# sovrasov/3d-object-detection.pytorch

Hardware: AMD Instinct MI355X
Metric: regression train crops/sec @224^2 bs256 MobileNetV2 (higher is better)
Workload: dtype bf16; 1 GPU; mobilenetv2 9-class Objectron keypoint regression, train step (fwd + l1/add/CE losses + bwd + AdamW), 224x224 crops, per-GPU batch 256; global_batch=256, parallelism=dp1, roofline_sampled_steps=0, rccl_ranks=0

## Files before the change

### 3d-object-detection.pytorch_amd/csrc/abi.hip

```cpp
#include <cstddef>
#include <initializer_list>
#include <type_traits>

#include "../../include/t3d.h"
#include "abi_entries.h"

namespace {

template <class T>
struct Unknown : std::false_type {};

template <class T>
constexpr char type_code() {
  using U = std::remove_cv_t<std::remove_pointer_t<T>>;
  if constexpr (std::is_pointer<T>::value) {
    if constexpr (std::is_same<U, t3d_prologue>::value) return 'P';
    else if constexpr (std::is_same<U, t3d_bnbwd>::value) return 'B';
    else if constexpr (std::is_same<U, t3d_loss_cfg>::value) return 'L';
    else if constexpr (std::is_same<U, t3d_draw_style>::value) return 'S';
    else if constexpr (std::is_same<U, t3d_bn_fold>::value) return 'F';
    else {
      static_assert(!std::is_function<U>::value, "t3d.h: a function pointer is not a data pointer");
      return 'p';
    }
  } else if constexpr (std::is_same<T, int>::value) return 'i';
  else if constexpr (std::is_same<T, long long>::value) return 'l';
  else if constexpr (std::is_same<T, unsigned long long>::value) return 'u';
  else if constexpr (std::is_same<T, float>::value) return 'f';
  else if constexpr (std::is_same<T, double>::value) return 'd';
  else {
    static_assert(Unknown<T>::value, "t3d.h: an argument type the ABI table has no code for (see t3d_abi_entry)");
    return '?';
  }
}

template <class... A>
struct Types {
  static constexpr char str[sizeof...(A) + 1] = {type_code<A>()..., '\0'};
};
template <class... A>
constexpr const char* types_of(int (*)(A...)) { return Types<A...>::str; }

struct Entry { const char* name; const char* types; int in_step; };
#define T3D_S(fn) {#fn, types_of(&fn), 1},
#define T3D_Q(fn) {#fn, types_of(&fn), 0},
constexpr Entry kEntries[] = {T3D_ABI_ENTRIES(T3D_S, T3D_Q)};
#undef T3D_S
#undef T3D_Q
constexpr int kNumEntries = (int)(sizeof(kEntries) / sizeof(kEntries[0]));

struct Field { const char* name; size_t offset, bytes; };
struct Text { char s[640]; };

template <size_t N>
constexpr Text describe(const Field (&f)[N]) {
  Text t{};
  size_t n = 0;
  for (size_t i = 0; i < N; ++i) {
    if (i) t.s[n++] = ',';
    for (const char* c = f[i].name; *c; ++c) t.s[n++] = *c;
    for (size_t v : {f[i].offset, f[i].bytes}) {
      t.s[n++] = ':';
      size_t div = 1;
      while (v / div >= 10) div *= 10;
      for (; div; div /= 10) t.s[n++] = (char)('0' + v / div % 10);
    }
  }
  t.s[n] = '\0';
  return t;
}

#define F(m) {#m, offsetof(T3D_THIS, m), sizeof(T3D_THIS::m)},
#define T3D_STRUCT(type, members)                        \
  namespace layout_##type {                              \
  using T3D_THIS = type;                                 \
  constexpr Field fields[] = {members};                  \
  constexpr Text text = describe(fields);                \
  }
T3D_STRUCT(t3d_prologue, F(scale) F(shift) F(se) F(act) F(se_after_act))
T3D_STRUCT(t3d_bnbwd, F(alpha) F(beta) F(gamma) F(per_sample))
T3D_STRUCT(t3d_aug_sample, F(offset) F(h) F(w) F(flags) F(alpha) F(beta255) F(reserved) F(m))
T3D_STRUCT(t3d_aug_chain, F(n_ops) F(flags) F(kind) F(p) F(m2))
T3D_STRUCT(t3d_det_sample, F(offset) F(h) F(w) F(turns) F(left) F(top) F(cx0) F(cy0) F(cx1) F(cy1) F(flags) F(delta) F(alpha)
           F(sat) F(hue) F(perm) F(reserved))
T3D_STRUCT(t3d_jpeg_info, F(h) F(w) F(ncomp) F(sampling) F(mcus_x) F(mcus_y) F(seg_mcus) F(nseg) F(scan_offset) F(scan_bytes)
           F(reason) F(reserved) F(comp_dc) F(comp_ac) F(quant) F(dc_bits) F(dc_vals) F(ac_bits) F(ac_vals))
T3D_STRUCT(t3d_jpeg_seg, F(byte) F(pred) F(bit) F(reserved) F(mcu))
T3D_STRUCT(t3d_jpeg_item, F(file_offset) F(file_bytes) F(out_offset) F(block_offset) F(seg_offset) F(reserved))
T3D_STRUCT(t3d_loss_cfg, F(c_l1) F(c_mse) F(c_smoothl1) F(smoothl1_beta) F(c_add) F(c_diag) F(c_wing) F(wing_w) F(wing_eps)
           F(c_ce) F(lam_reg) F(lam_cls))
T3D_STRUCT(t3d_draw_style, F(rect_th) F(edge_th) F(kp_radius) F(font_scale) F(flags) F(colors))
T3D_STRUCT(t3d_bn_fold, F(kind) F(C) F(nrep) F(rstride) F(stats) F(count) F(gamma) F(beta) F(rm) F(rv) F(nbt) F(momentum)
           F(eps) F(o0) F(o1) F(o2) F(o3) F(o4) F(mean) F(invstd))
#undef T3D_STRUCT
#undef F

struct Struct { const char* name; int size; const char* fields; };
#define T3D_ROW(type) {#type, (int)sizeof(type), layout_##type::text.s},
constexpr Struct kStructs[] = {
    T3D_ROW(t3d_prologue) T3D_ROW(t3d_bnbwd) T3D_ROW(t3d_aug_sample) T3D_ROW(t3d_aug_chain) T3D_ROW(t3d_det_sample)
    T3D_ROW(t3d_jpeg_info) T3D_ROW(t3d_jpeg_seg) T3D_ROW(t3d_jpeg_item) T3D_ROW(t3d_loss_cfg) T3D_ROW(t3d_draw_style)
    T3D_ROW(t3d_bn_fold)};
#undef T3D_ROW
constexpr int kNumStructs = (int)(sizeof(kStructs) / sizeof(kStructs[0]));

}

extern "C" int t3d_abi_entry(int index, const char** name, const char** types, int* in_step) {
  if (index < 0 || index >= kNumEntries) return T3D_ERR_ARG;
  if (name) *name = kEntries[index].name;
  if (types) *types = kEntries[index].types;
  if (in_step) *in_step = kEntries[index].in_step;
  return T3D_OK;
}

extern "C" int t3d_abi_struct(int index, const char** name, int* size, const char** fields) {
  if (index < 0 || index >= kNumStructs) return T3D_ERR_ARG;
  if (name) *name = kStructs[index].name;
  if (size) *size = kStructs[index].size;
  if (fields) *fields = kStructs[index].fields;
  return T3D_OK;
}
```

### 3d-object-detection.pytorch_amd/csrc/elementwise.hip

```cpp
#include "common.h"

namespace {

template <typename T, bool U8>
__global__ __launch_bounds__(256) void im2col_kernel(const void* __restrict__ xin, const float* __restrict__ mean,
                                                     const float* __restrict__ istd, T* __restrict__ col, int B,
                                                     int H, int W, int Ho, int Wo) {
  extern __shared__ float tile[];
  const int WP = W + 2;
  const int hp = (Ho + 1) / 2;
  const int b = blockIdx.x / hp, oy0 = (blockIdx.x % hp) * 2;
  const int iy0 = oy0 * 2 - 1;
  const int tid = threadIdx.x;
  for (int i = tid; i < 15 * 2; i += 256) {
    const int rr = i >> 1;
    tile[rr * WP + ((i & 1) ? W + 1 : 0)] = 0.f;
  }
  if constexpr (U8) {
    const unsigned char* xu = reinterpret_cast<const unsigned char*>(xin);
    const float mu[3] = {mean[0], mean[1], mean[2]}, is[3] = {istd[0], istd[1], istd[2]};
    const int RB = W * 3;
    if ((RB & 3) == 0) {
      const int R4 = RB >> 2;
      for (int i = tid; i < 5 * R4; i += 256) {
// ... 177 lines not shown
  load_affine(a, c0, sc, sh);
#pragma unroll
  for (int j = 0; j < 8; ++j) s1[j] = s2[j] = 0.f;
  if (on) {
    for (size_t i = g; i < nvec; i += nthr) {
      float d[8], yv[8];
      Vec8<T>::load(dv + i * 8, d);
      Vec8<T>::load(y + i * 8, yv);
      const size_t bo = (i / CG / a.HW) * a.C + c0;
#pragma unroll
      for (int j = 0; j < 8; ++j) {
        const float da = fmaf(a.vec[bo + j], d[j], a.vec2[bo + j]);
        const float v = Vec8<T>::round(da * act_grad(yv[j] * sc[j] + sh[j], a.act));
        d[j] = v;
        s1[j] += v;
        s2[j] = fmaf(v, yv[j], s2[j]);
      }
      Vec8<T>::store(o + i * 8, d);
    }
  }
  if (a.stats) flush_stats(lstat, a.C, c0, on, s1, s2, a.stats);
}

__device__ __forceinline__ int pool_cgs(int CG) {
  int c = 1;
  while (c < CG && c < 32) c <<= 1;
  return c;
}

template <typename T>
__global__ __launch_bounds__(256) void se_after_sums_kernel(const EwArgs a) {
  __shared__ float red[8 * 32 * 8];
  const int CG = a.C / 8, b = blockIdx.x;
  const int cgs = pool_cgs(CG), nslots = 256 / cgs, rowl = cgs * 8;
  const int cgl = threadIdx.x & (cgs - 1), slot = threadIdx.x / cgs;
  const int cg = blockIdx.y * cgs + cgl;
  const bool on = cg < CG;
  const int c0 = on ? cg * 8 : 0;
  const T* __restrict__ dv = reinterpret_cast<const T*>(a.a);
  const T* __restrict__ y = reinterpret_cast<const T*>(a.b);
  float sc[8], sh[8], acc[8];
  load_affine(a, c0, sc, sh);
#pragma unroll
  for (int j = 0; j < 8; ++j) acc[j] = 0.f;
  if (on) {
    for (int hw = slot; hw < a.HW; hw += nslots) {
      float v[8], d[8];
      const size_t off = ((size_t)b * a.HW + hw) * a.C + c0;
      Vec8<T>::load(y + off, v);
      Vec8<T>::load(dv + off, d);
      act_affine_vec<8>(v, sc, sh, a.act);
#pragma unroll
      for (int j = 0; j < 8; ++j) acc[j] = fmaf(d[j], v[j], acc[j]);
    }
  }
#pragma unroll
  for (int j = 0; j < 8; ++j) red[slot * rowl + cgl * 8 + j] = acc[j];
  __syncthreads();
  const int t = threadIdx.x;
  const int c = blockIdx.y * rowl + t;
  if (t < rowl && c < a.C) {
    float s = 0.f;
    for (int q = 0; q < nslots; ++q) s += red[q * rowl + t];
    a.pooled[((size_t)b * a.C + c) * 2] = s;
    a.pooled[((size_t)b * a.C + c) * 2 + 1] = 0.f;
  }
}

template <typename T>
__global__ __launch_bounds__(256) void gap_fwd_kernel(const EwArgs a) {
  __shared__ float red[8 * 32 * 8];
  __shared__ float redm[8 * 32 * 8];
  __shared__ int redi[8 * 32 * 8];
  const int CG = a.C / 8, b = blockIdx.x;
  const int cgs = pool_cgs(CG), nslots = 256 / cgs, rowl = cgs * 8;
  const int cgl = threadIdx.x & (cgs - 1), slot = threadIdx.x / cgs;
  const int cg = blockIdx.y * cgs + cgl;
  const bool on = cg < CG;
  const int c0 = on ? cg * 8 : 0;
  const bool want_max = a.mode != T3D_POOL_AVG;
  const T* __restrict__ y = reinterpret_cast<const T*>(a.a);
  float sc[8], sh[8], acc[8], mx[8];
  int mi[8];
  load_affine(a, c0, sc, sh);
#pragma unroll
  for (int j = 0; j < 8; ++j) { acc[j] = 0.f; mx[j] = -INFINITY; mi[j] = 0; }
  if (on) {
    for (int hw = slot; hw < a.HW; hw += nslots) {
      float v[8];
      Vec8<T>::load(y + ((size_t)b * a.HW + hw) * a.C + c0, v);
      act_affine_vec<8>(v, sc, sh, a.act);
#pragma unroll
      for (int j = 0; j < 8; ++j) {
        acc[j] += v[j];
        if (v[j] > mx[j]) { mx[j] = v[j]; mi[j] = hw; }
      }
    }
  }
#pragma unroll
  for (int j = 0; j < 8; ++j) {
    red[slot * rowl + cgl * 8 + j] = acc[j];
    if (want_max) { redm[slot * rowl + cgl * 8 + j] = mx[j]; redi[slot * rowl + cgl * 8 + j] = mi[j]; }
  }
  __syncthreads();
  const int t = threadIdx.x;
  const int c = blockIdx.y * rowl + t;
  if (t < rowl && c < a.C) {
    float s = 0.f;
    for (int q = 0; q < nslots; ++q) s += red[q * rowl + t];
    float out = s * a.inv_hw;
    if (want_max) {
      float m = redm[t];
      int im = redi[t];
      for (int q = 1; q < nslots; ++q) {
        const float mq = redm[q * rowl + t];
        const int iq = redi[q * rowl + t];
        if (mq > m || (mq == m && iq < im)) { m = mq; im = iq; }
      }
      if (a.argmax) a.argmax[(size_t)b * a.C + c] = im;
      out = (a.mode == T3D_POOL_MAX) ? m : out + m;
    }
    a.pooled[(size_t)b * a.C + c] = out;
  }
}

template <typename T>
__global__ __launch_bounds__(256) void gap_bwd_kernel(const EwArgs a, int B, const int g_nrep, const long long g_rstride) {
  __shared__ float red[2][8 * 32 * 8];
  const int CG = a.C / 8;
  const int cgs = pool_cgs(CG), nslots = 256 / cgs, rowl = cgs * 8;
  const int cgl = threadIdx.x & (cgs - 1), slot = threadIdx.x / cgs;
  const int cg = blockIdx.y * cgs + cgl;
  const bool on = cg < CG;
  const int c0 = on ? cg * 8 : 0;
  const T* __restrict__ y = reinterpret_cast<const T*>(a.a);
  T* __restrict__ dz = reinterpret_cast<T*>(a.out);
  float sc[8], sh[8], s1[8], s2[8];
  load_affine(a, c0, sc, sh);
#pragma unroll
  for (int j = 0; j < 8; ++j) s1[j] = s2[j] = 0.f;
  if (on) {
    for (int b = blockIdx.x; b < B; b += gridDim.x) {
      float dp[8], dm[8];
      int am[8];
#pragma unroll
      for (int j = 0; j < 8; ++j) {
        const float g = a.vec[(size_t)b * a.C + c0 + j];
        dp[j] = (a.mode == T3D_POOL_MAX) ? 0.f : g * a.inv_hw;
        dm[j] = (a.mode == T3D_POOL_AVG) ? 0.f : g;
        am[j] = (a.mode == T3D_POOL_AVG) ? -1 : a.argmax[(size_t)b * a.C + c0 + j];
      }
      for (int hw = slot; hw < a.HW; hw += nslots) {
        const size_t off = ((size_t)b * a.HW + hw) * a.C + c0;
        float v[8], d[8];
        Vec8<T>::load(y + off, v);
#pragma unroll
        for (int j = 0; j < 8; ++j) d[j] = dp[j] + (hw == am[j] ? dm[j] : 0.f);
        act_grad_affine_vec<8>(d, v, sc, sh, a.act);
#pragma unroll
        for (int j = 0; j < 8; ++j) {
          d[j] = Vec8<T>::round(d[j]);
          s1[j] += d[j];
          s2[j] = fmaf(d[j], v[j], s2[j]);
        }
        Vec8<T>::store(dz + off, d);
      }
    }
  }
  if (a.stats) {
#pragma unroll
    for (int j = 0; j < 8; ++j) {
      red[0][slot * rowl + cgl * 8 + j] = s1[j];
      red[1][slot * rowl + cgl * 8 + j] = s2[j];
    }
    __syncthreads();
    const int t = threadIdx.x, c = blockIdx.y * rowl + t;
    if (t < rowl && c < a.C) {
      double u1 = 0.0, u2 = 0.0;
      for (int q = 0; q < nslots; ++q) {
        u1 += (double)red[0][q * rowl + t];
        u2 += (double)red[1][q * rowl + t];
      }
      double* st = a.stats + (size_t)(blockIdx.x % g_nrep) * g_rstride;
      atomicAdd(st + c, u1);
      atomicAdd(st + a.C + c, u2);
    }
  }
}

inline void fill_pro(EwArgs& a, const t3d_prologue* pro) {
  if (pro) { a.scale = pro->scale; a.shift = pro->shift; a.act = pro->act; }
}
inline int ew_grid(size_t nvec) {
  size_t g = (nvec + 255) / 256;
  return (int)(g < 1 ? 1 : (g > 2048 ? 2048 : g));
}

}

static int im2col_launch(int dtype, const void* x, bool u8, const float* mean, const float* istd, void* col, int B,
                         int H, int W, void* stream) {
  if (!x || !col || B <= 0 || H <= 0 || W <= 0 || (u8 && (!mean || !istd))) return T3D_ERR_ARG;
  const int Ho = (H + 2 - 3) / 2 + 1, Wo = (W + 2 - 3) / 2 + 1;
  const int grid = B * ((Ho + 1) / 2);
  const size_t lds = (size_t)15 * (W + 2) * sizeof(float);
  if (lds > 64 * 1024) return T3D_ERR_UNSUPPORTED;
  hipStream_t st = reinterpret_cast<hipStream_t>(stream);
#define T3D_IM2COL(T, U) \
  T3D_LAUNCH((im2col_kernel<T, U>), dim3(grid), dim3(256), lds, st, x, mean, istd, (T*)col, B, H, W, Ho, Wo)
  if (dtype == T3D_F32) {
    if (u8) T3D_IM2COL(float, true); else T3D_IM2COL(float, false);
  } else if (dtype == T3D_BF16) {
    if (u8) T3D_IM2COL(bf16_t, true); else T3D_IM2COL(bf16_t, false);
  } else if (dtype == T3D_F16) {
    if (u8) T3D_IM2COL(f16_t, true); else T3D_IM2COL(f16_t, false);
  } else {
    return T3D_ERR_ARG;
  }
#undef T3D_IM2COL
  T3D_CHECK_LAUNCH();
  return T3D_OK;
}

extern "C" int t3d_stem_im2col(int dtype, const float* x, void* col, int B, int H, int W, void* stream) {
  return im2col_launch(dtype, x, false, nullptr, nullptr, col, B, H, W, stream);
}

extern "C" int t3d_stem_im2col_u8(int dtype, const unsigned char* x, const float* mean, const float* inv_std, void* col,
                                  int B, int H, int W, void* stream) {
  return im2col_launch(dtype, x, true, mean, inv_std, col, B, H, W, stream);
}

extern "C" int t3d_bn_apply(int dtype, const void* y, const t3d_prologue* pro, const void* residual, void* z,
                            int M, int C, void* stream) {
  if (!y || !z || M <= 0 || C <= 0 || (C % 8)) return T3D_ERR_ARG;
  if (pro && pro->se) return T3D_ERR_UNSUPPORTED;
  EwArgs a{};
  a.a = y; a.res = residual; a.out = z; a.M = M; a.C = C;
  fill_pro(a, pro);
  const int grid = ew_grid((size_t)M * (C / 8));
  if ((size_t)grid * 256 < (size_t)(C / 8)) return T3D_ERR_UNSUPPORTED;
  hipStream_t st = reinterpret_cast<hipStream_t>(stream);
  a.fold = t3d_take_fold(a.scale);
  const size_t lds = a.fold ? (size_t)2 * C * sizeof(float) : 0;
  if (dtype == T3D_F32) T3D_LAUNCH(bn_apply_kernel<float>, dim3(grid), dim3(256), lds, st, a);
  else if (dtype == T3D_BF16) T3D_LAUNCH(bn_apply_kernel<bf16_t>, dim3(grid), dim3(256), lds, st, a);
  else if (dtype == T3D_F16) T3D_LAUNCH(bn_apply_kernel<f16_t>, dim3(grid), dim3(256), lds, st, a);
  else return T3D_ERR_ARG;
  T3D_CHECK_LAUNCH();
  return T3D_OK;
}

extern "C" int t3d_bn_act_bwd(int dtype, const void* dz, const void* y, const t3d_prologue* pro, void* dzp,
                              double* stats, int M, int C, void* stream) {
  if (!dz || !y || !dzp || M <= 0 || C <= 0 || (C % 8)) return T3D_ERR_ARG;
  if (pro && pro->se) return T3D_ERR_UNSUPPORTED;
  EwArgs a{};
  a.a = dz; a.b = y; a.out = dzp; a.stats = stats; a.M = M; a.C = C;
  fill_pro(a, pro);
  int grid = ew_grid((size_t)M * (C / 8));
  if (grid > 1024) grid = 1024;
  if ((size_t)grid * 256 < (size_t)(C / 8)) return T3D_ERR_UNSUPPORTED;
  const size_t lds = (size_t)2 * C * sizeof(double);
  hipStream_t st = reinterpret_cast<hipStream_t>(stream);
  if (dtype == T3D_F32) T3D_LAUNCH(bn_act_bwd_kernel<float>, dim3(grid), dim3(256), lds, st, a);
  else if (dtype == T3D_BF16) T3D_LAUNCH(bn_act_bwd_kernel<bf16_t>, dim3(grid), dim3(256), lds, st, a);
  else return T3D_ERR_ARG;
  T3D_CHECK_LAUNCH();
  return T3D_OK;
}

extern "C" int t3d_se_after_sums(int dtype, const void* dv, const void* y, const t3d_prologue* pro, float* ps, int B, int HW,
                                 int C, void* stream) {
  if (!dv || !y || !ps || B <= 0 || HW <= 0 || C <= 0 || (C % 8)) return T3D_ERR_ARG;
  if (pro && pro->se) return T3D_ERR_UNSUPPORTED;
  EwArgs a{};
  a.a = dv; a.b = y; a.pooled = ps; a.C = C; a.HW = HW;
  fill_pro(a, pro);
  dim3 grid(B, cdiv(C / 8, 32));
  hipStream_t st = reinterpret_cast<hipStream_t>(stream);
  if (const int rc = t3d_fold_fallback(a.scale, st)) return rc;
  if (dtype == T3D_F32) T3D_LAUNCH(se_after_sums_kernel<float>, grid, dim3(256), 0, st, a);
  else if (dtype == T3D_BF16) T3D_LAUNCH(se_after_sums_kernel<bf16_t>, grid, dim3(256), 0, st, a);
  else return T3D_ERR_ARG;
  T3D_CHECK_LAUNCH();
  return T3D_OK;
}

extern "C" int t3d_se_after_apply(int dtype, const void* dv, const void* y, const t3d_prologue* pro, const float* s,
                                  const float* g, void* du, double* stats, int B, int HW, int C, void* stream) {
  if (!dv || !y || !s || !g || !du || B <= 0 || HW <= 0 || C <= 0 || (C % 8)) return T3D_ERR_ARG;
  if (pro && pro->se) return T3D_ERR_UNSUPPORTED;
  EwArgs a{};
  a.a = dv; a.b = y; a.out = du; a.stats = stats; a.vec = s; a.vec2 = g; a.M = B * HW; a.C = C; a.HW = HW;
  fill_pro(a, pro);
  int grid = ew_grid((size_t)a.M * (C / 8));
  if (grid > 1024) grid = 1024;
  if ((size_t)grid * 256 < (size_t)(C / 8)) return T3D_ERR_UNSUPPORTED;
  const size_t lds = (size_t)2 * C * sizeof(double);
  hipStream_t st = reinterpret_cast<hipStream_t>(stream);
  if (dtype == T3D_F32) T3D_LAUNCH(se_after_apply_kernel<float>, dim3(grid), dim3(256), lds, st, a);
  else if (dtype == T3D_BF16) T3D_LAUNCH(se_after_apply_kernel<bf16_t>, dim3(grid), dim3(256), lds, st, a);
  else return T3D_ERR_ARG;
  T3D_CHECK_LAUNCH();
  return T3D_OK;
}

extern "C" int t3d_pool_fwd(int dtype, const void* y, const t3d_prologue* pro, int mode, float* pooled, int* argmax,
                            int B, int HW, int C, void* stream) {
  if (!y || !pooled || B <= 0 || HW <= 0 || C <= 0 || (C % 8)) return T3D_ERR_ARG;
  if (mode != T3D_POOL_AVG && mode != T3D_POOL_MAX && mode != T3D_POOL_AVGMAX) return T3D_ERR_ARG;
  if (pro && pro->se) return T3D_ERR_UNSUPPORTED;
  EwArgs a{};
  a.a = y; a.pooled = pooled; a.C = C; a.HW = HW; a.inv_hw = 1.f / (float)HW; a.mode = mode; a.argmax = argmax;
  fill_pro(a, pro);
  dim3 grid(B, cdiv(C / 8, 32));
  hipStream_t st = reinterpret_cast<hipStream_t>(stream);
  if (const int rc = t3d_fold_fallback(a.scale, st)) return rc;
  if (dtype == T3D_F32) T3D_LAUNCH(gap_fwd_kernel<float>, grid, dim3(256), 0, st, a);
  else if (dtype == T3D_BF16) T3D_LAUNCH(gap_fwd_kernel<bf16_t>, grid, dim3(256), 0, st, a);
  else if (dtype == T3D_F16) T3D_LAUNCH(gap_fwd_kernel<f16_t>, grid, dim3(256), 0, st, a);
  else return T3D_ERR_ARG;
  T3D_CHECK_LAUNCH();
  return T3D_OK;
}

extern "C" int t3d_gap_fwd(int dtype, const void* y, const t3d_prologue* pro, float* pooled, int B, int HW, int C,
                           void* stream) {
  return t3d_pool_fwd(dtype, y, pro, T3D_POOL_AVG, pooled, nullptr, B, HW, C, stream);
}

extern "C" int t3d_pool_bwd(int dtype, const float* dpooled, const void* y, const t3d_prologue* pro, int mode,
                            const int* argmax, void* dz, double* stats, int B, int HW, int C, void* stream) {
  if (!dpooled || !y || !dz || B <= 0 || HW <= 0 || C <= 0 || (C % 8)) return T3D_ERR_ARG;
  if (mode != T3D_POOL_AVG && mode != T3D_POOL_MAX && mode != T3D_POOL_AVGMAX) return T3D_ERR_ARG;
  if (mode != T3D_POOL_AVG && !argmax) return T3D_ERR_ARG;
  if (pro && pro->se) return T3D_ERR_UNSUPPORTED;
  EwArgs a{};
  a.a = y; a.vec = dpooled; a.out = dz; a.stats = stats; a.C = C; a.HW = HW; a.inv_hw = 1.f / (float)HW;
  a.mode = mode; a.argmax = const_cast<int*>(argmax);
  fill_pro(a, pro);
  dim3 grid(B < 256 ? B : 256, cdiv(C / 8, 32));
  hipStream_t st = reinterpret_cast<hipStream_t>(stream);
  if (dtype == T3D_F32) T3D_LAUNCH(gap_bwd_kernel<float>, grid, dim3(256), 0, st, a, B, g_t3d_reduce.nrep, g_t3d_reduce.stats_stride);
  else if (dtype == T3D_BF16) T3D_LAUNCH(gap_bwd_kernel<bf16_t>, grid, dim3(256), 0, st, a, B, g_t3d_reduce.nrep, g_t3d_reduce.stats_stride);
  else return T3D_ERR_ARG;
  T3D_CHECK_LAUNCH();
  return T3D_OK;
}
```

### 3d-object-detection.pytorch_amd/csrc/pwconv_common.h

```cpp
#pragma once
#include "common.h"

namespace t3d_pw {

struct GemmArgs {
  const void* a0;
  const void* a1;
  const float *p0, *p1, *p2;
  int act, se_after, per_sample, dgrad;
  const void* w;
  const float* bias;
  const void* e_y;
  const float *e_scale, *e_shift, *e_se;
  int e_act, e_se_after;
  const void* e_res;
  void* out;
  double* stats;
  float* ps_stats;
  int ps_wave;
  int M, HW, Kin, Nout, mtiles;
  int kz;
  float* part;
  const void* a2;
  int Kin2, ks1;
  int row0;
  const T3dFold* fold;
  const void* z_res;
  void* z_out;
  int unused_[8];
  int wfrag;
  T3dQuant quant;
};

template <typename T> __device__ __forceinline__ void ldvec(const T* p, float* v);
template <> __device__ __forceinline__ void ldvec<float>(const float* p, float* v) {
  const float4 a = *reinterpret_cast<const float4*>(p);
  v[0] = a.x; v[1] = a.y; v[2] = a.z; v[3] = a.w;
}
template <> __device__ __forceinline__ void ldvec<bf16_t>(const bf16_t* p, float* v) { Vec8<bf16_t>::load(p, v); }
template <typename T> __device__ __forceinline__ void stvec(T* p, const float* v);
template <> __device__ __forceinline__ void stvec<float>(float* p, const float* v) {
  *reinterpret_cast<float4*>(p) = make_float4(v[0], v[1], v[2], v[3]);
}
template <> __device__ __forceinline__ void stvec<bf16_t>(bf16_t* p, const float* v) { Vec8<bf16_t>::store(p, v); }


}
```

### 3d-object-detection.pytorch_amd/csrc/pwconv_deep.hip

```cpp
#include <cstdlib>
#include <type_traits>
#include "pwconv_route.h"

namespace t3d_pw {
namespace {

__device__ __forceinline__ f32x2 deep_fma_clamp01(f32x2 a, f32x2 b, f32x2 c) {
  f32x2 d;
  asm("v_pk_fma_f32 %0, %1, %2, %3 clamp" : "=v"(d) : "v"(a), "v"(b), "v"(c));
  return d;
}

#ifdef T3D_PW_TRACE
__device__ unsigned long long g_deep_trace[16];
#define DEEP_STAMP(i)                                                                                     \
  do {                                                                                                    \
    if (threadIdx.x == 0 && blockIdx.y == 0 && (blockIdx.x == 0 || blockIdx.x == gridDim.x - 1))         \
      g_deep_trace[(blockIdx.x == 0 ? 0 : 8) + (i)] = wall_clock64();                                     \
  } while (0)
#else
#define DEEP_STAMP(i)
#endif

constexpr int RT = 4;
constexpr int NW = 8;

template <bool DG, int NTW, int KSP>
__global__ __launch_bounds__(64 * NW) void pw_deep_kernel(const GemmArgs a, const int KS, const int ntiles, const int nrep,
                                                             const long long rstride) {
  constexpr int IT = RT * KSP / NW;
  static_assert(IT >= 1 && IT * NW == RT * KSP, "staging items must divide over the waves");
  extern __shared__ __attribute__((aligned(16))) unsigned char smem[];
  bf16x8* Af = reinterpret_cast<bf16x8*>(smem);
  const int kpad = KS * 32;
  float* coef = reinterpret_cast<float*>(smem + (size_t)2 * RT * KSP * 1024);
  const int BN = ntiles * 16;
  float* ecoef = coef + 3 * kpad;
  double* dstat = reinterpret_cast<double*>(ecoef + 2 * BN);

  const int tid = threadIdx.x, lane = tid & 63, wave = tid >> 6;
  const int lg = lane >> 4, lc = lane & 15;
  const int m0 = blockIdx.x * (16 * RT), n0 = blockIdx.y * BN;
  const bf16_t* __restrict__ A0 = reinterpret_cast<const bf16_t*>(a.a0);
  const bf16_t* __restrict__ A1 = reinterpret_cast<const bf16_t*>(a.a1);
  bf16_t* __restrict__ out = reinterpret_cast<bf16_t*>(a.out);
  const int nph = (KS + KSP - 1) / KSP;
  DEEP_STAMP(0);

  int tix[NTW];
  bool tok[NTW];
  const int tlast = min(ntiles, (a.Nout - n0 + 31) / 32 * 2) - 1;
  const bf16x8* wt_[NTW];
#pragma unroll
  for (int i = 0; i < NTW; ++i) {
    const int t = wave + NW * i;
    tok[i] = t <= tlast;
    tix[i] = min(t, tlast);
    wt_[i] = reinterpret_cast<const bf16x8*>(a.w) + ((size_t)(n0 / 16 + tix[i]) * KS) * 64 + lane;
  }
  bf16x8 wf[2][KSP][NTW];
  auto w_issue = [&](auto slot_tag, const int ph) {
    constexpr int SL = decltype(slot_tag)::value;
#pragma unroll
    for (int u = 0; u < KSP; ++u) {
      const int ks = min(ph * KSP + u, KS - 1);
#pragma unroll
      for (int t = 0; t < NTW; ++t) wf[SL][u][t] = wt_[t][(size_t)ks * 64];
    }
  };
  const int srt = wave % RT, sks = (wave / RT) * IT;
  const int mrow = min(m0 + srt * 16 + lc, a.M - 1);
  const size_t arow = (size_t)mrow * a.Kin + lg * 8;
  const bool rok = m0 + srt * 16 + lc < a.M;
  bf16x8 pa[2][IT], pb[DG ? 2 : 1][DG ? IT : 1];
  auto a_issue = [&](auto slot_tag, const int ph) {
    constexpr int SL = decltype(slot_tag)::value;
#pragma unroll
    for (int j = 0; j < IT; ++j) {
      const size_t o = arow + min((ph * KSP + sks + j) * 32, a.Kin - 8 - lg * 8);
      pa[SL][j] = *reinterpret_cast<const bf16x8*>(A0 + o);
      if (DG) pb[DG ? SL : 0][DG ? j : 0] = *reinterpret_cast<const bf16x8*>(A1 + o);
    }
  };
  w_issue(std::integral_constant<int, 0>{}, 0);
  a_issue(std::integral_constant<int, 0>{}, 0);
  a_issue(std::integral_constant<int, 1>{}, 1);

  for (int i = tid; i < BN * 2; i += 64 * NW) dstat[i] = 0.0;
  for (int i = tid; i < BN; i += 64 * NW) {
    const int n = n0 + i;
    const bool v = DG && a.e_scale && n < a.Nout;
    ecoef[i] = v ? a.e_scale[n] : 1.f;
    ecoef[BN + i] = v ? a.e_shift[n] : 0.f;
  }
  if (a.fold) {
    for (int i = a.Kin + tid; i < kpad; i += 64 * NW) {
      coef[i] = DG ? 0.f : 1.f; coef[kpad + i] = 0.f; coef[2 * kpad + i] = 0.f;
    }
    t3d_fold_block<DG ? 2 : 1>(a.fold, 0, a.Kin, coef, kpad, blockIdx.x == 0 && blockIdx.y == 0);
  } else {
    for (int i = tid; i < kpad; i += 64 * NW) {
      const bool v = i < a.Kin;
      if (!DG) {
        coef[i] = (v && a.p0) ? a.p0[i] : 1.f;
        coef[kpad + i] = (v && a.p0) ? a.p1[i] : 0.f;
      } else {
        coef[i] = v ? a.p0[i] : 0.f;
        coef[kpad + i] = v ? a.p1[i] : 0.f;
        coef[2 * kpad + i] = v ? a.p2[i] : 0.f;
      }
    }
    __syncthreads();
  }
  const bool c6f = !DG && a.p0 && a.act == T3D_ACT_RELU6;
  if (c6f) {
    for (int i = tid; i < 2 * kpad; i += 64 * NW) coef[i] *= T3D_SIXTH;
    __syncthreads();
  }
  const int fact = c6f ? -1 : a.act;
  DEEP_STAMP(1);

  f32x4 acc[RT][NTW];
#pragma unroll
  for (int r = 0; r < RT; ++r)
#pragma unroll
    for (int t = 0; t < NTW; ++t) acc[r][t] = f32x4{0.f, 0.f, 0.f, 0.f};

  auto phase = [&](auto slot_tag, const int ph) {
    constexpr int SL = decltype(slot_tag)::value;
    bf16x8* Ab = Af + (size_t)SL * RT * KSP * 64;
#pragma unroll
    for (int j = 0; j < IT; ++j) {
      const int k = (ph * KSP + sks + j) * 32 + lg * 8;
      const bool ok = rok && (k < a.Kin);
      const int kc = min(k, kpad - 8);
      const float4 c0a = *reinterpret_cast<const float4*>(coef + kc), c0b = *reinterpret_cast<const float4*>(coef + kc + 4);
      const float4 c1a = *reinterpret_cast<const float4*>(coef + kpad + kc),
                   c1b = *reinterpret_cast<const float4*>(coef + kpad + kc + 4);
      const float c0[8] = {c0a.x, c0a.y, c0a.z, c0a.w, c0b.x, c0b.y, c0b.z, c0b.w};
      const float c1[8] = {c1a.x, c1a.y, c1a.z, c1a.w, c1b.x, c1b.y, c1b.z, c1b.w};
      float x[8];
#pragma unroll
      for (int e = 0; e < 8; ++e) x[e] = (float)pa[SL][j][e];
      if (!DG) {
        if (fact == -1) {
#pragma unroll
          for (int e = 0; e < 8; e += 2) {
            const f32x2 t = deep_fma_clamp01(f32x2{x[e], x[e + 1]}, f32x2{c0[e], c0[e + 1]}, f32x2{c1[e], c1[e + 1]});
            x[e] = t[0];
            x[e + 1] = t[1];
          }
        } else {
          act_affine_vec<8>(x, c0, c1, fact);
        }
      } else {
        const float4 c2a = *reinterpret_cast<const float4*>(coef + 2 * kpad + kc),
                     c2b = *reinterpret_cast<const float4*>(coef + 2 * kpad + kc + 4);
        const float c2[8] = {c2a.x, c2a.y, c2a.z, c2a.w, c2b.x, c2b.y, c2b.z, c2b.w};
#pragma unroll
        for (int e = 0; e < 8; ++e) x[e] = c0[e] * x[e] + c1[e] * (float)pb[DG ? SL : 0][DG ? j : 0][e] + c2[e];
      }
      bf16x8 b;
#pragma unroll
      for (int e = 0; e < 8; ++e) b[e] = ok ? (bf16_t)x[e] : (bf16_t)0.f;
      Ab[(srt * KSP + sks + j) * 64 + lane] = b;
    }
    __syncthreads();
    if (ph == 0) DEEP_STAMP(2);
    __builtin_amdgcn_sched_barrier(0);
    w_issue(std::integral_constant<int, 1 - SL>{}, ph + 1);
    a_issue(std::integral_constant<int, SL>{}, ph + 2);
    __builtin_amdgcn_sched_barrier(0);
#pragma unroll
    for (int u = 0; u < KSP; ++u) {
      bf16x8 b[RT];
#pragma unroll
      for (int r = 0; r < RT; ++r) b[r] = Ab[(r * KSP + u) * 64 + lane];
#pragma unroll
      for (int t = 0; t < NTW; ++t)
#pragma unroll
        for (int r = 0; r < RT; ++r) acc[r][t] = __builtin_amdgcn_mfma_f32_16x16x32_bf16(wf[SL][u][t], b[r], acc[r][t], 0, 0, 0);
    }
    __builtin_amdgcn_sched_barrier(0);
  };
  for (int ph = 0; ph < nph; ph += 2) {
    phase(std::integral_constant<int, 0>{}, ph);
    if (ph + 1 < nph) phase(std::integral_constant<int, 1>{}, ph + 1);
  }

  DEEP_STAMP(3);
  const bool keep_stats = a.stats != nullptr;
  float st1[NTW][4], st2[NTW][4];
#pragma unroll
  for (int i = 0; i < NTW; ++i)
#pragma unroll
    for (int j = 0; j < 4; ++j) st1[i][j] = st2[i][j] = 0.f;
  bf16x4 eyr[DG ? RT : 1][NTW], err[DG ? RT : 1][NTW];
  if (DG) {
#pragma unroll
    for (int r = 0; r < RT; ++r) {
      const size_t mo = (size_t)min(m0 + r * 16 + lc, a.M - 1) * a.Nout;
#pragma unroll
      for (int i = 0; i < NTW; ++i) {
        const int n = min(n0 + (tix[i] >> 1) * 32 + lg * 8 + (tix[i] & 1) * 4, a.Nout - 4);
        if (a.e_y) eyr[DG ? r : 0][i] = *reinterpret_cast<const bf16x4*>(reinterpret_cast<const bf16_t*>(a.e_y) + mo + n);
        if (a.e_res) err[DG ? r : 0][i] = *reinterpret_cast<const bf16x4*>(reinterpret_cast<const bf16_t*>(a.e_res) + mo + n);
      }
    }
  }
#pragma unroll
  for (int r = 0; r < RT; ++r) {
    const int m = m0 + r * 16 + lc;
    const bool ok = m < a.M;
#pragma unroll
    for (int i = 0; i < NTW; ++i) {
      const int nl = (tix[i] >> 1) * 32 + lg * 8 + (tix[i] & 1) * 4, n = n0 + nl;
      if (!tok[i] || n >= a.Nout) continue;
      float v[4], yv[4];
#pragma unroll
      for (int j = 0; j < 4; ++j) v[j] = acc[r][i][j];
      if (c6f) {
#pragma unroll
        for (int j = 0; j < 4; ++j) v[j] *= 6.f;
      }
      if (DG && a.e_y) {
#pragma unroll
        for (int j = 0; j < 4; ++j) yv[j] = (float)eyr[DG ? r : 0][i][j];
        if (a.e_act != T3D_ACT_NONE) {
          const float4 s0 = *reinterpret_cast<const float4*>(ecoef + nl), h0 = *reinterpret_cast<const float4*>(ecoef + BN + nl);
          const float es[4] = {s0.x, s0.y, s0.z, s0.w}, eh[4] = {h0.x, h0.y, h0.z, h0.w};
          act_grad_affine_vec<4>(v, yv, es, eh, a.e_act);
        }
      }
      if (DG && a.e_res) {
#pragma unroll
        for (int j = 0; j < 4; ++j) v[j] += (float)err[DG ? r : 0][i][j];
      }
      bf16x4 o;
#pragma unroll
      for (int j = 0; j < 4; ++j) {
        o[j] = (bf16_t)v[j];
        v[j] = ok ? (float)o[j] : 0.f;
      }
      if (ok) *reinterpret_cast<bf16x4*>(out + (size_t)m * a.Nout + n) = o;
      if (keep_stats) {
#pragma unroll
        for (int j = 0; j < 4; ++j) {
          st1[i][j] += v[j];
          st2[i][j] = fmaf(v[j], (DG && a.e_y) ? yv[j] : v[j], st2[i][j]);
        }
      }
    }
  }
  DEEP_STAMP(4);
  if (keep_stats) {
#pragma unroll
    for (int i = 0; i < NTW; ++i) {
      const int nl = (tix[i] >> 1) * 32 + lg * 8 + (tix[i] & 1) * 4;
#pragma unroll
      for (int j = 0; j < 4; ++j) {
        const float s1 = row16_sum(st1[i][j]), s2 = row16_sum(st2[i][j]);
        if (lc == 0 && tok[i] && n0 + nl < a.Nout) {
          dstat[(nl + j) * 2] = t3d_snap(s1, a.quant, false);
          dstat[(nl + j) * 2 + 1] = t3d_snap(s2, a.quant, !DG);
        }
      }
    }
    __syncthreads();
    for (int i = tid; i < BN * 2; i += 64 * NW) {
      const int n = n0 + (i >> 1);
      if (n < a.Nout) atomicAdd(a.stats + (size_t)(blockIdx.x % nrep) * rstride + (size_t)(i & 1) * a.Nout + n, dstat[i]);
    }
  }
  DEEP_STAMP(5);
}

size_t deep_lds(int KS, int ntiles, int KSP = 4) { return (size_t)2 * RT * KSP * 1024 + (size_t)3 * KS * 32 * 4 + (size_t)ntiles * 16 * (2 * 4 + 2 * 8); }

template <bool DG, int NTW, int KSP>
int launch_deep(GemmArgs& a, int KS, int ntiles, int nchunks, hipStream_t st) {
  const size_t lds = deep_lds(KS, ntiles, KSP);
  const void* fn = (const void*)pw_deep_kernel<DG, NTW, KSP>;
  if (lds > 64 * 1024) (void)t3d_max_lds(fn, (int)lds);
  a.quant = (!DG && a.stats && !T3D_ENV_SET("T3D_NO_SNAP")) ? t3d_quant_for(a.M) : T3dQuant{0.0, 0.0};
  a.fold = t3d_take_fold(a.p0);
  T3D_LAUNCH_TIMED((pw_deep_kernel<DG, NTW, KSP>), dim3(cdiv(a.M, 16 * RT), nchunks), dim3(64 * NW), lds, st, a, KS, ntiles,
                     g_t3d_reduce.nrep, g_t3d_reduce.stats_stride);
  T3D_CHECK_LAUNCH();
  return T3D_OK;
}

__global__ void pack_frag_kernel(const unsigned short* __restrict__ w, unsigned short* __restrict__ out, int rows, int cols, int KS,
                                 size_t total) {
  for (size_t i = blockIdx.x * (size_t)blockDim.x + threadIdx.x; i < total; i += (size_t)gridDim.x * blockDim.x) {
    const int j = i & 7, lc = (i >> 3) & 15, lg = (i >> 7) & 3;
    const size_t tk = i >> 9;
    const int ks = (int)(tk % KS), T = (int)(tk / KS);
    const int n = (T >> 1) * 32 + (lc >> 2) * 8 + (T & 1) * 4 + (lc & 3), k = ks * 32 + lg * 8 + j;
    out[i] = (n < rows && k < cols) ? w[(size_t)n * cols + k] : (unsigned short)0;
  }
}

}

#ifdef T3D_PW_TRACE
extern "C" int t3d_debug_deep_trace(unsigned long long* out) {
  return hipMemcpyFromSymbol(out, HIP_SYMBOL(g_deep_trace), sizeof(unsigned long long) * 16) == hipSuccess ? 0 : -1;
}
#endif

bool deep_shape(int Kin, int Nout) {
  if (Kin < 512 || (Kin % 8) || (Nout % 8)) return false;
  const int KS = cdiv(Kin, 32);
  int nt_cap = 120 / KS;
  if (nt_cap > 10) nt_cap = 10;
  nt_cap &= ~1;
  return !(nt_cap >= 2 && Nout <= nt_cap * 16);
}

struct DeepChunks {
  int nchunks, ntiles;
  explicit DeepChunks(int Nout) {
    const int pairs = cdiv(Nout, 32);
    nchunks = cdiv(pairs, 8);
    ntiles = 2 * cdiv(pairs, nchunks);
  }
};

bool deep_can(const PwCall& c) {
  if (c.dtype != T3D_BF16 || !c.wfrag || (c.op != PW_FWD && c.op != PW_DGRAD) || c.gen() || c.bias) return false;
  if (c.op == PW_DGRAD && !c.alpha_gamma) return false;
  return deep_shape(c.Kin, c.Nout) && deep_lds(cdiv(c.Kin, 32), DeepChunks(c.Nout).ntiles) <= 150 * 1024;
}

int deep_launch(const PwCall& c, GemmArgs& a, hipStream_t st) {
  if (!deep_can(c)) return T3D_ERR_ARG;
  const DeepChunks ch(a.Nout);
  return a.dgrad ? launch_deep<true, 2, 4>(a, cdiv(a.Kin, 32), ch.ntiles, ch.nchunks, st)
                 : launch_deep<false, 2, 4>(a, cdiv(a.Kin, 32), ch.ntiles, ch.nchunks, st);
}

}

extern "C" int t3d_pwconv_frag_bytes(int rows, int cols) {
  if (rows <= 0 || cols <= 0) return 0;
  return 2 * cdiv(rows, 32) * cdiv(cols, 32) * 1024;
}

extern "C" int t3d_pwconv_wants_frag(int K, int N) { return t3d_pw::deep_shape(K, N) ? 1 : 0; }

extern "C" int t3d_pwconv_pack_frag(const void* w, void* out, int rows, int cols, void* stream) {
  if (!w || !out || rows <= 0 || cols <= 0) return T3D_ERR_ARG;
  const size_t total = (size_t)t3d_pwconv_frag_bytes(rows, cols) / 2;
  T3D_LAUNCH(t3d_pw::pack_frag_kernel, dim3((unsigned)((total + 255) / 256 < 2048 ? (total + 255) / 256 : 2048)), dim3(256), 0,
                     reinterpret_cast<hipStream_t>(stream), reinterpret_cast<const unsigned short*>(w), reinterpret_cast<unsigned short*>(out), rows,
                     cols, cdiv(cols, 32), total);
  T3D_CHECK_LAUNCH();
  return T3D_OK;
}
```

### 3d-object-detection.pytorch_amd/csrc/pwconv_route.h

```cpp
#pragma once
#include "pwconv_common.h"

namespace t3d_pw {

enum { PW_FWD = T3D_PW_OP_FWD, PW_FWD_STATS = T3D_PW_OP_FWD_STATS, PW_MAT = T3D_PW_OP_MAT, PW_DGRAD = T3D_PW_OP_DGRAD, PW_WGRAD = T3D_PW_OP_WGRAD };

struct PwCall {
  int op, dtype, wfrag;
  int gated;
  int per_sample;
  int ps_stats;
  int e_se;
  int bias, stats;
  int alpha_gamma;
  int act;
  int residual;
  int M, HW, Kin, Nout;
  bool gen() const { return per_sample || ps_stats || e_se || (op != PW_DGRAD && gated); }
};

int t3d_pw_route(const PwCall& c);

bool deep_can(const PwCall& c);
int deep_launch(const PwCall& c, GemmArgs& a, hipStream_t st);
bool deep_shape(int Kin, int Nout);
bool stream_can(const PwCall& c);
int stream_launch(const PwCall& c, GemmArgs& a, hipStream_t st);
bool stream_f16_can(const PwCall& c);
int stream_launch_f16(const PwCall& c, GemmArgs& a, hipStream_t st);
bool reg32_can(const PwCall& c);
int reg32_launch(const PwCall& c, GemmArgs& a, hipStream_t st);
bool reg32_wgrad_can(const PwCall& c);
int reg32_wgrad_launch(const PwCall& c, const float* dz, const float* y, const t3d_bnbwd* bb, const float* x, const t3d_prologue* pro,
                       float* dw, hipStream_t st);
bool lds_can(const PwCall& c);
int lds_launch(const PwCall& c, GemmArgs& a, hipStream_t st);
bool lds_wgrad_can(const PwCall& c);
int lds_wgrad_launch(const PwCall& c, const void* dz, const void* y, const t3d_bnbwd* bb, const void* x, const t3d_prologue* pro, float* dw,
                     hipStream_t st);
bool tr_can(const PwCall& c);
int tr_launch(const PwCall& c, const void* dz, const void* y, const t3d_bnbwd* bb, const void* x, const t3d_prologue* pro, float* dw,
              hipStream_t st);

}
```

### 3d-object-detection.pytorch_amd/csrc/pwconv_route.hip

```cpp
#include "pwconv_route.h"

using namespace t3d_pw;

extern "C" int t3d_bn_apply(int dtype, const void* y, const t3d_prologue* pro, const void* residual, void* z, int M, int C,
                            void* stream);

namespace {

int g_forced = T3D_PW_AUTO;

bool family_can(int route, const PwCall& c) {
  const bool wg = c.op == PW_WGRAD;
  switch (route) {
    case T3D_PW_DEEP: return deep_can(c);
    case T3D_PW_STREAM: return stream_can(c) || stream_f16_can(c);
    case T3D_PW_REG32: return wg ? reg32_wgrad_can(c) : reg32_can(c);
    case T3D_PW_LDS: return wg ? lds_wgrad_can(c) : lds_can(c);
    case T3D_PW_TR: return tr_can(c);
    default: return false;
  }
}
const int kOrder[] = {T3D_PW_DEEP, T3D_PW_STREAM, T3D_PW_REG32, T3D_PW_TR, T3D_PW_LDS};

int settle(int route, const PwCall& c, const float* key, hipStream_t st) {
// ... 17 lines not shown
  PwCall c{};
  c.op = op; c.dtype = dtype & ~T3D_W_FRAG; c.wfrag = (dtype & T3D_W_FRAG) != 0;
  c.M = M; c.HW = HW; c.Kin = Kin; c.Nout = Nout;
  return c;
}

}

int t3d_pw::t3d_pw_route(const PwCall& c) {
  const bool sizes = c.M > 0 && c.HW > 0 && c.Kin > 0 && c.Nout > 0 && !(c.Kin % 8) && !(c.Nout % 8);
  if (c.op == PW_FWD_STATS) {
    const bool stream = g_forced == T3D_PW_AUTO || g_forced == T3D_PW_STREAM;
    return sizes && stream && stream_can(c) ? T3D_PW_STREAM : T3D_ERR_UNSUPPORTED;
  }
  if (!sizes || c.dtype < T3D_F32 || c.dtype > T3D_F16) return T3D_ERR_ARG;
  if (c.wfrag && c.dtype == T3D_F32) return T3D_ERR_ARG;
  if (c.op == PW_MAT && c.gated) return T3D_ERR_ARG;
  if (c.op == PW_WGRAD && (c.wfrag || c.dtype == T3D_F16)) return T3D_ERR_ARG;
  const int none = c.op != PW_MAT ? T3D_ERR_UNSUPPORTED : !c.wfrag ? T3D_PW_PAIR : c.dtype == T3D_BF16 ? T3D_ERR_UNSUPPORTED : T3D_ERR_ARG;
  if (g_forced != T3D_PW_AUTO) return family_can(g_forced, c) ? g_forced : (none == T3D_PW_PAIR ? none : T3D_ERR_UNSUPPORTED);
  for (const int r : kOrder)
    if (family_can(r, c)) return r;
  return none;
}

extern "C" int t3d_pwconv_route(int op, int dtype, int gated, int per_sample, int ps_stats, int e_se, int bias, int stats,
                                int alpha_gamma, int act, int residual, int M, int HW, int K, int N) {
  if (op < PW_FWD || op > PW_WGRAD) return T3D_ERR_ARG;
  const bool bwd = op == PW_DGRAD || op == PW_WGRAD;
  PwCall c = call(op, dtype, M, HW, bwd ? N : K, bwd ? K : N);
  const bool fwd = !bwd, dg = op == PW_DGRAD;
  c.gated = gated && !dg; c.per_sample = per_sample && bwd; c.ps_stats = ps_stats && dg; c.e_se = e_se && dg;
  c.bias = bias && (op == PW_FWD || op == PW_FWD_STATS); c.stats = stats && op != PW_WGRAD; c.alpha_gamma = alpha_gamma && bwd;
  c.act = fwd ? act : T3D_ACT_NONE; c.residual = residual && op == PW_MAT;
  return t3d_pw_route(c);
}

extern "C" int t3d_pwconv_force_route(int route) {
  if (route != T3D_PW_AUTO && (route < 0 || route > T3D_PW_TR)) return T3D_ERR_ARG;
  g_forced = route;
  return T3D_OK;
}

extern "C" int t3d_pwconv_fwd(int dtype, const void* x, const t3d_prologue* pro, const void* w, const float* bias,
                              void* y, double* stats, int M, int HW, int K, int N, void* stream) {
  if (!x || !w || (!y && !stats)) return T3D_ERR_ARG;
  PwCall c = call(y ? PW_FWD : PW_FWD_STATS, dtype, M, HW, K, N);
  c.gated = pro && pro->se; c.act = pro ? pro->act : T3D_ACT_NONE; c.bias = bias != nullptr; c.stats = stats != nullptr;
  const int route = t3d_pw_route(c);
  if (route < 0) return route;
  GemmArgs a{};
  a.a0 = x;
  if (pro) { a.p0 = pro->scale; a.p1 = pro->shift; a.p2 = pro->se; a.act = pro->act; a.se_after = pro->se_after_act; }
  a.w = w; a.bias = bias; a.out = y; a.stats = stats;
  a.M = M; a.HW = HW; a.Kin = K; a.Nout = N;
  return run(route, c, a, stream);
}

extern "C" int t3d_pwconv_fwd_mat(int dtype, const void* y_in, const t3d_prologue* pro_in, const void* residual, void* z_out,
                                  const void* w, void* y, double* stats, int M, int HW, int K, int N, void* stream) {
  if (!y_in || !pro_in || !z_out || !w || !y) return T3D_ERR_ARG;
  PwCall c = call(PW_MAT, dtype, M, HW, K, N);
  c.gated = pro_in->se != nullptr; c.act = pro_in->act; c.residual = residual != nullptr; c.stats = stats != nullptr;
  const int route = t3d_pw_route(c);
  if (route < 0) return route;
  if (route == T3D_PW_PAIR) {
    if (c.dtype == T3D_F32 && g_forced == T3D_PW_AUTO)
      if (const int rc = t3d_fold_fallback(pro_in->scale, reinterpret_cast<hipStream_t>(stream))) return rc;
    if (const int rc = t3d_bn_apply(c.dtype, y_in, pro_in, residual, z_out, M, K, stream)) return rc;
    return t3d_pwconv_fwd(c.dtype, z_out, nullptr, w, nullptr, y, stats, M, HW, K, N, stream);
  }
  GemmArgs a{};
  a.a0 = y_in;
  a.p0 = pro_in->scale; a.p1 = pro_in->shift; a.act = pro_in->act;
  a.z_res = residual; a.z_out = z_out;
  a.w = w; a.out = y; a.stats = stats;
  a.M = M; a.HW = HW; a.Kin = K; a.Nout = N;
  return run(route, c, a, stream);
}

extern "C" int t3d_pwconv_dgrad(int dtype, const void* dz, const void* y, const t3d_bnbwd* bb, const void* wt,
                                const void* x_raw, const t3d_prologue* pro_in, const void* residual, void* dx,
                                double* stats, float* ps_stats, int M, int HW, int K, int N, void* stream) {
  if (!dz || !y || !bb || !wt || !dx || !bb->beta) return T3D_ERR_ARG;
  PwCall c = call(PW_DGRAD, dtype, M, HW, N, K);
  c.per_sample = bb->per_sample != 0; c.alpha_gamma = bb->alpha && bb->gamma; c.e_se = x_raw && pro_in && pro_in->se;
  c.stats = stats != nullptr; c.ps_stats = ps_stats != nullptr;
  const int route = t3d_pw_route(c);
  if (route < 0) return route;
  GemmArgs a{};
  a.dgrad = 1;
  a.a0 = dz; a.a1 = y;
  a.p0 = bb->alpha; a.p1 = bb->beta; a.p2 = bb->gamma; a.per_sample = bb->per_sample;
  a.w = wt;
  if (x_raw) {
    a.e_y = x_raw;
    if (pro_in) {
      a.e_scale = pro_in->scale; a.e_shift = pro_in->shift; a.e_se = pro_in->se;
      a.e_act = pro_in->act; a.e_se_after = pro_in->se_after_act;
    }
  }
  a.e_res = residual; a.out = dx; a.stats = stats; a.ps_stats = ps_stats;
  a.M = M; a.HW = HW; a.Kin = N; a.Nout = K;
  return run(route, c, a, stream);
}

extern "C" int t3d_pwconv_wgrad(int dtype, const void* dz, const void* y, const t3d_bnbwd* bb, const void* x,
                                const t3d_prologue* pro, float* dw, int M, int HW, int K, int N, void* stream) {
  if (!dz || !y || !bb || !x || !dw) return T3D_ERR_ARG;
  PwCall c = call(PW_WGRAD, dtype, M, HW, N, K);
  c.gated = pro && pro->se; c.per_sample = bb->per_sample != 0; c.alpha_gamma = bb->alpha && bb->gamma;
  const int route = t3d_pw_route(c);
  if (route < 0) return route;
  hipStream_t st = reinterpret_cast<hipStream_t>(stream);
  if (const int rc = settle(route, c, bb->alpha, st)) return rc;
  switch (route) {
    case T3D_PW_TR: return tr_launch(c, dz, y, bb, x, pro, dw, st);
    case T3D_PW_REG32:
      return reg32_wgrad_launch(c, reinterpret_cast<const float*>(dz), reinterpret_cast<const float*>(y), bb,
                                reinterpret_cast<const float*>(x), pro, dw, st);
    default: return lds_wgrad_launch(c, dz, y, bb, x, pro, dw, st);
  }
}
```

### 3d-object-detection.pytorch_amd/csrc/pwconv_stream.hip

```cpp
#include <cstdlib>
#include <type_traits>
#ifdef T3D_PW_TRACE
#include <hip/hip_runtime.h>
static __device__ unsigned long long g_pw_trace[16];
#define T3D_FOLD_STAMP(i)                                                                                 \
  do {                                                                                                    \
    asm volatile("s_waitcnt vmcnt(0) lgkmcnt(0)" ::: "memory");                                           \
    if (threadIdx.x == 0 && (blockIdx.x == 0 || blockIdx.x == gridDim.x - 1))                            \
      g_pw_trace[(blockIdx.x == 0 ? 0 : 8) + 5 + (i)] = wall_clock64();                                   \
  } while (0)
#endif
#include "pwconv_route.h"

#ifndef T3D_PW_F16
typedef bf16_t ST;
typedef bf16x8 ST8;
#define T3D_PW_MFMA __builtin_amdgcn_mfma_f32_16x16x32_bf16
#define T3D_PW_LAUNCH stream_launch
#define T3D_PW_CAN stream_can
#else
typedef f16_t ST;
typedef f16x8 ST8;
#define T3D_PW_MFMA __builtin_amdgcn_mfma_f32_16x16x32_f16
#define T3D_PW_LAUNCH stream_launch_f16
#define T3D_PW_CAN stream_f16_can
#endif

namespace t3d_pw {
__device__ __forceinline__ f32x2 pk_fma_clamp01(f32x2 a, f32x2 b, f32x2 c) {
  f32x2 d;
  asm("v_pk_fma_f32 %0, %1, %2, %3 clamp" : "=v"(d) : "v"(a), "v"(b), "v"(c));
  return d;
}

namespace {


#ifdef T3D_PW_TRACE
#define PW_STAMP(i)                                                                                     \
  do {                                                                                                    \
    if (threadIdx.x == 0 && (blockIdx.x == 0 || blockIdx.x == gridDim.x - 1))                            \
      g_pw_trace[(blockIdx.x == 0 ? 0 : 8) + (i)] = wall_clock64();                                       \
  } while (0)
#else
#define PW_STAMP(i)
#endif

template <int NT, int R, bool DG, bool GEN, bool YF = false, int KU = 2, bool ZM = false>
__global__ __launch_bounds__(512, KU > 2 ? 1 : 2) void pw_stream_kernel(const GemmArgs a, const int nchunks, const int KS, const int nrep, const long long rstride) {
  constexpr int BN = NT * 16;
  extern __shared__ __attribute__((aligned(16))) unsigned char smem[];
  ST8* Wf = reinterpret_cast<ST8*>(smem);
  const int kpad = KS * 32;
  float* coef = reinterpret_cast<float*>(smem + (size_t)NT * KS * 1024);
  float* lstat = coef + 3 * kpad;
  float* ecoef = lstat + BN * 2;
  double* dstat = reinterpret_cast<double*>(ecoef + 2 * BN);

  const int tid = threadIdx.x, lane = tid & 63, wave = tid >> 6;
  const int lg = lane >> 4, lc = lane & 15;
  const int nxb = gridDim.x / nchunks;
  int chunk, xb;
  if (nchunks > 1 && (nxb & 7) == 0) {
    const int xcd = blockIdx.x & 7, j = blockIdx.x >> 3;
    chunk = j % nchunks;
    xb = (j / nchunks) * 8 + xcd;
  } else {
    chunk = blockIdx.x % nchunks;
    xb = blockIdx.x / nchunks;
  }
  const int n0 = chunk * BN;
  const ST* __restrict__ A0 = reinterpret_cast<const ST*>(a.a0);
  const ST* __restrict__ A1 = reinterpret_cast<const ST*>(a.a1);
  const ST* __restrict__ A2 = reinterpret_cast<const ST*>(a.a2);
  const int ks1 = A2 ? a.ks1 : (1 << 30);
  const ST* __restrict__ Wg = reinterpret_cast<const ST*>(a.w);
  ST* __restrict__ out = reinterpret_cast<ST*>(a.out);
  PW_STAMP(0);

  const int nthr = blockDim.x, WAVES = nthr >> 6;
  auto stage_weights = [&]() {
  if (a.wfrag) {
    constexpr int SU = 8;
    const int total = NT * KS * 64, tiles = (a.Nout + 31) / 32 * 2, t0 = n0 / 16;
    const ST8* __restrict__ P = reinterpret_cast<const ST8*>(a.w) + (size_t)t0 * KS * 64;
    const int valid = max(0, min(NT, tiles - t0)) * KS * 64;
    for (int i0 = tid; i0 < total; i0 += nthr * SU) {
      ST8 v[SU];
#pragma unroll
      for (int u = 0; u < SU; ++u) v[u] = P[min(i0 + u * nthr, valid - 1)];
#pragma unroll
      for (int u = 0; u < SU; ++u) {
        const int i = i0 + u * nthr;
        if (i >= valid) {
#pragma unroll
          for (int j = 0; j < 8; ++j) v[u][j] = (ST)0.f;
        }
        if (i < total) Wf[i] = v[u];
      }
    }
  } else {
    constexpr int SU = 8;
    const int total = NT * KS * 64;
    for (int i0 = tid; i0 < total; i0 += nthr * SU) {
      ST8 v[SU];
      bool ok[SU];
#pragma unroll
      for (int u = 0; u < SU; ++u) {
        const int i = min(i0 + u * nthr, total - 1);
        const int l = i & 63, ks = (i >> 6) % KS, t = (i >> 6) / KS;
        const int n = n0 + (t >> 1) * 32 + ((l & 15) >> 2) * 8 + (t & 1) * 4 + (l & 3), k = ks * 32 + (l >> 4) * 8;
        ok[u] = n < a.Nout && k < a.Kin;
        v[u] = *reinterpret_cast<const ST8*>(Wg + (size_t)min(n, a.Nout - 1) * a.Kin + min(k, a.Kin - 8));
      }
#pragma unroll
      for (int u = 0; u < SU; ++u) {
        if (!ok[u]) {
#pragma unroll
          for (int j = 0; j < 8; ++j) v[u][j] = (ST)0.f;
        }
        if (i0 + u * nthr < total) Wf[i0 + u * nthr] = v[u];
      }
    }
  }
  for (int i = tid; i < BN * 2; i += nthr) { lstat[i] = 0.f; dstat[i] = 0.0; }
  for (int i = tid; i < BN; i += nthr) {
    const int n = n0 + i;
    const bool v = DG && a.e_scale && n < a.Nout;
    ecoef[i] = v ? a.e_scale[n] : 1.f;
    ecoef[BN + i] = v ? a.e_shift[n] : 0.f;
  }
  };
  constexpr bool DGL = DG && !YF;
  if (!YF && a.fold) {
    for (int i = a.Kin + tid; i < kpad; i += nthr) {
      coef[i] = DG ? 0.f : 1.f; coef[kpad + i] = 0.f; coef[2 * kpad + i] = 0.f;
    }
    t3d_fold_block<DG ? 2 : 1>(a.fold, 0, a.Kin, coef, kpad, blockIdx.x == 0, stage_weights);
  } else {
  stage_weights();
  for (int i = tid; i < kpad; i += nthr) {
    const bool v = i < a.Kin;
    if (YF) {
      coef[i] = 1.f; coef[kpad + i] = 0.f; coef[2 * kpad + i] = 0.f;
    } else if (!DG) {
      coef[i] = (v && a.p0) ? a.p0[i] : 1.f;
      coef[kpad + i] = (v && a.p0) ? a.p1[i] : 0.f;
    } else {
      coef[i] = (v && !a.per_sample) ? a.p0[i] : 0.f;
      coef[kpad + i] = v ? a.p1[i] : 0.f;
      coef[2 * kpad + i] = (v && !a.per_sample) ? a.p2[i] : 0.f;
    }
  }
  }
  __syncthreads();
  const bool c6f = !DG && !ZM && !YF && a.act == T3D_ACT_RELU6 && !(GEN && a.p2);
  if (c6f) {
    for (int i = tid; i < 2 * kpad; i += nthr) coef[i] *= T3D_SIXTH;
    __syncthreads();
  }
  PW_STAMP(1);

  const bool plainA = !ZM && (YF || (!DG && !a.p0 && !a.p2 && a.act == T3D_ACT_NONE));
  const bool keep_stats = a.stats != nullptr;
  float st1[NT / 2][8], st2[NT / 2][8];
#pragma unroll
  for (int q = 0; q < NT / 2; ++q)
#pragma unroll
    for (int j = 0; j < 8; ++j) st1[q][j] = st2[q][j] = 0.f;

  const int ngroups = (a.M + 16 * R - 1) / (16 * R);
  const int nb = n0 + lg * 8;

  const bool ps_mode = GEN && a.ps_stats != nullptr;
  const int wv = xb * WAVES + wave, nwv = nxb * WAVES;
  const int gps = (a.HW + 16 * R - 1) / (16 * R);
  const bool wos = ps_mode && a.ps_wave;
  const int s_end = ps_mode ? a.M / a.HW : 1, s_step = wos ? nwv : (ps_mode ? nxb : 1);
  for (int sb = wos ? wv : (ps_mode ? xb : 0); sb < s_end; sb += s_step) {
  const int g_begin = wos ? 0 : (ps_mode ? wave : wv), g_end = ps_mode ? gps : ngroups, g_step = wos ? 1 : (ps_mode ? WAVES : nwv);
  const int mbase = ps_mode ? sb * a.HW : 0, mlim = ps_mode ? min(a.M, (sb + 1) * a.HW) : a.M;
  for (int g = g_begin; g < g_end; g += g_step) {
    const int m0 = mbase + g * 16 * R;
    f32x4 acc[R][NT];
#pragma unroll
    for (int r = 0; r < R; ++r)
#pragma unroll
      for (int t = 0; t < NT; ++t) acc[r][t] = f32x4{0.f, 0.f, 0.f, 0.f};
    int mrow[R], mld[R];
    bool mok[R];
#pragma unroll
    for (int r = 0; r < R; ++r) {
      mrow[r] = m0 + r * 16 + lc;
      mok[r] = mrow[r] < mlim;
      mld[r] = min(mrow[r], a.M - 1);
    }

    constexpr bool HOIST = DG && !YF && !GEN && KU > 2;
    ST8 eyh[R][NT / 2];
    if constexpr (HOIST) {
#pragma unroll
      for (int r = 0; r < R; ++r)
#pragma unroll
        for (int q = 0; q < NT / 2; ++q)
          eyh[r][q] = *reinterpret_cast<const ST8*>(reinterpret_cast<const ST*>(a.e_y) + (size_t)mld[r] * a.Nout +
                                                       min(nb + 32 * q, a.Nout - 8));
    }
    auto k_round = [&](auto ku_tag, auto guard_tag, const int ks0) {
      constexpr int KUr = decltype(ku_tag)::value;
      constexpr bool GUARD = decltype(guard_tag)::value;
      ST8 fa[KUr][R], fb[KUr][R];
      ST8 fz[ZM ? KUr : 1][R];
      float4 gs[GEN && !DGL ? KUr : 1][R][2];
      const bool gated = GEN && !DGL && a.p2 != nullptr;
#pragma unroll
      for (int u = 0; u < KUr; ++u) {
        const int ks = ks0 + u;
        if (GUARD && ks >= KS) continue;
        if (YF && ks >= ks1) {
          const int k = min((ks - ks1) * 32 + lg * 8, a.Kin2 - 8);
#pragma unroll
          for (int r = 0; r < R; ++r) fa[u][r] = *reinterpret_cast<const ST8*>(A2 + (size_t)mld[r] * a.Kin2 + k);
        } else {
          const int k = min(ks * 32 + lg * 8, a.row0 - 8);
#pragma unroll
          for (int r = 0; r < R; ++r) {
            {
              fa[u][r] = *reinterpret_cast<const ST8*>(A0 + (size_t)mld[r] * a.row0 + k);
              if (DGL) fb[u][r] = *reinterpret_cast<const ST8*>(A1 + (size_t)mld[r] * a.row0 + k);
              if constexpr (ZM) {
                if (a.z_res)
                  fz[u][r] = *reinterpret_cast<const ST8*>(reinterpret_cast<const ST*>(a.z_res) + (size_t)mld[r] * a.row0 + k);
              }
              if constexpr (GEN && !DGL) {
                if (gated) {
                  const float* gp = a.p2 + (size_t)(mld[r] / a.HW) * a.Kin + min(ks * 32 + lg * 8, a.Kin - 8);
                  gs[u][r][0] = *reinterpret_cast<const float4*>(gp);
                  gs[u][r][1] = *reinterpret_cast<const float4*>(gp + 4);
                }
              }
            }
          }
        }
      }
#pragma unroll
      for (int u = 0; u < KUr; ++u) {
        const int ks = ks0 + u;
        if (!GUARD || ks < KS) {
          const int k = ks * 32 + lg * 8;
          ST8 b[R];
          if (plainA) {
#pragma unroll
            for (int r = 0; r < R; ++r) b[r] = fa[u][r];
          } else {
            const float4 c0a = *reinterpret_cast<const float4*>(coef + k), c0b = *reinterpret_cast<const float4*>(coef + k + 4);
            const float4 c1a = *reinterpret_cast<const float4*>(coef + kpad + k),
                         c1b = *reinterpret_cast<const float4*>(coef + kpad + k + 4);
            const float c0[8] = {c0a.x, c0a.y, c0a.z, c0a.w, c0b.x, c0b.y, c0b.z, c0b.w};
            const float c1[8] = {c1a.x, c1a.y, c1a.z, c1a.w, c1b.x, c1b.y, c1b.z, c1b.w};
            if (!DGL) {
#pragma unroll
              for (int r = 0; r < R; ++r) {
                const bool ok = mok[r] && (k < a.Kin);
                float x[8];
#pragma unroll
                for (int j = 0; j < 8; ++j) x[j] = (float)fa[u][r][j];
                if (GEN && a.p2) {
                  const float4 g0 = gs[GEN && !DGL ? u : 0][r][0], g1 = gs[GEN && !DGL ? u : 0][r][1];
                  const float sg[8] = {g0.x, g0.y, g0.z, g0.w, g1.x, g1.y, g1.z, g1.w};
                  float sv[8];
#pragma unroll
                  for (int j = 0; j < 8; ++j) sv[j] = ok ? sg[j] : 1.f;
                  if (!a.se_after) {
                    float c0s[8], c1s[8];
#pragma unroll
                    for (int j = 0; j < 8; ++j) { c0s[j] = c0[j] * sv[j]; c1s[j] = c1[j] * sv[j]; }
                    act_affine_vec<8>(x, c0s, c1s, a.act);
                  } else {
                    act_affine_vec<8>(x, c0, c1, a.act);
#pragma unroll
                    for (int j = 0; j < 8; ++j) x[j] *= sv[j];
                  }
                } else if (c6f) {
#pragma unroll
                  for (int j = 0; j < 8; j += 2) {
                    const f32x2 t = pk_fma_clamp01(f32x2{x[j], x[j + 1]}, f32x2{c0[j], c0[j + 1]}, f32x2{c1[j], c1[j + 1]});
                    x[j] = t[0];
                    x[j + 1] = t[1];
                  }
                } else {
                  act_affine_vec<8>(x, c0, c1, a.act);
                }
                if constexpr (ZM) {
                  if (a.z_res) {
#pragma unroll
                    for (int j = 0; j < 8; ++j) x[j] += (float)fz[u][r][j];
                  }
                }
#pragma unroll
                for (int j = 0; j < 8; ++j) b[r][j] = (ST)x[j];
                if constexpr (ZM) {
                  if (chunk == 0 && ok)
                    *reinterpret_cast<ST8*>(reinterpret_cast<ST*>(a.z_out) + (size_t)mrow[r] * a.row0 + k) = b[r];
                }
              }
            } else {
              const float4 c2a = *reinterpret_cast<const float4*>(coef + 2 * kpad + k),
                           c2b = *reinterpret_cast<const float4*>(coef + 2 * kpad + k + 4);
              const float c2[8] = {c2a.x, c2a.y, c2a.z, c2a.w, c2b.x, c2b.y, c2b.z, c2b.w};
#pragma unroll
              for (int r = 0; r < R; ++r) {
                const bool ok = mok[r] && (k < a.Kin);
                const size_t pb = (GEN && a.per_sample && ok) ? (size_t)(mrow[r] / a.HW) * a.Kin + k : 0;
#pragma unroll
                for (int j = 0; j < 8; ++j) {
                  const float al = (GEN && a.per_sample) ? (ok ? a.p0[pb + j] : 0.f) : c0[j];
                  const float ga = (GEN && a.per_sample) ? (ok ? a.p2[pb + j] : 0.f) : c2[j];
                  b[r][j] = (ST)(al * (float)fa[u][r][j] + c1[j] * (float)fb[u][r][j] + ga);
                }
              }
            }
          }
#pragma unroll
          for (int t = 0; t < NT; ++t) {
            const ST8 wf = Wf[(t * KS + ks) * 64 + lane];
#pragma unroll
            for (int r = 0; r < R; ++r) acc[r][t] = T3D_PW_MFMA(wf, b[r], acc[r][t], 0, 0, 0);
          }
        }
      }
    };
    int ks0 = 0;
    if constexpr (KU > 2)
      for (; ks0 + KU <= KS; ks0 += KU) k_round(std::integral_constant<int, KU>{}, std::false_type{}, ks0);
    for (; ks0 < KS; ks0 += 2) k_round(std::integral_constant<int, 2>{}, std::true_type{}, ks0);


    if (g == g_begin) PW_STAMP(2);
#pragma unroll
    for (int r = 0; r < R; ++r) {
      const int m = mrow[r];
      const bool ok = mok[r];
      const int mrow0 = m0 + r * 16, mlast = mrow0 + 15;
      const int bidx = ok ? m / a.HW : 0;
      ST8 eyr[NT / 2], err[NT / 2];
      float4 esg[GEN ? NT / 2 : 1][2];
      if constexpr (GEN && DG) {
        if (a.e_se) {
#pragma unroll
          for (int q = 0; q < NT / 2; ++q) {
            const float* gp = a.e_se + (size_t)(mld[r] / a.HW) * a.Nout + min(nb + 32 * q, a.Nout - 8);
            esg[q][0] = *reinterpret_cast<const float4*>(gp);
            esg[q][1] = *reinterpret_cast<const float4*>(gp + 4);
          }
        }
      }
      if constexpr (HOIST) {
#pragma unroll
        for (int q = 0; q < NT / 2; ++q) eyr[q] = eyh[r][q];
      } else if (DG) {
        if (a.e_y) {
#pragma unroll
          for (int q = 0; q < NT / 2; ++q)
            eyr[q] = *reinterpret_cast<const ST8*>(reinterpret_cast<const ST*>(a.e_y) + (size_t)mld[r] * a.Nout +
                                                      min(nb + 32 * q, a.Nout - 8));
        }
        if (a.e_res) {
#pragma unroll
          for (int q = 0; q < NT / 2; ++q)
            err[q] = *reinterpret_cast<const ST8*>(reinterpret_cast<const ST*>(a.e_res) + (size_t)mld[r] * a.Nout +
                                                      min(nb + 32 * q, a.Nout - 8));
        }
      }
#pragma unroll
      for (int q = 0; q < NT / 2; ++q) {
        const int n = nb + 32 * q;
        if (n >= a.Nout) continue;
        float v[8], yv[8];
#pragma unroll
        for (int j = 0; j < 8; ++j) v[j] = acc[r][2 * q + (j >> 2)][j & 3];
        if (c6f) {
#pragma unroll
          for (int j = 0; j < 8; ++j) v[j] *= 6.f;
        }
        if ((!DG || YF) && a.bias) {
#pragma unroll
          for (int j = 0; j < 8; ++j) v[j] += a.bias[n + j];
        }
        if (DG && a.e_y) {
#pragma unroll
          for (int j = 0; j < 8; ++j) yv[j] = (float)eyr[q][j];
          if (GEN && a.e_se) {
            const float4 s0 = *reinterpret_cast<const float4*>(ecoef + (n - n0)), s1 = *reinterpret_cast<const float4*>(ecoef + (n - n0) + 4);
            const float4 h0 = *reinterpret_cast<const float4*>(ecoef + BN + (n - n0)),
                         h1 = *reinterpret_cast<const float4*>(ecoef + BN + (n - n0) + 4);
            float es[8] = {s0.x, s0.y, s0.z, s0.w, s1.x, s1.y, s1.z, s1.w};
// ... 32 lines not shown
#pragma unroll
        for (int j = 0; j < 8; ++j) v[j] = ok ? Vec8<ST>::round(v[j]) : 0.f;
        if (ok && out) Vec8<ST>::store(out + (size_t)m * a.Nout + n, v);
        if (keep_stats) {
#pragma unroll
          for (int j = 0; j < 8; ++j) {
            st1[q][j] += v[j];
            st2[q][j] = fmaf(v[j], (DG && a.e_y) ? yv[j] : v[j], st2[q][j]);
          }
        } else if (GEN && a.ps_stats) {
#pragma unroll
          for (int j = 0; j < 8; ++j) {
            st1[q][j] += v[j];
            st2[q][j] = fmaf(v[j], yv[j], st2[q][j]);
          }
        }
      }
    }
  }
  if (wos) {
#pragma unroll
    for (int q = 0; q < NT / 2; ++q) {
      const int n = nb + 32 * q;
#pragma unroll
      for (int j = 0; j < 8; ++j) {
        const float s1 = row16_sum(st1[q][j]), s2 = row16_sum(st2[q][j]);
        st1[q][j] = st2[q][j] = 0.f;
        if (lc == 0 && n < a.Nout) {
          a.ps_stats[((size_t)sb * a.Nout + n + j) * 2] = s1;
          a.ps_stats[((size_t)sb * a.Nout + n + j) * 2 + 1] = s2;
        }
      }
    }
  } else if (ps_mode) {
#pragma unroll
    for (int q = 0; q < NT / 2; ++q) {
      const int n = nb + 32 * q;
#pragma unroll
      for (int j = 0; j < 8; ++j) {
        const float s1 = row16_sum(st1[q][j]), s2 = row16_sum(st2[q][j]);
        st1[q][j] = st2[q][j] = 0.f;
        if (lc == 0 && n < a.Nout && g_begin < g_end) {
          atomicAdd(dstat + (n - n0 + j) * 2, (double)s1);
          atomicAdd(dstat + (n - n0 + j) * 2 + 1, (double)s2);
        }
      }
    }
    __syncthreads();
    for (int i = tid; i < BN * 2; i += nthr) {
      const int n = n0 + (i >> 1);
      if (n < a.Nout) a.ps_stats[((size_t)sb * a.Nout + n) * 2 + (i & 1)] = (float)dstat[i];
      dstat[i] = 0.0;
    }
    __syncthreads();
  }
  }
  PW_STAMP(3);

  if (keep_stats) {
#pragma unroll
    for (int q = 0; q < NT / 2; ++q) {
      const int n = nb + 32 * q;
      float mine = 0.f;
#pragma unroll
      for (int j = 0; j < 8; ++j) {
        const float s1 = row16_sum(st1[q][j]), s2 = row16_sum(st2[q][j]);
        mine = lc == j ? s1 : (lc == j + 8 ? s2 : mine);
      }
      if (n < a.Nout) {
        const double d = lc < 8 ? t3d_snap(mine, a.quant, false) : t3d_snap(mine, a.quant, !DG);
        atomicAdd(dstat + (n - n0 + (lc & 7)) * 2 + (lc >> 3), d);
      }
    }
    __syncthreads();
    for (int i = tid; i < BN * 2; i += nthr) {
      const int n = n0 + (i >> 1);
      if (n < a.Nout) atomicAdd(a.stats + (size_t)(xb % nrep) * rstride + (size_t)(i & 1) * a.Nout + n, dstat[i]);
    }
  }
  PW_STAMP(4);
}

template <int NT, int R, bool DG, bool GEN, bool YF = false, int KU = 2, bool ZM = false>
int launch_v(GemmArgs& a, int KS, hipStream_t st) {
  constexpr int BN = NT * 16;
  const int kpad = KS * 32;
  const size_t lds = (size_t)NT * KS * 1024 + (size_t)3 * kpad * 4 + BN * 4 * 4 + BN * 2 * 8;
  const int nchunks = cdiv(a.Nout, BN);
  const int ngroups = cdiv(a.M, 16 * R);
  const bool ps = GEN && a.ps_stats != nullptr;
  const int gps = cdiv(a.HW, 16 * R);
  const int threads = (lds <= 48 * 1024 || (ps && gps <= 4)) ? 256 : 512;
  const void* fn = (const void*)pw_stream_kernel<NT, R, DG, GEN, YF, KU, ZM>;
  if (lds > 64 * 1024) (void)t3d_max_lds(fn, (int)lds);
  static int occ_cache[2] = {0, 0};
  int& occ = occ_cache[threads == 512];
  if (occ == 0) {
    int n = 0;
    if (hipOccupancyMaxActiveBlocksPerMultiprocessor(&n, fn, threads, 0) != hipSuccess || n < 1) n = 1;
    occ = n;
  }
  int per_cu = occ;
  const int by_lds = (int)(160 * 1024 / (lds + 512));
  if (per_cu > by_lds) per_cu = by_lds;
  if (per_cu < 1) per_cu = 1;
  int nxb = (256 * per_cu) / nchunks;
  a.ps_wave = (ps && gps <= 16) ? 1 : 0;
  const int need = ps ? (a.ps_wave ? cdiv(a.M / a.HW, threads / 64) : a.M / a.HW) : cdiv(ngroups, threads / 64);
  if (nxb > need) nxb = need;
  if (nxb < 1) nxb = 1;
  if (nchunks > 1 && nxb >= 8) {
    const int up = (nxb + 7) & ~7;
    nxb = (up * nchunks <= 256 * per_cu) ? up : (nxb & ~7);
  }
  a.quant = (!DG && a.stats && !T3D_ENV_SET("T3D_NO_SNAP")) ? t3d_quant_for(a.M) : T3dQuant{0.0, 0.0};
  a.fold = (YF || a.per_sample) ? nullptr : t3d_take_fold(a.p0);
  T3D_LAUNCH_TIMED((pw_stream_kernel<NT, R, DG, GEN, YF, KU, ZM>), dim3(nxb * nchunks), dim3(threads), lds, st, a, nchunks, KS,
                     g_t3d_reduce.nrep, g_t3d_reduce.stats_stride);
  T3D_CHECK_LAUNCH();
  return T3D_OK;
}

template <int NT, int R>
int launch_nt(GemmArgs& a, int KS, hipStream_t st) {
#ifdef T3D_PW_F16
  if (a.p2) return launch_v<NT, R, false, true>(a, KS, st);
  return launch_v<NT, R, false, false>(a, KS, st);
#else
  if (a.a2) return launch_v<NT, R, true, false, true>(a, KS, st);
  const bool gen = a.per_sample || a.ps_stats || a.e_se || (!a.dgrad && a.p2);
  if (a.dgrad) return gen ? launch_v<NT, R, true, true>(a, KS, st) : launch_v<NT, R, true, false>(a, KS, st);
  if (a.z_out) return launch_v<NT, R, false, false, false, 2, true>(a, KS, st);
  return gen ? launch_v<NT, R, false, true>(a, KS, st) : launch_v<NT, R, false, false>(a, KS, st);
#endif
}

}

#if defined(T3D_PW_TRACE) && !defined(T3D_PW_F16)
extern "C" int t3d_debug_pw_trace(unsigned long long* out) {
  return hipMemcpyFromSymbol(out, HIP_SYMBOL(g_pw_trace), sizeof(unsigned long long) * 16) == hipSuccess ? 0 : -1;
}
#endif

#ifdef T3D_PW_F16
bool T3D_PW_CAN(const PwCall& c) { return c.dtype == T3D_F16 && c.op == PW_FWD && !c.stats && c.Kin <= 1920; }
#else
bool T3D_PW_CAN(const PwCall& c) {
  if (c.dtype != T3D_BF16 || c.op == PW_WGRAD || c.Kin > 1920) return false;
  if (c.ps_stats && (c.stats || c.M % c.HW)) return false;
  return !(c.op == PW_MAT && c.gated);
}
#endif

int T3D_PW_LAUNCH(const PwCall& c, GemmArgs& a, hipStream_t st) {
  if (!T3D_PW_CAN(c)) return T3D_ERR_ARG;
  if (!a.row0) a.row0 = a.Kin;
  const int KS = cdiv(a.Kin, 32);
  int nt_cap = (120 * 1024 / 1024) / KS;
  if (nt_cap > 10) nt_cap = 10;
  const int gen_cap = 6;
  if (a.dgrad && (a.per_sample || a.ps_stats || a.e_se) && nt_cap > gen_cap) nt_cap = gen_cap;
  nt_cap &= ~1;
  int NT = 2;
  {
    int best_chunks = 1 << 30, best_pad = 1 << 30;
    for (int nt = 2; nt <= nt_cap; nt += 2) {
      const int ch = cdiv(a.Nout, nt * 16), pad = ch * nt * 16 - a.Nout;
      if (ch < best_chunks || (ch == best_chunks && pad < best_pad)) { best_chunks = ch; best_pad = pad; NT = nt; }
    }
  }
  if (NT > 6 && nt_cap >= 6 && cdiv(a.Nout, NT * 16) > 1 && a.Nout % 96 == 0 &&
      !(a.per_sample || a.ps_stats || a.e_se || (!a.dgrad && a.p2)))
    NT = 6;
  switch (NT) {
    case 2: return launch_nt<2, 2>(a, KS, st);
    case 4: return launch_nt<4, 2>(a, KS, st);
    case 6:
      if (a.per_sample || a.ps_stats || a.e_se || (!a.dgrad && a.p2)) return launch_nt<6, 1>(a, KS, st);
      return launch_nt<6, 2>(a, KS, st);
    case 8: return launch_nt<8, 1>(a, KS, st);
    default: return launch_nt<10, 1>(a, KS, st);
  }
}

}
```

### 3d-object-detection.pytorch_amd/csrc/pwconv_wgrad_tr.hip

```cpp
#include <cstdlib>
#include "pwconv_route.h"

namespace {

__device__ __forceinline__ f32x2 pk_fma_clamp01(f32x2 a, f32x2 b, f32x2 c) {
  f32x2 d;
  asm("v_pk_fma_f32 %0, %1, %2, %3 clamp" : "=v"(d) : "v"(a), "v"(b), "v"(c));
  return d;
}

typedef __attribute__((ext_vector_type(4))) short s16x4;

__device__ __forceinline__ void act_vec8(float* v, int act) {
  switch (act) {
    case T3D_ACT_RELU:
#pragma unroll
      for (int j = 0; j < 8; ++j) v[j] = fmaxf(v[j], 0.f);
      break;
    case T3D_ACT_RELU6:
#pragma unroll
      for (int j = 0; j < 8; ++j) v[j] = __builtin_amdgcn_fmed3f(v[j], 0.f, 6.f);
      break;
    case T3D_ACT_HSWISH:
#pragma unroll
      for (int j = 0; j < 8; ++j) v[j] = v[j] * (__builtin_amdgcn_fmed3f(v[j] + 3.f, 0.f, 6.f) * T3D_SIXTH);
      break;
    default: break;
  }
}

struct WgtArgs {
  const void *dz, *y, *x;
  const float *alpha, *beta, *gamma;
  int per_sample;
  const float *scale, *shift, *se;
  int act, se_after;
  float* dw;
  int M, HW, K, N;
  int yfree, Nz;
  int swap;
  int ptiles, qtiles, rows_per_split, nsplit;
  float* ws;
  const T3dFold* fold;
  const bf16_t* wd;
  const bf16_t* wtr;
  const void *e_res, *e_y;
  void* dx;
  double* stats;
  int nrep;
  long long rstride;
  int unused_[10];
  int assign;
  int gs_ns;
  unsigned mulHW;
};

__device__ __forceinline__ bf16x8 tr_frag(const bf16_t* tile, int rs, int ch0, int lane) {
  const int g = lane >> 4, q = (lane & 15) >> 2, p = lane & 3;
  const bf16_t* a0 = tile + (8 * g + q) * rs + ch0 + 4 * p;
  const s16x4 lo = __builtin_amdgcn_ds_read_tr16_b64_v4i16((s16x4 __attribute__((address_space(3)))*)(a0));
  const s16x4 hi = __builtin_amdgcn_ds_read_tr16_b64_v4i16((s16x4 __attribute__((address_space(3)))*)(a0 + 4 * rs));
  typedef __attribute__((ext_vector_type(8))) short s16x8;
  const s16x8 v = {lo[0], lo[1], lo[2], lo[3], hi[0], hi[1], hi[2], hi[3]};
  return __builtin_bit_cast(bf16x8, v);
}

template <int NTPW, int NTQ, bool SWAP, int G, int D, int GEN, bool YF, int SK = 1, bool DGF = false>
__global__ __launch_bounds__(256 * G) void pw_wgrad_tr_kernel(const WgtArgs a) {
  static_assert(!DGF || (YF && !SWAP), "the fused data gradient exists for the y-free layout only");
  constexpr int PB = 64 * NTPW, QB = 16 * NTQ;
  constexpr int RSP = PB + 8, RSQ = QB + 8;
  constexpr int STEP = 32 * SK;
  extern __shared__ __attribute__((aligned(16))) unsigned char smem[];
  constexpr int BUFE = STEP * (RSP + RSQ);
  const int grp = threadIdx.x >> 8;
  bf16_t* const tiles = reinterpret_cast<bf16_t*>(smem) + grp * 2 * BUFE;
  float* coef = reinterpret_cast<float*>(reinterpret_cast<bf16_t*>(smem) + G * 2 * BUFE);
  constexpr int RSW = PB + 8;
  constexpr int NCOEF = 3 * (SWAP ? QB : PB) + 2 * (SWAP ? PB : QB);
  bf16_t* const wdl = reinterpret_cast<bf16_t*>(coef + ((NCOEF + 3) & ~3));
  double* const dstat = reinterpret_cast<double*>(wdl + (DGF ? QB * RSW : 0));

  const int tid = threadIdx.x & 255, lane = tid & 63, wave = tid >> 6;
  const int P = SWAP ? a.K : a.N, Q = SWAP ? a.N : a.K;
  const int ntiles = a.ptiles * a.qtiles, s8 = a.nsplit & ~7;
  int tile, split;
  {
    const int L = blockIdx.x;
    if (ntiles > 1 && L < ntiles * s8) {
      const int j = L >> 3;
      tile = j % ntiles;
      split = (j / ntiles) * 8 + (L & 7);
    } else {
      const int Lr = ntiles > 1 ? L - ntiles * s8 : L;
      tile = Lr % ntiles;
      split = (ntiles > 1 ? s8 : 0) + Lr / ntiles;
    }
  }
  const int pt = tile / a.qtiles, qt = tile % a.qtiles;
  const int p0 = pt * PB, q0 = qt * QB;
  const int mbeg = split * a.rows_per_split, mend = min(a.M, mbeg + a.rows_per_split);
  constexpr int dyB = SWAP ? QB : PB, aB = SWAP ? PB : QB;
  const int dy0 = SWAP ? q0 : p0, a0c = SWAP ? p0 : q0;
  float* cdy = coef;
  float* ca = coef + 3 * dyB;
  if (!YF && a.fold) {
    const int nv = min(dyB, a.N - dy0);
    for (int i = nv + threadIdx.x; i < dyB; i += 256 * G) cdy[i] = cdy[dyB + i] = cdy[2 * dyB + i] = 0.f;
    t3d_fold_block<2>(a.fold, dy0, nv, cdy, dyB, false);
  } else {
  for (int i = threadIdx.x; i < dyB && !YF; i += 256 * G) {
    const int n = dy0 + i;
    const bool v = n < a.N;
    cdy[i] = (v && !a.per_sample) ? a.alpha[n] : 0.f;
    cdy[dyB + i] = v ? a.beta[n] : 0.f;
    cdy[2 * dyB + i] = (v && !a.per_sample) ? a.gamma[n] : 0.f;
  }
  }
  const bool c6 = !GEN && !YF && a.act == T3D_ACT_RELU6 && !a.se;
  for (int i = threadIdx.x; i < aB; i += 256 * G) {
    const int k = a0c + i;
    const bool v = k < a.K;
    ca[i] = ((v && a.scale) ? a.scale[k] : 1.f) * (c6 ? T3D_SIXTH : 1.f);
    ca[aB + i] = ((v && a.scale) ? a.shift[k] : 0.f) * (c6 ? T3D_SIXTH : 1.f);
  }
  float* const gsl = coef + ((NCOEF + 3) & ~3);
  const int gs_b0 = GEN ? mbeg / a.HW : 0;
  if constexpr (GEN == 2) {
    {
      const int nb = a.M / a.HW;
      for (int i = threadIdx.x; i < a.gs_ns * aB; i += 256 * G) {
        const int sb = i / aB, c = i % aB, b = min(gs_b0 + sb, nb - 1), k = a0c + c;
        gsl[i] = k < a.K ? a.se[(size_t)b * a.K + k] : 0.f;
      }
    }
  }
  if constexpr (DGF) {
    if (a.wd) {
      for (int i = threadIdx.x; i < QB * (PB / 8); i += 256 * G) {
        const int r = i / (PB / 8), c = (i % (PB / 8)) * 8;
        *reinterpret_cast<bf16x8*>(wdl + r * RSW + c) = *reinterpret_cast<const bf16x8*>(a.wd + (size_t)r * PB + c);
      }
    } else {
      const int Nz = a.Nz, K = a.K;
      float* fco = cdy;
      if (a.fold) {
        for (int i = Nz + threadIdx.x; i < dyB; i += 256 * G) fco[i] = fco[dyB + i] = fco[2 * dyB + i] = 0.f;
        t3d_fold_block<2>(a.fold, 0, Nz, fco, dyB, blockIdx.x == 0);
      } else {
        for (int i = threadIdx.x; i < dyB; i += 256 * G) {
          const bool v = i < Nz;
          fco[i] = v ? a.alpha[i] : 0.f; fco[dyB + i] = v ? a.beta[i] : 0.f; fco[2 * dyB + i] = v ? a.gamma[i] : 0.f;
        }
      }
      for (int i = threadIdx.x; i < QB * (RSW / 8); i += 256 * G) *reinterpret_cast<bf16x8*>(wdl + i * 8) = bf16x8{};
      __syncthreads();
      const float *alpha = fco, *beta = fco + dyB, *gamma = fco + 2 * dyB;
      const bf16_t* __restrict__ wtr = a.wtr;
      for (int i = threadIdx.x; i < QB * (Nz / 8); i += 256 * G) {
        const int k = i / (Nz / 8), n = (i % (Nz / 8)) * 8;
        if (k < K) {
          const bf16x8 v = *reinterpret_cast<const bf16x8*>(wtr + (size_t)k * Nz + n);
          bf16x8 o;
#pragma unroll
          for (int j = 0; j < 8; ++j) o[j] = (bf16_t)(alpha[n + j] * (float)v[j]);
          *reinterpret_cast<bf16x8*>(wdl + k * RSW + n) = o;
        }
      }
      f32x4* qred = reinterpret_cast<f32x4*>(tiles);
      const int lgq_ = lane >> 4, lcq_ = lane & 15;
      const int nst = (Nz + 31) / 32;
      for (int kt = 0; kt < QB / 16; ++kt)
        for (int qt2 = 0; qt2 < QB / 16; ++qt2) {
          f32x4 qa = {0.f, 0.f, 0.f, 0.f};
          if (grp == 0) {
            const int ka = min(kt * 16 + lcq_, K - 1), kb = min(qt2 * 16 + lcq_, K - 1);
            const bf16_t* ra = wtr + (size_t)ka * Nz;
            const bf16_t* rb = wtr + (size_t)kb * Nz;
            for (int st = wave; st < nst; st += 4) {
              const int n = st * 32 + 8 * lgq_;
              const bool live = n < Nz;
              const int nc = min(n, Nz - 8);
              const bf16x8 fa = *reinterpret_cast<const bf16x8*>(ra + nc);
              const bf16x8 fb = *reinterpret_cast<const bf16x8*>(rb + nc);
              bf16x8 b;
#pragma unroll
              for (int j = 0; j < 8; ++j) b[j] = (bf16_t)(live ? beta[nc + j] * (float)fb[j] : 0.f);
              qa = __builtin_amdgcn_mfma_f32_16x16x32_bf16(fa, b, qa, 0, 0, 0);
            }
            if (wave) qred[(wave - 1) * 64 + lane] = qa;
          }
          __syncthreads();
          if (grp == 0 && wave == 0) {
            qa += qred[lane];
            qa += qred[64 + lane];
            qa += qred[128 + lane];
#pragma unroll
            for (int r = 0; r < 4; ++r) {
              const int k = kt * 16 + 4 * lgq_ + r, k2 = qt2 * 16 + lcq_;
              if (k < K && k2 < K) wdl[k * RSW + Nz + k2] = (bf16_t)qa[r];
            }
          }
          __syncthreads();
        }
      if (grp == 0) {
        for (int kb = 0; kb < QB; kb += 16) {
          const int row = tid >> 4, sub = tid & 15, k = kb + row;
          float s2 = 0.f;
          if (k < K)
            for (int n = sub * 8; n < Nz; n += 128) {
              const bf16x8 v = *reinterpret_cast<const bf16x8*>(wtr + (size_t)k * Nz + n);
#pragma unroll
              for (int j = 0; j < 8; ++j) s2 = fmaf(gamma[n + j], (float)v[j], s2);
            }
          s2 = row16_sum(s2);
          if (sub == 0 && k < K) wdl[k * RSW + Nz + K] = (bf16_t)s2;
        }
      }
    }
    for (int i = threadIdx.x; i < 2 * QB; i += 256 * G) dstat[i] = 0.0;
  }
  const bf16_t* __restrict__ dz = reinterpret_cast<const bf16_t*>(a.dz);
  const bf16_t* __restrict__ yy = reinterpret_cast<const bf16_t*>(a.y);
  const bf16_t* __restrict__ xx = reinterpret_cast<const bf16_t*>(a.x);
  const bool plain_a = !a.scale && !a.se && a.act == T3D_ACT_NONE;

  constexpr int dyV = dyB / 8, aV = aB / 8;
  constexpr int ndv = STEP * dyV, nav = STEP * aV;
  constexpr int VDY = (ndv + 255) / 256, VA = (nav + 255) / 256;
  constexpr int NU = DGF ? (STEP / 16) * NTQ : 1, UPW = (NU + 3) / 4;
  struct Epi { bf16x4 res[UPW], xr[UPW]; };
  struct NoMask {};
  struct Regs { bf16x8 rz[VDY], ry[VDY], rx[VA]; Epi e; NoMask okm; };
  Regs rr[D];
  Epi ecur;
  const int lgq = lane >> 4, lcq = lane & 15;
  const bf16_t* __restrict__ eres = reinterpret_cast<const bf16_t*>(a.e_res);
  const bf16_t* __restrict__ eyr = reinterpret_cast<const bf16_t*>(a.e_y);

  auto gload = [&](Regs& R, int m0) {
#pragma unroll
    for (int i = 0; i < VDY; ++i) {
      const int v = min(tid + 256 * i, ndv - 1);
      const int row = v / dyV, m = min(m0 + row, a.M - 1);
      if constexpr (YF) {
        const int n = dy0 + (v % dyV) * 8;
        const bool fromz = n < a.Nz;
        const bf16_t* src = fromz ? dz + (size_t)m * a.Nz + n : xx + (size_t)m * a.K + min(max(n - a.Nz, 0), a.K - 8);
        R.rz[i] = *reinterpret_cast<const bf16x8*>(src);
      } else {
        const int n = min(dy0 + (v % dyV) * 8, a.N - 8);
        R.rz[i] = *reinterpret_cast<const bf16x8*>(dz + (size_t)m * a.N + n);
        R.ry[i] = *reinterpret_cast<const bf16x8*>(yy + (size_t)m * a.N + n);
      }
    }
#pragma unroll
    for (int i = 0; i < VA; ++i) {
      const int v = min(tid + 256 * i, nav - 1);
      const int row = v / aV, k = min(a0c + (v % aV) * 8, a.K - 8), m = min(m0 + row, a.M - 1);
      R.rx[i] = *reinterpret_cast<const bf16x8*>(xx + (size_t)m * a.K + k);
    }
    if constexpr (DGF) {
#pragma unroll
      for (int i = 0; i < UPW; ++i) {
        const int un = min(wave + 4 * i, NU - 1), pt = un / NTQ, kt = un % NTQ;
        const size_t o = (size_t)min(m0 + pt * 16 + lcq, a.M - 1) * a.K + min(kt * 16 + 4 * lgq, a.K - 4);
        if (eres) R.e.res[i] = *reinterpret_cast<const bf16x4*>(eres + o);
        if (eyr) R.e.xr[i] = *reinterpret_cast<const bf16x4*>(eyr + o);
      }
    }
  };
  auto ld8 = [](const float* p, float* o) {
    const float4 q0 = *reinterpret_cast<const float4*>(p), q1 = *reinterpret_cast<const float4*>(p + 4);
    o[0] = q0.x; o[1] = q0.y; o[2] = q0.z; o[3] = q0.w; o[4] = q1.x; o[5] = q1.y; o[6] = q1.z; o[7] = q1.w;
  };
  bf16x8 zero8;
#pragma unroll
  for (int j = 0; j < 8; ++j) zero8[j] = (bf16_t)0.f;
  auto lstore = [&](const Regs& R, int m0, int buf) {
    const auto& rz = R.rz; const auto& ry = R.ry; const auto& rx = R.rx;
    bf16_t* const pb_ = tiles + buf * BUFE;
    bf16_t* const qb_ = pb_ + STEP * RSP;
    bf16_t* dyt = SWAP ? qb_ : pb_;
    bf16_t* at = SWAP ? pb_ : qb_;
    constexpr int rsd = SWAP ? RSQ : RSP, rsa = SWAP ? RSP : RSQ;
#pragma unroll
    for (int i = 0; i < VDY; ++i) {
      const int v = tid + 256 * i;
      if (v < ndv) {
        const int row = v / dyV, cl = (v % dyV) * 8, m = m0 + row;
        const bool ok = m < mend && dy0 + cl < a.N;
        bf16x8 o;
        if constexpr (YF) {
          const int n = dy0 + cl;
          o = rz[i];
          if (n >= a.Nz + a.K) {
            o = zero8;
            if (n == a.Nz + a.K) o[0] = (bf16_t)1.f;
          }
          *reinterpret_cast<bf16x8*>(dyt + row * rsd + cl) = ok ? o : zero8;
          continue;
        }
        float al[8], be[8], ga[8];
        ld8(cdy + dyB + cl, be);
        if constexpr (GEN == 1) {
          if (a.per_sample) {
            const size_t pb = (size_t)(min(m, a.M - 1) / a.HW) * a.N + min(dy0 + cl, a.N - 8);
#pragma unroll
            for (int j = 0; j < 8; ++j) { al[j] = a.alpha[pb + j]; ga[j] = a.gamma[pb + j]; }
          } else {
            ld8(cdy + cl, al);
            ld8(cdy + 2 * dyB + cl, ga);
          }
        } else {
          ld8(cdy + cl, al);
          ld8(cdy + 2 * dyB + cl, ga);
        }
#pragma unroll
        for (int j = 0; j < 8; ++j) o[j] = (bf16_t)fmaf(al[j], (float)rz[i][j], fmaf(be[j], (float)ry[i][j], ga[j]));
        *reinterpret_cast<bf16x8*>(dyt + row * rsd + cl) = ok ? o : zero8;
      }
    }
#pragma unroll
    for (int i = 0; i < VA; ++i) {
      const int v = tid + 256 * i;
      if (v < nav) {
        const int row = v / aV, cl = (v % aV) * 8, m = m0 + row;
        const bool ok = m < mend && a0c + cl < a.K;
        bf16x8 o = rx[i];
        if (!plain_a) {
          float u[8], sc[8], sh[8];
          ld8(ca + cl, sc);
          ld8(ca + aB + cl, sh);
#pragma unroll
          for (int j = 0; j < 8; ++j) u[j] = (float)rx[i][j];
          bool done = false;
          if constexpr (GEN == 2) {
            float svv[8];
            const int rel = min(m, mend - 1) - gs_b0 * a.HW;
            ld8(gsl + (int)__umulhi((unsigned)rel, a.mulHW) * aB + cl, svv);
            if (a.se_after) {
              act_affine_vec<8>(u, sc, sh, a.act);
#pragma unroll
              for (int j = 0; j < 8; ++j) u[j] *= svv[j];
            } else {
#pragma unroll
              for (int j = 0; j < 8; ++j) u[j] = fmaf(u[j], sc[j], sh[j]) * svv[j];
              act_vec8(u, a.act);
            }
            done = true;
          }
          if constexpr (GEN == 1) {
            if (a.se) {
              float svv[8];
              {
                const float* se = a.se + (size_t)(min(m, a.M - 1) / a.HW) * a.K + min(a0c + cl, a.K - 8);
#pragma unroll
                for (int j = 0; j < 8; ++j) svv[j] = se[j];
              }
#pragma unroll
              for (int j = 0; j < 8; ++j) {
                float t = fmaf(u[j], sc[j], sh[j]);
                const float sv = svv[j];
                if (!a.se_after) t *= sv;
                t = act_apply(t, a.act);
                if (a.se_after) t *= sv;
                u[j] = t;
              }
              done = true;
            }
          }
          if (c6) {
#pragma unroll
            for (int j = 0; j < 8; j += 2) {
              const f32x2 t = pk_fma_clamp01(f32x2{u[j], u[j + 1]}, f32x2{sc[j], sc[j + 1]}, f32x2{sh[j], sh[j + 1]});
              u[j] = t[0];
              u[j + 1] = t[1];
            }
          } else if (!done) act_affine_vec<8>(u, sc, sh, a.act);
#pragma unroll
          for (int j = 0; j < 8; ++j) o[j] = (bf16_t)u[j];
        }
        *reinterpret_cast<bf16x8*>(at + row * rsa + cl) = ok ? o : zero8;
      }
    }
  };

  f32x4 acc[NTPW][NTQ];
#pragma unroll
  for (int i = 0; i < NTPW; ++i)
#pragma unroll
    for (int j = 0; j < NTQ; ++j) acc[i][j] = f32x4{0.f, 0.f, 0.f, 0.f};
  float st1[UPW][4], st2[UPW][4];
#pragma unroll
  for (int i = 0; i < UPW; ++i)
#pragma unroll
    for (int r = 0; r < 4; ++r) st1[i][r] = st2[i][r] = 0.f;
  auto dgrad_step = [&](const bf16_t* pcur, int m0) {
    bf16_t* __restrict__ dxo = reinterpret_cast<bf16_t*>(a.dx);
#pragma unroll
    for (int i = 0; i < UPW; ++i) {
      const int un = wave + 4 * i;
      if (un < NU) {
        const int pt = un / NTQ, kt = un % NTQ;
        f32x4 d = {0.f, 0.f, 0.f, 0.f};
#pragma unroll
        for (int js = 0; js < PB / 32; ++js) {
          const bf16x8 af = *reinterpret_cast<const bf16x8*>(wdl + (kt * 16 + lcq) * RSW + js * 32 + 8 * lgq);
          const bf16x8 bfr = *reinterpret_cast<const bf16x8*>(pcur + (pt * 16 + lcq) * RSP + js * 32 + 8 * lgq);
          d = __builtin_amdgcn_mfma_f32_16x16x32_bf16(af, bfr, d, 0, 0, 0);
        }
        const int m = m0 + pt * 16 + lcq, k = kt * 16 + 4 * lgq;
        const bool ok = m < mend && k < a.K;
        float v[4] = {d[0], d[1], d[2], d[3]}, yv[4] = {0.f, 0.f, 0.f, 0.f};
        if (eres) {
#pragma unroll
          for (int r = 0; r < 4; ++r) v[r] += (float)ecur.res[i][r];
        }
        bf16x4 o;
#pragma unroll
        for (int r = 0; r < 4; ++r) {
          o[r] = (bf16_t)v[r];
          v[r] = ok ? (float)o[r] : 0.f;
        }
        if (ok) *reinterpret_cast<bf16x4*>(dxo + (size_t)m * a.K + k) = o;
        if (a.stats) {
#pragma unroll
          for (int r = 0; r < 4; ++r) {
            if (eyr) yv[r] = (float)ecur.xr[i][r];
            st1[i][r] += v[r];
            st2[i][r] = fmaf(v[r], eyr ? yv[r] : v[r], st2[i][r]);
          }
        }
      }
    }
  };

  __syncthreads();
  const int nsteps = (mend - mbeg + STEP - 1) / STEP;
  const int niter = (nsteps + G - 1) / G;
  auto step_m = [&](int it) { return mbeg + (it * G + grp) * STEP; };
#pragma unroll
  for (int u = 0; u < D; ++u) gload(rr[u], step_m(u));
  lstore(rr[0], step_m(0), 0);
  if constexpr (DGF) ecur = rr[0].e;
  __syncthreads();
  int buf = 0;
  for (int it0 = 0; it0 < niter; it0 += D) {
#pragma unroll
    for (int u = 0; u < D; ++u) {
      const int it = it0 + u;
      if (it < niter) {
        gload(rr[u], step_m(it + D));
        const bf16_t* pcur = tiles + buf * BUFE;
        const bf16_t* qcur = pcur + STEP * RSP;
#pragma unroll
        for (int kk = 0; kk < SK; ++kk) {
          bf16x8 qf[NTQ];
#pragma unroll
          for (int j = 0; j < NTQ; ++j) qf[j] = tr_frag(qcur + kk * 32 * RSQ, RSQ, j * 16, lane);
#pragma unroll
          for (int i = 0; i < NTPW; ++i) {
            const bf16x8 pf = tr_frag(pcur + kk * 32 * RSP, RSP, (wave + 4 * i) * 16, lane);
#pragma unroll
            for (int j = 0; j < NTQ; ++j) acc[i][j] = __builtin_amdgcn_mfma_f32_16x16x32_bf16(pf, qf[j], acc[i][j], 0, 0, 0);
          }
        }
        if constexpr (DGF) {
          dgrad_step(pcur, step_m(it));
          ecur = rr[(u + 1) % D].e;
        }
        lstore(rr[(u + 1) % D], step_m(it + 1), buf ^ 1);
        __syncthreads();
        buf ^= 1;
      }
    }
  }

  if constexpr (DGF) {
    if (a.stats) {
#pragma unroll
      for (int i = 0; i < UPW; ++i) {
        const int un = wave + 4 * i;
#pragma unroll
        for (int r = 0; r < 4; ++r) {
          const float s1 = row16_sum(st1[i][r]), s2 = row16_sum(st2[i][r]);
          const int k = (un % NTQ) * 16 + 4 * lgq + r;
          if (un < NU && lcq == 0 && k < a.K) {
            atomicAdd(dstat + 2 * k, (double)s1);
            atomicAdd(dstat + 2 * k + 1, (double)s2);
          }
        }
      }
      __syncthreads();
      for (int i = threadIdx.x; i < 2 * a.K; i += 256 * G)
        atomicAdd(a.stats + (size_t)(blockIdx.x % a.nrep) * a.rstride + (size_t)(i & 1) * a.K + (i >> 1), dstat[i]);
      __syncthreads();
    }
  }
  if constexpr (G == 2) {
    f32x4* ex = reinterpret_cast<f32x4*>(smem);
#pragma unroll
    for (int i = 0; i < NTPW; ++i) {
      if (grp == 1) {
#pragma unroll
        for (int j = 0; j < NTQ; ++j) ex[(tid * NTQ) + j] = acc[i][j];
      }
      __syncthreads();
      if (grp == 0) {
#pragma unroll
        for (int j = 0; j < NTQ; ++j) acc[i][j] += ex[(tid * NTQ) + j];
      }
      __syncthreads();
    }
    if (grp == 1) return;
  }

  if (c6) {
#pragma unroll
    for (int i = 0; i < NTPW; ++i)
#pragma unroll
      for (int j = 0; j < NTQ; ++j) acc[i][j] = acc[i][j] * 6.f;
  }
  const int lg = lane >> 4, lc = lane & 15;
  if (a.ws) {
    float* wsb = a.ws + ((size_t)split * ntiles + tile) * (PB * QB);
#pragma unroll
    for (int i = 0; i < NTPW; ++i)
#pragma unroll
      for (int j = 0; j < NTQ; ++j)
#pragma unroll
        for (int r = 0; r < 4; ++r)
          wsb[((wave + 4 * i) * 16 + lg * 4 + r) * QB + j * 16 + lc] = acc[i][j][r];
    return;
  }
#pragma unroll
  for (int i = 0; i < NTPW; ++i)
#pragma unroll
    for (int j = 0; j < NTQ; ++j)
#pragma unroll
      for (int r = 0; r < 4; ++r) {
        const int p = p0 + (wave + 4 * i) * 16 + lg * 4 + r, q = q0 + j * 16 + lc;
        if (p < P && q < Q) {
          const int n = SWAP ? q : p, k = SWAP ? p : q;
          unsafeAtomicAdd(a.dw + (size_t)n * a.K + k, acc[i][j][r]);
        }
      }
}

template <int SP>
__global__ __launch_bounds__(256) void wgrad_reduce_kernel(const float* __restrict__ ws, float* __restrict__ dw, int N, int K,
                                                           int PB, int QB, int qtiles, int tiles, int S, int assign) {
  constexpr int EL = 256 / SP;
  __shared__ float red[SP][EL];
  const int Qpad = qtiles * QB;
  const int el = threadIdx.x % EL, sp = threadIdx.x / EL;
  const int e = blockIdx.x * EL + el;
  const int p = e / Qpad, q = e % Qpad;
  const bool live = p < N && q < K;
  float s = 0.f;
  if (live) {
    const float* src = ws + (size_t)((p / PB) * qtiles + q / QB) * (PB * QB) + (size_t)(p % PB) * QB + q % QB;
    const size_t stride = (size_t)tiles * PB * QB;
#pragma unroll 8
    for (int i = sp; i < S; i += SP) s += src[(size_t)i * stride];
  }
  if (SP > 1) {
    red[sp][el] = s;
    __syncthreads();
    if (sp == 0) {
#pragma unroll
      for (int j = 1; j < SP; ++j) s += red[j][el];
    }
  }
  if (sp == 0 && live) dw[(size_t)p * K + q] = assign ? s : dw[(size_t)p * K + q] + s;
}

template <int SG>
__global__ __launch_bounds__(256) void wgrad_reduce_tr_kernel(const float* __restrict__ ws, float* __restrict__ dw, int N, int K,
                                                               int PB, int QB, int qtiles, int tiles, int S, int assign) {
  constexpr int PT = 8 / SG;
  __shared__ float part[8][33];
  const int Qpad = qtiles * QB, nq = (Qpad + 31) / 32;
  const int p0 = (blockIdx.x / nq) * PT, q0 = (blockIdx.x % nq) * 32;
  const int tx = threadIdx.x & 31, rest = threadIdx.x >> 5, sg = rest / PT, pl = rest % PT;
  const size_t stride = (size_t)tiles * PB * QB;
  const int q = q0 + tx, p = p0 + pl;
  float s = 0.f;
  if (p < K && q < N) {
    const float* src = ws + (size_t)((p / PB) * qtiles + q / QB) * (PB * QB) + (size_t)(p % PB) * QB + q % QB;
#pragma unroll 8
    for (int i = sg; i < S; i += SG) s += src[(size_t)i * stride];
  }
  part[rest][tx] = s;
  __syncthreads();
  if (threadIdx.x < 32 * PT) {
    const int pl2 = threadIdx.x % PT, ql = threadIdx.x / PT;
    const int k = p0 + pl2, n = q0 + ql;
    if (k < K && n < N) {
      float t = part[pl2][ql];
#pragma unroll
      for (int g = 1; g < SG; ++g) t += part[g * PT + pl2][ql];
      dw[(size_t)n * K + k] = assign ? t : dw[(size_t)n * K + k] + t;
    }
  }
}

template <int NTPW, int NTQ, bool SWAP, int D, int GEN, bool YF = false, int SK = 1>
int launch_d(WgtArgs& a, hipStream_t st) {
  constexpr int G = 2;
  constexpr int STEP = 32 * SK;
  constexpr int PB = 64 * NTPW, QB = 16 * NTQ;
  const int P = a.swap ? a.K : a.N, Q = a.swap ? a.N : a.K;
  a.ptiles = cdiv(P, PB);
  a.qtiles = cdiv(Q, QB);
  const int tiles = a.ptiles * a.qtiles;
  const int dyB = a.swap ? QB : PB, aB = a.swap ? PB : QB;
  size_t lds = (size_t)G * 2 * STEP * ((PB + 8) + (QB + 8)) * 2 + (size_t)(3 * dyB + 2 * aB) * 4;
  const int tgt_blocks = 256;
  const long long cap_mb = 8;
  int S = (tgt_blocks + tiles - 1) / tiles;
  const long long tile_bytes = (long long)tiles * PB * QB * 4;
  const bool use_ws = g_t3d_ws.ptr && g_t3d_ws.bytes >= tile_bytes;
  if (use_ws) {
    const long long fit = g_t3d_ws.bytes / tile_bytes;
    if (S > fit) S = (int)fit;
  } else {
    const long long flush_cap = (cap_mb << 20) / ((long long)a.N * a.K * 4 + 1);
    if (S > flush_cap) S = (int)(flush_cap < 1 ? 1 : flush_cap);
  }
  const int maxs = cdiv(a.M, STEP * 4 * G);
  if (S > maxs) S = maxs;
  if (S < 1) S = 1;
  a.rows_per_split = cdiv(cdiv(a.M, S), STEP) * STEP;
  S = cdiv(a.M, a.rows_per_split);
  a.gs_ns = 0;
  if constexpr (GEN == 2) {
    const long long ns = a.rows_per_split / a.HW + 2, span = (long long)a.rows_per_split + a.HW;
    if (!a.se || a.per_sample || a.HW < 2 || ns * aB * 4 > 32 * 1024 || span * a.HW >= (1ll << 32)) return launch_d<NTPW, NTQ, SWAP, 1, 1>(a, st);
    a.gs_ns = (int)ns;
    a.mulHW = (unsigned)(((1ull << 32) + a.HW - 1) / a.HW);
    lds = ((lds + 15) & ~(size_t)15) + (size_t)ns * aB * 4;
  }
  a.ws = use_ws ? reinterpret_cast<float*>(g_t3d_ws.ptr) : nullptr;
  if (a.assign && !use_ws && hipMemsetAsync(a.dw, 0, (size_t)a.N * a.K * sizeof(float), st) != hipSuccess) return T3D_ERR_LAUNCH;
  if (lds > 64 * 1024)
    (void)t3d_max_lds((const void*)pw_wgrad_tr_kernel<NTPW, NTQ, SWAP, G, D, GEN, YF, SK, false>, (int)lds);
  a.nsplit = S;
  T3D_LAUNCH_TIMED((pw_wgrad_tr_kernel<NTPW, NTQ, SWAP, G, D, GEN, YF, SK, false>), dim3(tiles * S), dim3(256 * G), lds, st, a);
  if (use_ws) {
#define T3D_WGR(SPV)                                                                                                              \
  do {                                                                                                                            \
    if (SWAP)                                                                                                                     \
      T3D_LAUNCH(wgrad_reduce_tr_kernel<(SPV == 16 ? 8 : SPV)>, dim3(cdiv(a.K, 8 / (SPV == 16 ? 8 : SPV)) * cdiv(a.qtiles * QB, 32)), dim3(256), 0, st, \
                         a.ws, a.dw, a.N, a.K, PB, QB, a.qtiles, tiles, S, a.assign);                                             \
    else                                                                                                                          \
      T3D_LAUNCH(wgrad_reduce_kernel<SPV>, dim3(cdiv(a.N * a.qtiles * QB, 256 / SPV)), dim3(256), 0, st, a.ws, a.dw, a.N, \
                         a.K, PB, QB, a.qtiles, tiles, S, a.assign);                                                              \
  } while (0)
    if (S >= 64) T3D_WGR(16);
    else if (S >= 8) T3D_WGR(4);
    else T3D_WGR(1);
#undef T3D_WGR
  }
  T3D_CHECK_LAUNCH();
  return T3D_OK;
}

template <int NTPW, int NTQ, bool SWAP>
int launch_sw(WgtArgs& a, hipStream_t st) {
  constexpr bool narrow = 64 * NTPW + 16 * NTQ <= 288;
  const bool sk2 = narrow && a.M >= (1 << 20);
  if (a.yfree) {
    if constexpr (SWAP) return T3D_ERR_ARG;
    else {
      if constexpr (narrow)
        if (sk2) return launch_d<NTPW, NTQ, false, 2, false, true, 2>(a, st);
      return launch_d<NTPW, NTQ, false, 2, false, true>(a, st);
    }
  }
  if (a.per_sample) return launch_d<NTPW, NTQ, SWAP, 1, 1>(a, st);
  if (a.se) return launch_d<NTPW, NTQ, SWAP, 2, 2>(a, st);
  if constexpr (narrow)
    if (sk2) return launch_d<NTPW, NTQ, SWAP, 2, false, false, 2>(a, st);
  return launch_d<NTPW, NTQ, SWAP, 2, false>(a, st);
}

template <int NTPW, int NTQ>
int launch_cfg(WgtArgs& a, hipStream_t st) {
  return a.swap ? launch_sw<NTPW, NTQ, true>(a, st) : launch_sw<NTPW, NTQ, false>(a, st);
}

static int choose_and_launch(WgtArgs& a, hipStream_t st) {
  const int M = a.M, K = a.K, N = a.N;
  a.swap = K > N;
  const int P = a.swap ? K : N, Q = a.swap ? N : K;
  const int min_steps = 12;
  auto steps_with = [&](int ntpw, int qb) {
    const int tiles = cdiv(P, 64 * ntpw) * cdiv(Q, qb);
    int S = cdiv(256, tiles);
    if (S < 1) S = 1;
    return M / (S * 2 * 32);
  };
  if (Q <= 16) return (P <= 64 || steps_with(2, 16) < min_steps) ? launch_cfg<1, 1>(a, st) : launch_cfg<2, 1>(a, st);
  if (Q <= 32) {
    if (P <= 64 || steps_with(3, 32) < min_steps) return launch_cfg<1, 2>(a, st);
    return P <= 128 ? launch_cfg<2, 2>(a, st) : launch_cfg<3, 2>(a, st);
  }
  if (Q <= 64) {
    if (P > 192 && steps_with(6, 64) >= min_steps && a.yfree) return launch_cfg<6, 4>(a, st);
    if (P > 64 && steps_with(3, 64) >= min_steps) return launch_cfg<3, 4>(a, st);
    return launch_cfg<1, 4>(a, st);
  }
  if (Q <= 96) return (P > 64 && steps_with(3, 96) >= 5) ? launch_cfg<3, 6>(a, st) : launch_cfg<1, 6>(a, st);
  if (Q <= 112) return (P > 64 && steps_with(3, 112) >= 8) ? launch_cfg<3, 7>(a, st) : launch_cfg<1, 7>(a, st);
  if (Q % 128 == 0) return (P > 64 && steps_with(3, 128) >= min_steps) ? launch_cfg<3, 8>(a, st) : launch_cfg<1, 8>(a, st);
  return (P > 64 && steps_with(3, 160) >= min_steps) ? launch_cfg<3, 10>(a, st) : launch_cfg<1, 10>(a, st);
}

}

int t3d_pw_wgrad_reduce(const float* ws, float* dw, int N, int K, int PB, int QB, int qtiles, int tiles, int S, hipStream_t st) {
  const int blocks = [&](int sp) { return cdiv(N * qtiles * QB, 256 / sp); }(S >= 64 ? 16 : (S >= 8 ? 4 : 1));
  if (S >= 64) T3D_LAUNCH(wgrad_reduce_kernel<16>, dim3(blocks), dim3(256), 0, st, ws, dw, N, K, PB, QB, qtiles, tiles, S, 0);
  else if (S >= 8) T3D_LAUNCH(wgrad_reduce_kernel<4>, dim3(blocks), dim3(256), 0, st, ws, dw, N, K, PB, QB, qtiles, tiles, S, 0);
  else T3D_LAUNCH(wgrad_reduce_kernel<1>, dim3(blocks), dim3(256), 0, st, ws, dw, N, K, PB, QB, qtiles, tiles, S, 0);
  T3D_CHECK_LAUNCH();
  return T3D_OK;
}

bool t3d_pw::tr_can(const PwCall& c) { return c.dtype == T3D_BF16 && c.op == PW_WGRAD; }

int t3d_pw::tr_launch(const PwCall& c, const void* dz, const void* y, const t3d_bnbwd* bb, const void* x, const t3d_prologue* pro,
                      float* dw, hipStream_t st) {
  if (!tr_can(c)) return T3D_ERR_ARG;
  WgtArgs a{};
  a.dz = dz; a.y = y; a.x = x;
  a.alpha = bb->alpha; a.beta = bb->beta; a.gamma = bb->gamma; a.per_sample = bb->per_sample;
  if (pro) { a.scale = pro->scale; a.shift = pro->shift; a.se = pro->se; a.act = pro->act; a.se_after = pro->se_after_act; }
  a.dw = dw; a.M = c.M; a.HW = c.HW; a.K = c.Nout; a.N = c.Kin;
  a.fold = a.per_sample ? nullptr : t3d_take_fold(a.alpha);
  return choose_and_launch(a, st);
}

struct YfCfg { int ntpw, ntq, sk, S, rows_per_split, PB, QB; };
static bool yf_cfg(int M, int K, int N, YfCfg& c) {
  const int P = N + K + 8;
  if (K > 32 || P > 256 || P <= 64) return false;
  c.ntq = K <= 16 ? 1 : 2;
  c.ntpw = P <= 128 ? 2 : (P <= 192 ? 3 : 4);
  c.sk = M >= (1 << 20) ? 2 : 1;
  c.PB = 64 * c.ntpw; c.QB = 16 * c.ntq;
  const int step = 32 * c.sk;
  int S = 256;
  const int maxs = cdiv(M, step * 4 * 2);
  if (S > maxs) S = maxs;
  if (S < 1) S = 1;
  c.rows_per_split = cdiv(cdiv(M, S), step) * step;
  c.S = cdiv(M, c.rows_per_split);
  return true;
}

template <int NTPW, int NTQ, int SK>
static int launch_fused(WgtArgs& a, const YfCfg& c, hipStream_t st) {
  constexpr int G = 2, STEP = 32 * SK, PB = 64 * NTPW, QB = 16 * NTQ;
  a.ptiles = a.qtiles = 1;
  a.rows_per_split = c.rows_per_split;
  a.nsplit = c.S;
  const int ncoef = 3 * PB + 2 * QB;
  const size_t lds = (size_t)G * 2 * STEP * ((PB + 8) + (QB + 8)) * 2 + (size_t)((ncoef + 3) & ~3) * 4 + (size_t)QB * (PB + 8) * 2 +
                     (size_t)2 * QB * sizeof(double);
  const void* fn = (const void*)pw_wgrad_tr_kernel<NTPW, NTQ, false, G, 2, false, true, SK, true>;
  if (lds > 64 * 1024) (void)t3d_max_lds(fn, (int)lds);
  T3D_LAUNCH_TIMED((pw_wgrad_tr_kernel<NTPW, NTQ, false, G, 2, false, true, SK, true>), dim3(c.S), dim3(256 * G), lds, st, a);
  T3D_CHECK_LAUNCH();
  return T3D_OK;
}

size_t t3d_pw_bwd_yfree_scratch(int M, int K, int N) {
  YfCfg c;
  if (!yf_cfg(M, K, N, c)) return 0;
  return (size_t)c.S * c.PB * c.QB * 4 + (((size_t)(N + K + 8) * K * 4 + 255) & ~(size_t)255);
}

int t3d_pw_bwd_yfree_launch(const void* dz, const void* x, const void* wd, const void* wt, const t3d_bnbwd* bb, const void* x_raw,
                            const void* residual, void* dx, double* stats, void* scratch, int M, int HW, int K, int N, hipStream_t st) {
  YfCfg c;
  if (!yf_cfg(M, K, N, c)) return T3D_ERR_UNSUPPORTED;
  WgtArgs a{};
  a.dz = dz; a.x = x; a.y = dz;
  if (!wd) {
    a.wtr = reinterpret_cast<const bf16_t*>(wt);
    a.alpha = bb->alpha; a.beta = bb->beta; a.gamma = bb->gamma;
    a.fold = t3d_take_fold(bb->alpha);
  }
  a.M = M; a.HW = HW; a.K = K;
  a.yfree = 1; a.Nz = N; a.N = N + K + 8;
  a.ws = reinterpret_cast<float*>(scratch);
  a.wd = reinterpret_cast<const bf16_t*>(wd);
  a.e_res = residual; a.e_y = x_raw; a.dx = dx; a.stats = stats;
  a.nrep = g_t3d_reduce.nrep; a.rstride = g_t3d_reduce.stats_stride;
  if (a.stats && a.nrep < 1) { a.nrep = 1; a.rstride = 0; }
#define T3D_YFL(P_, Q_, S_) return launch_fused<P_, Q_, S_>(a, c, st)
  if (c.ntpw == 2 && c.ntq == 1) { if (c.sk == 2) T3D_YFL(2, 1, 2); else T3D_YFL(2, 1, 1); }
  if (c.ntpw == 2 && c.ntq == 2) { if (c.sk == 2) T3D_YFL(2, 2, 2); else T3D_YFL(2, 2, 1); }
  if (c.ntpw == 3 && c.ntq == 1) { if (c.sk == 2) T3D_YFL(3, 1, 2); else T3D_YFL(3, 1, 1); }
  if (c.ntpw == 3 && c.ntq == 2) { if (c.sk == 2) T3D_YFL(3, 2, 2); else T3D_YFL(3, 2, 1); }
  if (c.ntpw == 4 && c.ntq == 2) { if (c.sk == 2) T3D_YFL(4, 2, 2); else T3D_YFL(4, 2, 1); }
  if (c.ntpw == 4 && c.ntq == 1) { if (c.sk == 2) T3D_YFL(4, 1, 2); else T3D_YFL(4, 1, 1); }
#undef T3D_YFL
  return T3D_ERR_UNSUPPORTED;
}

int t3d_pw_bwd_yfree_reduce(void* scratch, float** tmp_out, int M, int K, int N, hipStream_t st) {
  YfCfg c;
  if (!yf_cfg(M, K, N, c)) return T3D_ERR_UNSUPPORTED;
  float* ws = reinterpret_cast<float*>(scratch);
  float* tmp = ws + (size_t)c.S * c.PB * c.QB;
  const int rows = N + K + 8;
#define T3D_YFR(SPV) T3D_LAUNCH(wgrad_reduce_kernel<SPV>, dim3(cdiv(rows * c.QB, 256 / SPV)), dim3(256), 0, st, ws, tmp, rows, K, c.PB, c.QB, 1, 1, c.S, 1)
  if (c.S >= 64) T3D_YFR(16);
  else if (c.S >= 8) T3D_YFR(4);
  else T3D_YFR(1);
// ... 15 lines not shown
```

### 3d-object-detection.pytorch_amd/torchdet3d/_native.py

```python
import ctypes
import os

import torch

_HERE = os.path.dirname(os.path.abspath(__file__))
LIB_PATH = os.environ.get('T3D_LIB') or os.path.join(os.path.dirname(_HERE), 'libt3d_hip.so')

W_FRAG = 0x100
F32, BF16, F16 = 0, 1, 2
ACT = {'none': 0, 'relu': 1, 'relu6': 2, 'hswish': 3}
DW_AUTO, DW_TILE, DW_ROW3, DW_PLANE7, DW_ROWK, DW_LDS = -1, 0, 1, 2, 3, 4
PW_AUTO, PW_DEEP, PW_STREAM, PW_REG32, PW_LDS, PW_TR, PW_PAIR = -1, 0, 1, 2, 3, 4, 5
PW_OP_FWD, PW_OP_FWD_STATS, PW_OP_MAT, PW_OP_DGRAD, PW_OP_WGRAD = 0, 1, 2, 3, 4
ERR_ARG, ERR_UNSUPPORTED = -1, -3
POOL = {'avg': 0, 'max': 1, 'avg+max': 2}
_P, _I, _F, _D, _L = ctypes.c_void_p, ctypes.c_int, ctypes.c_float, ctypes.c_double, ctypes.c_longlong


class BnBwd(ctypes.Structure):
    _fields_ = [('alpha', _P), ('beta', _P), ('gamma', _P), ('per_sample', _I)]


class Prologue(ctypes.Structure):
    _fields_ = [('scale', _P), ('shift', _P), ('se', _P), ('act', _I), ('se_after_act', _I)]


class LossCfg(ctypes.Structure):
    _fields_ = [(n, _F) for n in ('c_l1', 'c_mse', 'c_smoothl1', 'smoothl1_beta', 'c_add', 'c_diag', 'c_wing',
                                  'wing_w', 'wing_eps', 'c_ce', 'lam_reg', 'lam_cls')]


class BnFold(ctypes.Structure):
    _fields_ = [('kind', _I), ('C', _I), ('nrep', _I), ('rstride', _L), ('stats', _P), ('count', _D), ('gamma', _P), ('beta', _P),
                ('rm', _P), ('rv', _P), ('nbt', _P), ('momentum', _F), ('eps', _F), ('o0', _P), ('o1', _P), ('o2', _P),
                ('o3', _P), ('o4', _P), ('mean', _P), ('invstd', _P)]


class DrawStyleC(ctypes.Structure):
    _fields_ = [('rect_th', _I), ('edge_th', _I), ('kp_radius', _I), ('font_scale', _I), ('flags', _I),
                ('colors', ctypes.c_ubyte * 3 * 8)]


DRAW_IDS = 1
_PP = ctypes.POINTER(Prologue)
_BP = ctypes.POINTER(BnBwd)
_LP = ctypes.POINTER(LossCfg)

_ARGTYPE = {'i': _I, 'l': _L, 'u': ctypes.c_ulonglong, 'f': _F, 'd': _D, 'p': _P,
            'P': _PP, 'B': _BP, 'L': _LP, 'S': ctypes.POINTER(DrawStyleC),
            'F': _P}


def _rows(fn, *outs):
    if fn.argtypes is None:
        fn.argtypes, fn.restype = [_I] + [ctypes.POINTER(type(o)) for o in outs], _I
    i = 0
    while fn(i, *[ctypes.byref(o) for o in outs]) == 0:
        yield tuple(o.value.decode() if isinstance(o, ctypes.c_char_p) else o.value for o in outs)
        i += 1


def abi_structs():
    return {name: (size, [(f, int(o), int(b)) for f, o, b in (x.split(':') for x in fields.split(','))])
            for name, size, fields in _rows(lib().t3d_abi_struct, ctypes.c_char_p(), _I(), ctypes.c_char_p())}


_lib = None


def lib():
    global _lib, SIGNATURES, STEP_ENTRIES
    if _lib is None:
        if not os.path.exists(LIB_PATH):
            raise RuntimeError(f'{LIB_PATH} not found: build it with `python __graft_entry__.py` '
                               '(there is no CPU fallback for the HIP path)')
        loaded = ctypes.CDLL(LIB_PATH)
        rows = list(_rows(loaded.t3d_abi_entry, ctypes.c_char_p(), ctypes.c_char_p(), _I()))
        SIGNATURES = dict((name, [_ARGTYPE[c] for c in types]) for name, types, _ in rows)
        STEP_ENTRIES = frozenset(name for name, _, in_step in rows if in_step)
        for name, args in SIGNATURES.items():
            fn = getattr(loaded, name)
            fn.argtypes = args
            fn.restype = _I
        _lib = loaded
    return _lib


def __getattr__(name):
    if name in ('SIGNATURES', 'STEP_ENTRIES'):
        lib()
        return globals()[name]
    raise AttributeError(f'module {__name__!r} has no attribute {name!r}')


def ptr(t):
    if t is None:
        return None
    assert t.is_cuda and t.is_contiguous(), 'native ops need contiguous device tensors'
    return t.data_ptr()


def dtype_code(t):
    if t.dtype == torch.float32:
# ... 13 lines not shown
        return _raw_stream(torch.cuda.current_device())
    return torch.cuda.current_stream().cuda_stream


class KernelTimer:

    def __init__(self, only=None, prealloc=0, kernel_exact=False):
        self.only, self.rec, self.sig, self.kernel_exact = only, [], [], kernel_exact
        self.pool = [torch.cuda.Event(enable_timing=True) for _ in range(prealloc)]
        for e in self.pool:
            e.record()

    def event(self):
        return self.pool.pop() if self.pool else torch.cuda.Event(enable_timing=True)

    def per_launch(self):
        torch.cuda.synchronize()
        return [(n, sg, e0.elapsed_time(e1), nb) for (n, nb, e0, e1), sg in zip(self.rec, self.sig)]

    def summary(self):
        torch.cuda.synchronize()
        out = {}
        for name, nbytes, e0, e1 in self.rec:
            d = out.setdefault(name, dict(launches=0, ms=0.0, bytes=0))
            d['launches'] += 1
            d['ms'] += e0.elapsed_time(e1)
            d['bytes'] += nbytes or 0
        return out


timer = None
_KERNEL_TIMED = frozenset(('t3d_dwconv_fwd', 't3d_dwconv_bwd', 't3d_expdw_fwd', 't3d_pwconv_fwd', 't3d_pwconv_fwd_mat', 't3d_pwconv_dgrad',
                           't3d_pwconv_wgrad', 't3d_pwconv_dgrad_yfree', 't3d_pwconv_wgrad_yfree', 't3d_pwconv_bwd_yfree',
                           't3d_pwconv_bwd_yfree_w'))
_ABLATE = frozenset(x for x in os.environ.get('T3D_ABLATE', '').split(',') if x)


SLOT_IMGS, SLOT_GT, SLOT_CATS, SLOT_DROPOUT, SLOT_STEP, SLOT_LR, SLOT_RB_DST, SLOT_RB_EVENT, NSLOTS = range(9)
recorder = None


def call(name, *args, nbytes=None, slots=None):
    if _ABLATE and name in _ABLATE:
        return
    fn = getattr(lib(), name)
    if recorder is not None:
        recorder.add_call(name, args, nbytes, slots)
        rc = fn(*args)
        recorder.after_call()
        if rc != 0:
            raise RuntimeError(f'{name} failed with code {rc}')
        return
    t = timer
    if t is not None and (t.only is None or name in t.only):
        e0, e1 = t.event(), t.event()
        if name in _KERNEL_TIMED and t.kernel_exact:
            lib().t3d_set_launch_events(e0.cuda_event, e1.cuda_event)
            rc = fn(*args)
            lib().t3d_set_launch_events(None, None)
        else:
            e0.record()
            rc = fn(*args)
            e1.record()
        t.rec.append((name, nbytes, e0, e1))
        t.sig.append(tuple(a for a in args[:-1] if isinstance(a, int) and not isinstance(a, bool) and 0 <= a < (1 << 31)))
    else:
        rc = fn(*args)
    if rc != 0:
        raise RuntimeError(f'{name} failed with code {rc}')


def launch_count():
    n = ctypes.c_ulonglong(0)
    lib().t3d_launch_count(ctypes.byref(n), None)
    return n.value


def prologue(scale=None, shift=None, se=None, act='none', se_after_act=False):
    p = Prologue(ptr(scale), ptr(shift), ptr(se), ACT[act] if isinstance(act, str) else act, int(se_after_act))
    p._keep = (scale, shift, se)
    return p


def bnbwd(alpha, beta, gamma, per_sample=False):
    b = BnBwd(ptr(alpha), ptr(beta), ptr(gamma), int(per_sample))
    b._keep = (alpha, beta, gamma)
    return b


_U64 = (1 << 64) - 1


def _word(argtype, v):
    import struct
    if argtype is _F:
        return struct.unpack('<I', struct.pack('<f', float(v)))[0]
    if argtype is _D:
        return struct.unpack('<Q', struct.pack('<d', float(v)))[0]
    if v is None:
        return 0
    return int(v) & _U64


def double_bits(x):
    import struct
    return struct.unpack('<Q', struct.pack('<d', float(x)))[0]


HANDOFF = os.environ.get('T3D_PLAN_HANDOFF', '1') != '0'


class PlanRecorder:

    def __init__(self, ptr_slots=None):
        self.plan = _P()
        rc = lib().t3d_plan_create(ctypes.byref(self.plan))
        if rc != 0:
            raise RuntimeError(f't3d_plan_create failed with code {rc}')
        self.ptr_slots = dict(ptr_slots or {})
        self.calls = []
        self.keep = []
        self.breaks = []
        n = ctypes.c_ulonglong(0)
        lib().t3d_launch_count(ctypes.byref(n), None)
        self.launches, self.last_on = n.value, {}
        self.broken = None

    def add_call(self, name, args, nbytes, slots):
        types = SIGNATURES[name]
        n = len(types)
        if len(args) != n:
            raise RuntimeError(f'{name}: {len(args)} arguments for a {n}-argument entry point')
        kinds, words, sizes = (_I * n)(), (ctypes.c_ulonglong * n)(), (_I * n)()
        for i, (t, v) in enumerate(zip(types, args)):
            if slots and i in slots:
                kinds[i], words[i] = 2, slots[i]
            elif isinstance(v, ctypes.Structure):
                kinds[i], words[i], sizes[i] = 1, ctypes.addressof(v), ctypes.sizeof(v)
                self.keep.append(getattr(v, '_keep', None))
            elif t is _P and v is not None and int(v) in self.ptr_slots:
                kinds[i], words[i] = 2, self.ptr_slots[int(v)]
            elif t in (_PP, _BP, _LP):
                if v is not None:
                    raise RuntimeError(f'{name}: argument {i} is not a ctypes structure')
                kinds[i], words[i] = 0, 0
            else:
                kinds[i], words[i] = 0, _word(t, v)
        rc = lib().t3d_plan_add_call(self.plan, name.encode(), n, kinds, words, sizes)
        if rc != 0:
            raise RuntimeError(f't3d_plan_add_call({name}) failed with code {rc}')
        self.calls.append((name, tuple(a for a in args[:-1] if isinstance(a, int) and not isinstance(a, bool) and 0 <= a < (1 << 31)),
                           nbytes))

    def after_call(self):
        n, st = ctypes.c_ulonglong(0), _P()
        lib().t3d_launch_count(ctypes.byref(n), ctypes.byref(st))
        if n.value != self.launches:
            self.launches = n.value
            self.last_on[st.value or 0] = lib().t3d_plan_num_ops(self.plan, -1) - 1

    def add_fork(self, from_stream, to_stream):
        prod = self.last_on.get(from_stream or 0) if HANDOFF else None
        if prod is not None:
            rc = lib().t3d_plan_add_fork_after(self.plan, prod, from_stream, to_stream)
        else:
            rc = lib().t3d_plan_add_fork(self.plan, from_stream, to_stream)
        if rc != 0:
            raise RuntimeError(f't3d_plan_add_fork failed with code {rc}')

# ... 24 lines not shown
```

### 3d-object-detection.pytorch_amd/torchdet3d/models/engine.py

```python
import contextlib
import math
import os

import torch

from .. import _native as N
from .arch import Arch

BN_EPS, BN_MOM = 1e-5, 0.1
NREP = 16
FUSED_EVAL_MIN_B = int(os.environ.get('T3D_FUSED_EVAL_MIN_B', '96'))
DW_SLOTS = 512
WORKSPACE_BYTES = 64 << 20
MAIN_WORKSPACE_BYTES = 16 << 20
YFREE_MIN_ELEMS = int(os.environ.get('T3D_YFREE_MIN', 8 << 20))
YFREE_MAX_K = 112
HOOK_MIN = 1 << 20
SE_AFTER_FUSED = None


def _se_after_fused_by_shape(dt, B, HW, C, R):
    if B < 8:
        return False
    if C * R <= 4096:
        return True
    return B >= 16 and B * HW >= 1024


class _BN:
    __slots__ = ('name', 'C', 'gamma', 'beta', 'dgamma', 'dbeta', 'rm', 'rv', 'nbt', 'stats', 'bstats', 'scale',
                 'shift', 'mean', 'invstd', 'alpha', 'bbeta', 'gammac', 'count', 'pro_cache', 'pend', 'desc', 'nrep')


def _nrep_for(C):
    return 16 if C <= 160 else (8 if C <= 640 else 4)


def _concurrent_stream(device, tries=8):
    main = torch.cuda.current_stream(device)
    cands = []
    with torch.cuda.device(device):
        probe = torch.zeros(1, device=device)
        for _ in range(tries):
            st = torch.cuda.Stream(device=device, priority=0)
            cands.append(st)
            e0, e_side, e_main = (torch.cuda.Event(enable_timing=True) for _ in range(3))
            torch.cuda.synchronize(device)
            e0.record(main)
            torch.cuda._sleep(4_000_000)
            e_main.record(main)
            with torch.cuda.stream(st):
                probe.add_(1.0)
                e_side.record(st)
            torch.cuda.synchronize(device)
            ratio = e0.elapsed_time(e_side) / max(e0.elapsed_time(e_main), 1e-6)
            _concurrent_stream.log.append(round(ratio, 3))
            if ratio < 0.5:
                return st
    return cands[0]


_concurrent_stream.log = []


class _Src:
    __slots__ = ('t', 'pro', 'B', 'H', 'W', 'C', 'raw', 'bn', 'gpro', 'finished_act', 'dz', 'zres', 'zbuf')

    def __init__(self, t, pro, B, H, W, C, raw=None, bn=None, gpro=None, finished_act=False):
        self.t, self.pro, self.B, self.H, self.W, self.C = t, pro, B, H, W, C
        self.raw, self.bn, self.gpro, self.finished_act = raw, bn, gpro, finished_act
        self.dz = None
        self.zres = self.zbuf = None


class Net:
    def __init__(self, name, num_classes=9, device='cuda', dtype=torch.float32, pooling_mode='avg', share=None):
        if pooling_mode not in N.POOL:
            raise ValueError(f'Unknown pooling mode: {pooling_mode}')
        self.pooling_mode, self.pool = pooling_mode, N.POOL[pooling_mode]
        self.arch = Arch(name)
        self.name, self.num_classes = name, num_classes
        self.feat_gain = 1.0
        if self.arch.head == 'conv_bias':
            self.pool = N.POOL['avg']
            self.feat_gain = 2.0 if pooling_mode == 'avg+max' else 1.0
        self.device = torch.device(device)
        assert dtype in (torch.float32, torch.bfloat16, torch.float16)
        self.dtype = dtype
        self.dt = {torch.float32: N.F32, torch.bfloat16: N.BF16, torch.float16: N.F16}[dtype]
        self.esz = 4 if dtype == torch.float32 else 2
        self._share = share
        self._layout()
        self._bufs = {}
        self._packed_dirty = True
        self._packed_version = -1
        self._pack_desc = self._se_pack_desc = None
        self._evdesc = None
        self._dwarena = self._zero_rows = None
        self._zgroups = {'fwd': {}, 'bwd': {}}
        self._zcovered = {'fwd': frozenset(), 'bwd': frozenset()}
        self._zgdesc, self._zdescs = {}, {}
        self._want_taps = None
        self._stop_after = None
        self._tap_res = {}
        self._dropout_calls = 0
        self.seed_rank = 0
        self.saved = None
        self.generation = 0
        self.grad_hook = None
        self._cur_pool_exact = False
        self._side = None
        if self.device.type == 'cuda' and not os.environ.get('T3D_NO_SIDE_STREAM'):
            self._side = _concurrent_stream(self.device)
        self._side_busy = False
        self.persistent_outputs = False
        self.set_input_normalization([0.5931, 0.4690, 0.4229], [0.2471, 0.2214, 0.2157])
        self._fused_eval = True

    def set_input_normalization(self, mean, std):
        self.in_mean = torch.tensor(mean, dtype=torch.float32, device=self.device)
        self.in_istd = 1.0 / torch.tensor(std, dtype=torch.float32, device=self.device)

    def _layout(self):
        a = self.arch
        shapes = a.param_shapes(self.num_classes)
        self.shapes = shapes
        order = [k for k, (s, kind) in shapes.items() if kind == 'param' and not k.startswith('regressors.')]
        off, self.offsets = 0, {}
        for k in order:
            n = int(math.prod(shapes[k][0]))
            self.offsets[k] = (off, n)
            off += (n + 3) // 4 * 4
        F = a.feat_c
        self.offsets['__wreg'] = (off, 9 * 18 * F)
        off += 9 * 18 * F
        self.offsets['__breg'] = (off, 9 * 18 + 2)
        off += 164
        for k in range(9):
            self.offsets[f'regressors.{k}.0.weight'] = (self.offsets['__wreg'][0] + k * 18 * F, 18 * F)
            self.offsets[f'regressors.{k}.0.bias'] = (self.offsets['__breg'][0] + k * 18, 18)
        self.nparams = off
        dev = self.device
        sh = self._share
        assert sh is None or (sh.nparams == off and sh.name == self.name and sh.device == dev)
        self.flat = sh.flat if sh is not None else torch.zeros(off, device=dev)
        self.gflat = sh.gflat if sh is not None else torch.zeros(off, device=dev)
        self.p, self.g = {}, {}
        for k, (s, kind) in shapes.items():
            if kind == 'param':
                o, n = self.offsets[k]
                self.p[k] = self.flat[o:o + n].view(s)
                self.g[k] = self.gflat[o:o + n].view(s)
        self.wreg, self.breg = self._view('__wreg', (9, 18, F)), self._view('__breg', (9, 18), 162)
        self.dwreg = self._view('__wreg', (9, 18, F), g=True)
        self.dbreg = self._view('__breg', (9, 18), 162, g=True)
        self.buffers = {}
        self.bns = {}
        for k, (s, kind) in shapes.items():
            if kind == 'buffer':
                self.buffers[k] = sh.buffers[k] if sh is not None else (
                    torch.zeros(s, device=dev, dtype=torch.int64) if k.endswith('tracked')
                    else (torch.ones(s, device=dev) if k.endswith('var') else torch.zeros(s, device=dev)))
        nbn = [k[:-len('.running_mean')] for k in shapes if k.endswith('.running_mean')]
        tot = sum(shapes[k + '.weight'][0][0] for k in nbn)
        self._statbuf = torch.zeros(NREP, 4 * tot, device=dev, dtype=torch.float64)
        self._stat_stride = 4 * tot
        self._aff = torch.zeros(7 * tot, device=dev)
        o = 0
        for k in nbn:
            C = shapes[k + '.weight'][0][0]
            b = _BN()
            b.name, b.C = k, C
            b.gamma, b.beta = self.p[k + '.weight'], self.p[k + '.bias']
            b.dgamma, b.dbeta = self.g[k + '.weight'], self.g[k + '.bias']
            b.rm, b.rv, b.nbt = self.buffers[k + '.running_mean'], self.buffers[k + '.running_var'], \
                self.buffers[k + '.num_batches_tracked']
            b.stats = self._statbuf[0, 2 * o:2 * o + 2 * C]
            b.bstats = self._statbuf[0, 2 * tot + 2 * o:2 * tot + 2 * o + 2 * C]
            sl = [self._aff[i * tot + o:i * tot + o + C] for i in range(7)]
            b.scale, b.shift, b.mean, b.invstd, b.alpha, b.bbeta, b.gammac = sl
            b.pro_cache = {}
            self.bns[k] = b
            o += C
        self._bn_total = tot
        for b in self.bns.values():
            b.pend = [False, False]
            b.desc = {}
            b.nrep = _nrep_for(b.C)
        self._cur_nrep = None
        if sh is None:
            self.reset_parameters()

    def nonfinite(self):
        return not bool(torch.isfinite(self._aff).all())

    def _view(self, key, shape, n=None, g=False):
        o, m = self.offsets[key]
        return (self.gflat if g else self.flat)[o:o + (n or m)].view(shape)

    @torch.no_grad()
# ... 709 lines not shown
    def backward(self, dkp, dlogits=None):
        with self._pass(main_scratch=True, workspace=True):
            return self._backward(dkp, dlogits)

    def _clear_backward(self):
        if self._dwarena is None:
            self._dw_arena_init()
        dw32 = self._buf('dstem32', (self.arch.stem_c, 32), torch.float32)
        if self._zero_rows is None:
            rows = [[t.data_ptr(), t.numel() * t.element_size()] for t in (self.gflat, dw32) if t.numel()]
            rows += [[v.data_ptr(), NREP * self.p[k].numel() * 4] for k, v in self._dwviews.items()]
            assert all(r[1] % 16 == 0 for r in rows)
            self._zero_rows = rows
        self._zero_group('bwd', self._zero_rows)
        return dw32

    def _backward(self, dkp, dlogits=None):
        sv = self.saved
        assert sv is not None and 'tap_order' not in sv, 'backward() needs a preceding forward(train=True)'
        a, st, dt, B = self.arch, N.stream(), self.dt, sv['B']
        dw32 = self._clear_backward()
        self._dwpending, self._dwflushed, self._hook_hi = 0, 0, self.gflat.numel()
        dkp = dkp.reshape(B, 18).to(torch.float32).contiguous()
        ncls = self.num_classes
        if ncls > 1:
            assert dlogits is not None
            dlogits = dlogits.to(torch.float32).contiguous()
        else:
            dlogits = None
        F = a.feat_c
        dpre = self._buf('dpre', (B, 18), torch.float32)
        df = self._buf('df', (B, F), torch.float32)
        bnc = self.bns[a.keys.head_bn] if a.head == 'linear_bn' else None
        hstat = None
        if a.head == 'conv_bias':
            hstat = self._buf('head_stats', (2 * F,), torch.float64, zgroup='bwd')
            self._replicas(1)
        N.call('t3d_head_bwd', N.ptr(sv['f']), sv['fpro'], N.ptr(sv['cats']), N.ptr(self.wreg),
               N.ptr(self.p['cls_fc.1.weight']), N.ptr(sv['mask']), N.ptr(sv['kp']), N.ptr(dkp), N.ptr(dlogits),
               N.ptr(dpre), N.ptr(df), self._bst(bnc) if bnc else (N.ptr(hstat) if sv['fpro'] is not None else None),
               None, None, None, None, B, F, ncls, st)
        self._wgrad(N.ptr(sv['f']), sv['fpro'], N.ptr(sv['cats']), N.ptr(sv['mask']), N.ptr(dpre), N.ptr(dlogits),
                    N.ptr(self.dwreg), N.ptr(self.dbreg), N.ptr(self.g['cls_fc.1.weight']), N.ptr(self.g['cls_fc.1.bias']),
                    B, F, ncls, entry='t3d_head_bwd_weights')
        dpooled = df
        if a.head == 'conv_bias':
            yc, pooled, Fc = sv['head_u'], sv['pooled'], a.classifier
            if sv['fpro'] is None:
                du = self._buf('dhead_u', (B, Fc), torch.float32)
                N.call('t3d_bn_act_bwd', N.F32, N.ptr(df), N.ptr(yc), sv['head_pro'], N.ptr(du), N.ptr(hstat), B, Fc, st)
                df = du
            gain, zeros = self._const(Fc, self.feat_gain), self._const(Fc, 0.0)
            bb = N.bnbwd(gain, zeros, zeros, False)
            self._wgrad(N.F32, N.ptr(df), N.ptr(yc), bb, N.ptr(pooled), None, N.ptr(self.g[a.keys.head_w]), B, 1, a.last_c, Fc)
            N.call('t3d_bn_bias_grad', N.ptr(hstat), N.ptr(hstat), Fc, float(B), N.ptr(gain), N.ptr(zeros), N.ptr(zeros),
                   N.ptr(self.g[a.keys.head_b]), st)
            dpooled = self._buf('dpooled', (B, a.last_c), torch.float32)
            N.call('t3d_pwconv_dgrad', N.F32, N.ptr(df), N.ptr(yc), bb, N.ptr(self.wt['classifier']), None, None,
                   None, N.ptr(dpooled), None, None, B, 1, a.last_c, Fc, st)
        elif a.head == 'linear_bn':
            bb = self._bn_bwd(bnc)
            self._settle_b(bnc)
            yc, pooled = sv['f'], sv['pooled']
            self._wgrad(N.F32, N.ptr(df), N.ptr(yc), bb, N.ptr(pooled), None,
                        N.ptr(self.g[a.keys.head_w]), B, 1, a.last_c, a.classifier)
            N.call('t3d_bn_bias_grad', N.ptr(bnc.stats), self._bst(bnc), a.classifier, float(B), N.ptr(bnc.alpha),
                   N.ptr(bnc.bbeta), N.ptr(bnc.gammac), N.ptr(self.g[a.keys.head_b]), st)
            dpooled = self._buf('dpooled', (B, a.last_c), torch.float32)
            N.call('t3d_pwconv_dgrad', N.F32, N.ptr(df), N.ptr(yc), bb, N.ptr(self.wt['classifier']), None, None,
                   None, N.ptr(dpooled), None, None, B, 1, a.last_c, a.classifier, st)
        self._backward_backbone(sv, dpooled, dw32)
        self._flush_dw()
        self._join_side()
        self._maybe_hook(0, force=True)
        assert not any(b.pend[1] for b in self.bns.values()), 'a BatchNorm backward finalize was never run'
        self.saved = None

    def _backward_backbone(self, sv, dpooled, dw32):
        a, st, dt, B = self.arch, N.stream(), self.dt, sv['B']
        lw = a.keys.last_w
        bnl = self.bns[a.keys.last_bn]
        x = sv['last_in']
        M, HW = B * sv['HWl'], sv['HWl']
        dzl = self._buf('dz:last', (M, a.last_c))
        N.call('t3d_pool_bwd', dt, N.ptr(dpooled), N.ptr(sv['yl']), sv['prol'], self.pool, N.ptr(sv['pool_argmax']),
               N.ptr(dzl), self._bst(bnl), B, HW, a.last_c, st)
        bb = self._bn_bwd(bnl)
        def last_wgrad():
            self._wgrad(dt, N.ptr(dzl), N.ptr(sv['yl']), bb, N.ptr(x.t), x.pro,
                        N.ptr(self.g[lw]), M, HW, x.C, a.last_c, nbytes=M * (x.C + a.last_c) * self.esz,
                        ro=bnl)
        last_wgrad()
        dz = self._pw_dgrad(dzl, sv['yl'], bb, self.wt[lw], x, None, M, HW, x.C, a.last_c, 'dz:lastin', bnl)

        self._maybe_hook(self.offsets[lw][0])
        for rec in reversed(sv['blocks']):
            dz = self._block_bwd(rec, dz)
            self._maybe_hook(self.offsets[a.keys.blocks[rec['idx']].first][0])

        self._stem_wgrad(sv, dz, dw32)

    def _stem_wgrad(self, sv, dz, dw32):
        a, st, dt = self.arch, N.stream(), self.dt
        s0 = sv['stem']
        bn0 = s0.bn
        bb = self._bn_bwd(bn0)
        self._settle_b(bn0)
        M = s0.B * s0.H * s0.W
        self._wgrad(dt, N.ptr(dz), N.ptr(s0.raw), bb, N.ptr(sv['col']), None, N.ptr(dw32),
                    M, s0.H * s0.W, 32, a.stem_c, nbytes=M * (32 + a.stem_c) * self.esz)
        self._flush_dw()
        self._join_side()
        N.call('t3d_copy_cols', N.ptr(dw32), N.ptr(self.g[a.keys.stem_w]), a.stem_c, 32, 27, st)

    def _pw_dgrad(self, dz, y, bb, wt, x, residual, M, HW, K, Nn, tag, bn=None):
        dx = self._buf(tag, (M, K))
        with_stats = x.bn is not None and not x.finished_act
        wd, wp = self._wsel(wt, not bb.per_sample and not (with_stats and x.gpro is not None and x.gpro.se))
        self._c('t3d_pwconv_dgrad', wd, N.ptr(dz), N.ptr(y), bb, wp,
                N.ptr(x.raw) if with_stats else None, x.gpro if with_stats else None,
                N.ptr(residual) if residual is not None else None, N.ptr(dx),
                self._bst(x.bn) if with_stats else None, None, M, HW, K, Nn, N.stream(),
                nbytes=M * (K + Nn) * self.esz, bwd=bn)
        if x.finished_act:
            dx = self._act_bwd(dx, x, tag + ':a')
        return dx

    def _dw_arena_init(self):
        names = [k for k, (sh, kind) in self.shapes.items() if kind == 'param' and len(sh) == 4 and sh[1] == 1 and sh[2] > 1]
        tot = sum(DW_SLOTS * self.p[k].numel() for k in names)
        self._dwarena = torch.zeros(tot, device=self.device, dtype=torch.float32)
        self._dwused = torch.zeros(max(len(names), 1), device=self.device, dtype=torch.int32)
        self._dwviews, self._dwidx, off = {}, {}, 0
        for k in names:
            n = self.p[k].numel()
            self._dwviews[k] = self._dwarena[off:off + DW_SLOTS * n]
            off += DW_SLOTS * n
        self._dworder = list(reversed(names))
        rows = []
        for i, k in enumerate(self._dworder):
            self._dwidx[k] = i
            rows.append([self._dwviews[k].data_ptr(), self.g[k].data_ptr(), self.p[k].numel(), self._dwused[i:i + 1].data_ptr()])
        self._dwdesc = torch.tensor(rows, dtype=torch.int64, device=self.device) if rows else None

    def _dw_replicas(self, name):
        assert self._dworder[self._dwflushed + self._dwpending] == name
        self._dwpending += 1
        i = self._dwidx[name]
        N.call('t3d_set_dw_slots', DW_SLOTS, N.ptr(self._dwused[i:i + 1]))
        return self._dwviews[name]

    def _flush_dw(self):
        if not self._dwpending:
            return
        N.call('t3d_sum_slots_batched', self._dwdesc[self._dwflushed:].data_ptr(), self._dwpending, N.stream())
        self._dwflushed += self._dwpending
        self._dwpending = 0

    def _maybe_hook(self, lo, force=False):
        if self.grad_hook is None:
            return
        if force or self._hook_hi - lo >= HOOK_MIN:
            self._flush_dw()
            if self._side is not None and not force:
                self._fork_side()
                self._hook(lo, True)
                self._side_busy = True
            else:
                self._join_side()
                self._hook(lo, False)
            self._hook_hi = lo

    def _hook(self, lo, on_side):
        if N.recorder is not None:
            N.recorder.host_break(('hook', lo, on_side))
        if on_side:
            with torch.cuda.stream(self._side):
                self.grad_hook(lo)
        else:
            self.grad_hook(lo)

    def _se_after_fused(self, B, HW, C, R):
        if self.arch.keys.scheme != 'timm' or C > 1024 or R > 1024:
# ... 158 lines not shown
```

### include/t3d.h

```cpp
#ifndef T3D_H_
#define T3D_H_
#include <stdint.h>
#ifdef __cplusplus
extern "C" {
#endif

enum { T3D_F32 = 0, T3D_BF16 = 1, T3D_F16 = 2 };
enum { T3D_W_FRAG = 0x100 };
enum { T3D_ACT_NONE = 0, T3D_ACT_RELU = 1, T3D_ACT_RELU6 = 2, T3D_ACT_HSWISH = 3 };
enum { T3D_OK = 0, T3D_ERR_ARG = -1, T3D_ERR_LAUNCH = -2, T3D_ERR_UNSUPPORTED = -3 };

typedef struct {
  const float* scale;
  const float* shift;
  const float* se;
  int act;
  int se_after_act;
} t3d_prologue;

int t3d_version(void);

int t3d_dwconv_fwd(int dtype, const void* x, const t3d_prologue* pro, const float* w, void* y,
                   double* stats, float* gap_sum, int B, int H, int W, int C, int k, int stride,
                   void* stream);

int t3d_bn_finalize(const double* stats, int C, double count, const float* gamma, const float* beta,
                    float* running_mean, float* running_var, int64_t* num_batches_tracked,
                    float momentum, float eps, float* scale, float* shift, float* mean, float* invstd,
                    void* stream);

int t3d_bn_eval_affine(int C, const float* gamma, const float* beta, const float* running_mean,
                       const float* running_var, float eps, float* scale, float* shift, void* stream);

int t3d_bn_eval_affine_batched(const long long* desc, int n, float eps, void* stream);

typedef struct {
  const float* alpha;
  const float* beta;
  const float* gamma;
  int per_sample;
} t3d_bnbwd;

int t3d_pwconv_fwd(int dtype, const void* x, const t3d_prologue* pro, const void* w, const float* bias,
                   void* y, double* stats, int M, int HW, int K, int N, void* stream);

int t3d_pwconv_frag_bytes(int rows, int cols);
int t3d_pwconv_wants_frag(int K, int N);
int t3d_pwconv_pack_frag(const void* w, void* out, int rows, int cols, void* stream);

int t3d_pwconv_dgrad(int dtype, const void* dz, const void* y, const t3d_bnbwd* bb, const void* wt,
                     const void* x_raw, const t3d_prologue* pro_in, const void* residual, void* dx,
                     double* stats, float* ps_stats, int M, int HW, int K, int N, void* stream);

int t3d_pack_weight(int dtype, const float* w, void* out, int rows, int cols, int transpose, void* stream);

int t3d_pwconv_wgrad(int dtype, const void* dz, const void* y, const t3d_bnbwd* bb, const void* x,
                     const t3d_prologue* pro, float* dw, int M, int HW, int K, int N, void* stream);

enum { T3D_PW_AUTO = -1, T3D_PW_DEEP = 0, T3D_PW_STREAM = 1, T3D_PW_REG32 = 2, T3D_PW_LDS = 3, T3D_PW_TR = 4, T3D_PW_PAIR = 5 };
enum { T3D_PW_OP_FWD = 0, T3D_PW_OP_FWD_STATS = 1, T3D_PW_OP_MAT = 2, T3D_PW_OP_DGRAD = 3, T3D_PW_OP_WGRAD = 4 };
int t3d_pwconv_route(int op, int dtype, int gated, int per_sample, int ps_stats, int e_se, int bias, int stats, int alpha_gamma,
                     int act, int residual, int M, int HW, int K, int N);
int t3d_pwconv_force_route(int route);

int t3d_pwconv_yfree_prep(const void* wt, const t3d_bnbwd* bb, void* wcat, float* cvec, int K, int N, void* stream);
int t3d_pwconv_dgrad_yfree(const void* dz, const void* x, const void* wcat, const float* cvec, const void* x_raw,
                           const t3d_prologue* pro_in, const void* residual, void* dx, double* stats, int M, int HW,
                           int K, int N, void* stream);
int t3d_pwconv_wgrad_yfree(const void* dz, const void* x, const t3d_bnbwd* bb, const void* w, float* dw, int M, int HW,
                           int K, int N, void* stream);

int t3d_pwconv_yfree_prep2(const void* wt, const t3d_bnbwd* bb, void* wcat, float* cvec, void* wd, int K, int N, void* stream);
int t3d_pwconv_bwd_yfree_w(const void* dz, const void* x, const void* wt, const t3d_bnbwd* bb, const void* x_raw,
                           const t3d_prologue* pro_in, const void* residual, void* dx, double* stats, void* scratch,
                           long long scratch_bytes, int M, int HW, int K, int N, void* stream);
int t3d_pwconv_bwd_yfree_scratch(int M, int K, int N);
int t3d_pwconv_bwd_yfree(const void* dz, const void* x, const void* wd, const void* x_raw, const t3d_prologue* pro_in,
                         const void* residual, void* dx, double* stats, void* scratch, long long scratch_bytes, int M, int HW,
                         int K, int N, void* stream);
int t3d_pwconv_wgrad_yfree_finish(void* scratch, const t3d_bnbwd* bb, const void* w, float* dw, int M, int K, int N, void* stream);

int t3d_dwconv_bwd(int dtype, const void* dz, const void* y, const t3d_bnbwd* bb, const float* w,
                   const void* x, const t3d_prologue* pro, const void* residual, void* dx, double* stats,
                   float* dw, int B, int H, int W, int C, int k, int stride, void* stream);

enum { T3D_DW_AUTO = -1, T3D_DW_TILE = 0, T3D_DW_ROW3 = 1, T3D_DW_PLANE7 = 2, T3D_DW_ROWK = 3, T3D_DW_LDS = 4 };
int t3d_dwconv_route(int backward, int dtype, int gated_input, int pooled, int B, int H, int W, int C, int k, int stride);
int t3d_dwconv_plan(int backward, int dtype, int gated_input, int pooled, int B, int H, int W, int C, int k, int stride,
                    int* out);
int t3d_dwconv_force_route(int route);

int t3d_bn_bwd_finalize(const double* stats, int C, double count, const float* gamma, const float* mean,
                        const float* invstd, float* alpha, float* beta, float* gammac, float* dgamma,
                        float* dbeta, void* stream);

int t3d_stem_im2col(int dtype, const float* x, void* col, int B, int H, int W, void* stream);
int t3d_stem_im2col_u8(int dtype, const unsigned char* x, const float* mean, const float* inv_std, void* col, int B, int H,
                       int W, void* stream);

int t3d_ir_block_eval(const void* x, const void* w1, const float* scale1, const float* shift1, int act1, const float* wdw,
                      const float* scale2, const float* shift2, int act2, const void* w2, const float* scale3,
                      const float* shift3, int residual, void* z, int B, int H, int W, int Cin, int Ce, int Cout, void* stream);

int t3d_crop_resize_u8(const unsigned char* frame, const int* rects, unsigned char* out, int n, int H, int W, int oh, int ow,
                       void* stream);

enum { T3D_AUG_FLIP = 1, T3D_AUG_LUT = 2, T3D_AUG_ROTATE = 4, T3D_AUG_SWAP_RB = 8 };
typedef struct {
  long long offset;
  int h, w;
  int flags;
  float alpha;
  float beta255;
  int reserved;
  double m[6];
} t3d_aug_sample;
int t3d_augment_crops_u8(const unsigned char* src, long long src_bytes, const void* samples, unsigned char* out, int B, int oh,
                         int ow, void* stream);

int t3d_augment_resized_u8(const unsigned char* arena, long long arena_bytes, const void* samples, unsigned char* out, int B,
                           int oh, int ow, void* stream);

enum { T3D_CHAIN_LUT = 1, T3D_CHAIN_HSV = 2, T3D_CHAIN_BRIGHTNESS = 3, T3D_CHAIN_CONTRAST = 4, T3D_CHAIN_SATURATION = 5,
// ... 352 lines not shown
```

Baseline: 39110 crops/s.

## Fuse global-average-pool backward into last pointwise conv dgrad and wgrad

When the head uses plain average pooling in bf16, the last layer's dz is no longer written out. The pool backward kernel now only accumulates BN statistics. The pointwise dgrad (deep and stream paths) and the transposed wgrad kernels rebuild dz on the fly from the pooled gradient, the activation output and the prologue affine, which removes a large M×C write and two reads. The GAP forward also folds BN finalize in-kernel instead of calling the fold fallback. The cost is more per-element arithmetic and LDS in the GEMM kernels, plus extra template variants and routing checks.

```diff
diff --git a/3d-object-detection.pytorch_amd/csrc/abi.hip b/3d-object-detection.pytorch_amd/csrc/abi.hip
--- a/3d-object-detection.pytorch_amd/csrc/abi.hip
+++ b/3d-object-detection.pytorch_amd/csrc/abi.hip
@@ -78,7 +78,7 @@
   constexpr Text text = describe(fields);                \
   }
 T3D_STRUCT(t3d_prologue, F(scale) F(shift) F(se) F(act) F(se_after_act))
-T3D_STRUCT(t3d_bnbwd, F(alpha) F(beta) F(gamma) F(per_sample))
+T3D_STRUCT(t3d_bnbwd, F(alpha) F(beta) F(gamma) F(per_sample) F(pool_act) F(pooled) F(pool_scale) F(pool_shift))
 T3D_STRUCT(t3d_aug_sample, F(offset) F(h) F(w) F(flags) F(alpha) F(beta255) F(reserved) F(m))
 T3D_STRUCT(t3d_aug_chain, F(n_ops) F(flags) F(kind) F(p) F(m2))
 T3D_STRUCT(t3d_det_sample, F(offset) F(h) F(w) F(turns) F(left) F(top) F(cx0) F(cy0) F(cx1) F(cy1) F(flags) F(delta) F(alpha)
diff --git a/3d-object-detection.pytorch_amd/csrc/elementwise.hip b/3d-object-detection.pytorch_amd/csrc/elementwise.hip
--- a/3d-object-detection.pytorch_amd/csrc/elementwise.hip
+++ b/3d-object-detection.pytorch_amd/csrc/elementwise.hip
@@ -283,7 +283,15 @@
   const T* __restrict__ y = reinterpret_cast<const T*>(a.a);
   float sc[8], sh[8], acc[8], mx[8];
   int mi[8];
-  load_affine(a, c0, sc, sh);
+  if (a.fold) {
+    const int cb = blockIdx.y * rowl;
+    t3d_fold_block<1>(a.fold, cb, min(rowl, a.C - cb), red, rowl, blockIdx.x == 0);
+#pragma unroll
+    for (int i = 0; i < 8; ++i) { sc[i] = on ? red[cgl * 8 + i] : 1.f; sh[i] = on ? red[rowl + cgl * 8 + i] : 0.f; }
+    __syncthreads();
+  } else {
+    load_affine(a, c0, sc, sh);
+  }
 #pragma unroll
   for (int j = 0; j < 8; ++j) { acc[j] = 0.f; mx[j] = -INFINITY; mi[j] = 0; }
   if (on) {
@@ -364,7 +372,7 @@
           s1[j] += d[j];
           s2[j] = fmaf(d[j], v[j], s2[j]);
         }
-        Vec8<T>::store(dz + off, d);
+        if (dz) Vec8<T>::store(dz + off, d);
       }
     }
   }
@@ -517,7 +525,7 @@
   fill_pro(a, pro);
   dim3 grid(B, cdiv(C / 8, 32));
   hipStream_t st = reinterpret_cast<hipStream_t>(stream);
-  if (const int rc = t3d_fold_fallback(a.scale, st)) return rc;
+  a.fold = t3d_take_fold(a.scale);
   if (dtype == T3D_F32) T3D_LAUNCH(gap_fwd_kernel<float>, grid, dim3(256), 0, st, a);
   else if (dtype == T3D_BF16) T3D_LAUNCH(gap_fwd_kernel<bf16_t>, grid, dim3(256), 0, st, a);
   else if (dtype == T3D_F16) T3D_LAUNCH(gap_fwd_kernel<f16_t>, grid, dim3(256), 0, st, a);
@@ -533,8 +541,9 @@
 
 extern "C" int t3d_pool_bwd(int dtype, const float* dpooled, const void* y, const t3d_prologue* pro, int mode,
                             const int* argmax, void* dz, double* stats, int B, int HW, int C, void* stream) {
-  if (!dpooled || !y || !dz || B <= 0 || HW <= 0 || C <= 0 || (C % 8)) return T3D_ERR_ARG;
+  if (!dpooled || !y || B <= 0 || HW <= 0 || C <= 0 || (C % 8)) return T3D_ERR_ARG;
   if (mode != T3D_POOL_AVG && mode != T3D_POOL_MAX && mode != T3D_POOL_AVGMAX) return T3D_ERR_ARG;
+  if (!dz && (mode != T3D_POOL_AVG || !stats)) return T3D_ERR_ARG;
   if (mode != T3D_POOL_AVG && !argmax) return T3D_ERR_ARG;
   if (pro && pro->se) return T3D_ERR_UNSUPPORTED;
   EwArgs a{};
diff --git a/3d-object-detection.pytorch_amd/csrc/pwconv_common.h b/3d-object-detection.pytorch_amd/csrc/pwconv_common.h
--- a/3d-object-detection.pytorch_amd/csrc/pwconv_common.h
+++ b/3d-object-detection.pytorch_amd/csrc/pwconv_common.h
@@ -27,7 +27,9 @@
   const T3dFold* fold;
   const void* z_res;
   void* z_out;
-  int unused_[8];
+  const float *pool_g, *pool_scale, *pool_shift;
+  int pool_act;
+  float pool_inv_hw;
   int wfrag;
   T3dQuant quant;
 };
@@ -44,5 +46,14 @@
 }
 template <> __device__ __forceinline__ void stvec<bf16_t>(bf16_t* p, const float* v) { Vec8<bf16_t>::store(p, v); }
 
+__device__ __forceinline__ void pooled_dz8(const float* g, const float* y, const float* sc, const float* sh, int act, float inv_hw,
+                                           float* d) {
+#pragma unroll
+  for (int j = 0; j < 8; ++j) d[j] = g[j] * inv_hw + 0.f;
+  act_grad_affine_vec<8>(d, y, sc, sh, act);
+#pragma unroll
+  for (int j = 0; j < 8; ++j) d[j] = Vec8<bf16_t>::round(d[j]);
+}
+
 
 }
diff --git a/3d-object-detection.pytorch_amd/csrc/pwconv_deep.hip b/3d-object-detection.pytorch_amd/csrc/pwconv_deep.hip
--- a/3d-object-detection.pytorch_amd/csrc/pwconv_deep.hip
+++ b/3d-object-detection.pytorch_amd/csrc/pwconv_deep.hip
@@ -25,9 +25,9 @@
 constexpr int RT = 4;
 constexpr int NW = 8;
 
-template <bool DG, int NTW, int KSP>
-__global__ __launch_bounds__(64 * NW) void pw_deep_kernel(const GemmArgs a, const int KS, const int ntiles, const int nrep,
-                                                             const long long rstride) {
+template <bool DG, int NTW, int KSP, bool PG>
+__device__ __forceinline__ void pw_deep_body(const GemmArgs a, const int KS, const int ntiles, const int nrep, const long long rstride) {
+  static_assert(DG || !PG, "the pooled form is a data gradient");
   constexpr int IT = RT * KSP / NW;
   static_assert(IT >= 1 && IT * NW == RT * KSP, "staging items must divide over the waves");
   extern __shared__ __attribute__((aligned(16))) unsigned char smem[];
@@ -35,7 +35,7 @@
   const int kpad = KS * 32;
   float* coef = reinterpret_cast<float*>(smem + (size_t)2 * RT * KSP * 1024);
   const int BN = ntiles * 16;
-  float* ecoef = coef + 3 * kpad;
+  float* ecoef = coef + (PG ? 5 : 3) * kpad;
   double* dstat = reinterpret_cast<double*>(ecoef + 2 * BN);
 
   const int tid = threadIdx.x, lane = tid & 63, wave = tid >> 6;
@@ -73,17 +73,31 @@
   const size_t arow = (size_t)mrow * a.Kin + lg * 8;
   const bool rok = m0 + srt * 16 + lc < a.M;
   bf16x8 pa[2][IT], pb[DG ? 2 : 1][DG ? IT : 1];
+  f32x4 pg[PG ? IT : 1][2];
+  const float* __restrict__ grow = PG ? a.pool_g + (size_t)(mrow / a.HW) * a.Kin + lg * 8 : nullptr;
   auto a_issue = [&](auto slot_tag, const int ph) {
     constexpr int SL = decltype(slot_tag)::value;
 #pragma unroll
     for (int j = 0; j < IT; ++j) {
-      const size_t o = arow + min((ph * KSP + sks + j) * 32, a.Kin - 8 - lg * 8);
-      pa[SL][j] = *reinterpret_cast<const bf16x8*>(A0 + o);
+      const int ko = min((ph * KSP + sks + j) * 32, a.Kin - 8 - lg * 8);
+      const size_t o = arow + ko;
+      if (!PG) pa[SL][j] = *reinterpret_cast<const bf16x8*>(A0 + o);
       if (DG) pb[DG ? SL : 0][DG ? j : 0] = *reinterpret_cast<const bf16x8*>(A1 + o);
+    }
+  };
+  auto g_issue = [&](const int ph) {
+    if constexpr (PG) {
+#pragma unroll
+      for (int j = 0; j < IT; ++j) {
+        const int ko = min((ph * KSP + sks + j) * 32, a.Kin - 8 - lg * 8);
+        pg[j][0] = *reinterpret_cast<const f32x4*>(grow + ko);
+        pg[j][1] = *reinterpret_cast<const f32x4*>(grow + ko + 4);
+      }
     }
   };
   w_issue(std::integral_constant<int, 0>{}, 0);
   a_issue(std::integral_constant<int, 0>{}, 0);
+  g_issue(0);
   a_issue(std::integral_constant<int, 1>{}, 1);
 
   for (int i = tid; i < BN * 2; i += 64 * NW) dstat[i] = 0.0;
@@ -92,6 +106,13 @@
     const bool v = DG && a.e_scale && n < a.Nout;
     ecoef[i] = v ? a.e_scale[n] : 1.f;
     ecoef[BN + i] = v ? a.e_shift[n] : 0.f;
+  }
+  if constexpr (PG) {
+    for (int i = tid; i < kpad; i += 64 * NW) {
+      const bool v = i < a.Kin && a.pool_scale;
+      coef[3 * kpad + i] = v ? a.pool_scale[i] : 1.f;
+      coef[4 * kpad + i] = v ? a.pool_shift[i] : 0.f;
+    }
   }
   if (a.fold) {
     for (int i = a.Kin + tid; i < kpad; i += 64 * NW) {
@@ -140,8 +161,20 @@
       const float c0[8] = {c0a.x, c0a.y, c0a.z, c0a.w, c0b.x, c0b.y, c0b.z, c0b.w};
       const float c1[8] = {c1a.x, c1a.y, c1a.z, c1a.w, c1b.x, c1b.y, c1b.z, c1b.w};
       float x[8];
-#pragma unroll
-      for (int e = 0; e < 8; ++e) x[e] = (float)pa[SL][j][e];
+      if constexpr (PG) {
+        const float4 sa = *reinterpret_cast<const float4*>(coef + 3 * kpad + kc), sb = *reinterpret_cast<const float4*>(coef + 3 * kpad + kc + 4);
+        const float4 ha = *reinterpret_cast<const float4*>(coef + 4 * kpad + kc), hb = *reinterpret_cast<const float4*>(coef + 4 * kpad + kc + 4);
+        const float ps[8] = {sa.x, sa.y, sa.z, sa.w, sb.x, sb.y, sb.z, sb.w}, ph_[8] = {ha.x, ha.y, ha.z, ha.w, hb.x, hb.y, hb.z, hb.w};
+        const f32x4 g0 = pg[PG ? j : 0][0], g1 = pg[PG ? j : 0][1];
+        const float g[8] = {g0[0], g0[1], g0[2], g0[3], g1[0], g1[1], g1[2], g1[3]};
+        float yv[8];
+#pragma unroll
+        for (int e = 0; e < 8; ++e) yv[e] = (float)pb[DG ? SL : 0][DG ? j : 0][e];
+        pooled_dz8(g, yv, ps, ph_, a.pool_act, a.pool_inv_hw, x);
+      } else {
+#pragma unroll
+        for (int e = 0; e < 8; ++e) x[e] = (float)pa[SL][j][e];
+      }
       if (!DG) {
         if (fact == -1) {
 #pragma unroll
@@ -169,6 +202,7 @@
     if (ph == 0) DEEP_STAMP(2);
     __builtin_amdgcn_sched_barrier(0);
     w_issue(std::integral_constant<int, 1 - SL>{}, ph + 1);
+    g_issue(ph + 1);
     a_issue(std::integral_constant<int, SL>{}, ph + 2);
     __builtin_amdgcn_sched_barrier(0);
 #pragma unroll
@@ -275,17 +309,37 @@
   DEEP_STAMP(5);
 }
 
-size_t deep_lds(int KS, int ntiles, int KSP = 4) { return (size_t)2 * RT * KSP * 1024 + (size_t)3 * KS * 32 * 4 + (size_t)ntiles * 16 * (2 * 4 + 2 * 8); }
-
 template <bool DG, int NTW, int KSP>
+__global__ __launch_bounds__(64 * NW) void pw_deep_kernel(const GemmArgs a, const int KS, const int ntiles, const int nrep,
+                                                             const long long rstride) {
+  pw_deep_body<DG, NTW, KSP, false>(a, KS, ntiles, nrep, rstride);
+}
+
+template <int NTW, int KSP>
+__global__ __launch_bounds__(64 * NW) void pw_deep_pooled_kernel(const GemmArgs a, const int KS, const int ntiles, const int nrep,
+                                                                    const long long rstride) {
+  pw_deep_body<true, NTW, KSP, true>(a, KS, ntiles, nrep, rstride);
+}
+
+size_t deep_lds(int KS, int ntiles, int KSP = 4, int rows = 3) {
+  return (size_t)2 * RT * KSP * 1024 + (size_t)rows * KS * 32 * 4 + (size_t)ntiles * 16 * (2 * 4 + 2 * 8);
+}
+
+template <bool DG, int NTW, int KSP, bool PG = false>
 int launch_deep(GemmArgs& a, int KS, int ntiles, int nchunks, hipStream_t st) {
-  const size_t lds = deep_lds(KS, ntiles, KSP);
-  const void* fn = (const void*)pw_deep_kernel<DG, NTW, KSP>;
+  const size_t lds = deep_lds(KS, ntiles, KSP, PG ? 5 : 3);
+  const void* fn;
+  if constexpr (PG) fn = (const void*)pw_deep_pooled_kernel<NTW, KSP>;
+  else fn = (const void*)pw_deep_kernel<DG, NTW, KSP>;
   if (lds > 64 * 1024) (void)t3d_max_lds(fn, (int)lds);
   a.quant = (!DG && a.stats && !T3D_ENV_SET("T3D_NO_SNAP")) ? t3d_quant_for(a.M) : T3dQuant{0.0, 0.0};
   a.fold = t3d_take_fold(a.p0);
-  T3D_LAUNCH_TIMED((pw_deep_kernel<DG, NTW, KSP>), dim3(cdiv(a.M, 16 * RT), nchunks), dim3(64 * NW), lds, st, a, KS, ntiles,
-                     g_t3d_reduce.nrep, g_t3d_reduce.stats_stride);
+  if constexpr (PG)
+    T3D_LAUNCH_TIMED((pw_deep_pooled_kernel<NTW, KSP>), dim3(cdiv(a.M, 16 * RT), nchunks), dim3(64 * NW), lds, st, a, KS, ntiles,
+                       g_t3d_reduce.nrep, g_t3d_reduce.stats_stride);
+  else
+    T3D_LAUNCH_TIMED((pw_deep_kernel<DG, NTW, KSP>), dim3(cdiv(a.M, 16 * RT), nchunks), dim3(64 * NW), lds, st, a, KS, ntiles,
+                       g_t3d_reduce.nrep, g_t3d_reduce.stats_stride);
   T3D_CHECK_LAUNCH();
   return T3D_OK;
 }
@@ -333,9 +387,17 @@
   return deep_shape(c.Kin, c.Nout) && deep_lds(cdiv(c.Kin, 32), DeepChunks(c.Nout).ntiles) <= 150 * 1024;
 }
 
+bool deep_pooled_can(const PwCall& c) {
+  return c.op == PW_DGRAD && deep_can(c) && deep_lds(cdiv(c.Kin, 32), DeepChunks(c.Nout).ntiles, 4, 5) <= 150 * 1024;
+}
+
 int deep_launch(const PwCall& c, GemmArgs& a, hipStream_t st) {
   if (!deep_can(c)) return T3D_ERR_ARG;
   const DeepChunks ch(a.Nout);
+  if (a.pool_g) {
+    if (!deep_pooled_can(c) || !a.dgrad) return T3D_ERR_ARG;
+    return launch_deep<true, 2, 4, true>(a, cdiv(a.Kin, 32), ch.ntiles, ch.nchunks, st);
+  }
   return a.dgrad ? launch_deep<true, 2, 4>(a, cdiv(a.Kin, 32), ch.ntiles, ch.nchunks, st)
                  : launch_deep<false, 2, 4>(a, cdiv(a.Kin, 32), ch.ntiles, ch.nchunks, st);
 }
diff --git a/3d-object-detection.pytorch_amd/csrc/pwconv_route.h b/3d-object-detection.pytorch_amd/csrc/pwconv_route.h
--- a/3d-object-detection.pytorch_amd/csrc/pwconv_route.h
+++ b/3d-object-detection.pytorch_amd/csrc/pwconv_route.h
@@ -22,9 +22,11 @@
 int t3d_pw_route(const PwCall& c);
 
 bool deep_can(const PwCall& c);
+bool deep_pooled_can(const PwCall& c);
 int deep_launch(const PwCall& c, GemmArgs& a, hipStream_t st);
 bool deep_shape(int Kin, int Nout);
 bool stream_can(const PwCall& c);
+bool stream_pooled_can(const PwCall& c);
 int stream_launch(const PwCall& c, GemmArgs& a, hipStream_t st);
 bool stream_f16_can(const PwCall& c);
 int stream_launch_f16(const PwCall& c, GemmArgs& a, hipStream_t st);
@@ -39,6 +41,7 @@
 int lds_wgrad_launch(const PwCall& c, const void* dz, const void* y, const t3d_bnbwd* bb, const void* x, const t3d_prologue* pro, float* dw,
                      hipStream_t st);
 bool tr_can(const PwCall& c);
+bool tr_pooled_can(const PwCall& c);
 int tr_launch(const PwCall& c, const void* dz, const void* y, const t3d_bnbwd* bb, const void* x, const t3d_prologue* pro, float* dw,
               hipStream_t st);
 
diff --git a/3d-object-detection.pytorch_amd/csrc/pwconv_route.hip b/3d-object-detection.pytorch_amd/csrc/pwconv_route.hip
--- a/3d-object-detection.pytorch_amd/csrc/pwconv_route.hip
+++ b/3d-object-detection.pytorch_amd/csrc/pwconv_route.hip
@@ -123,15 +123,23 @@
 extern "C" int t3d_pwconv_dgrad(int dtype, const void* dz, const void* y, const t3d_bnbwd* bb, const void* wt,
                                 const void* x_raw, const t3d_prologue* pro_in, const void* residual, void* dx,
                                 double* stats, float* ps_stats, int M, int HW, int K, int N, void* stream) {
-  if (!dz || !y || !bb || !wt || !dx || !bb->beta) return T3D_ERR_ARG;
+  if (!y || !bb || !wt || !dx || !bb->beta) return T3D_ERR_ARG;
+  const bool pooled = bb->pooled != nullptr;
+  if (pooled ? dz != nullptr : dz == nullptr) return T3D_ERR_ARG;
   PwCall c = call(PW_DGRAD, dtype, M, HW, N, K);
   c.per_sample = bb->per_sample != 0; c.alpha_gamma = bb->alpha && bb->gamma; c.e_se = x_raw && pro_in && pro_in->se;
   c.stats = stats != nullptr; c.ps_stats = ps_stats != nullptr;
   const int route = t3d_pw_route(c);
   if (route < 0) return route;
+  if (pooled && (c.gen() || !c.alpha_gamma || !(route == T3D_PW_DEEP ? deep_pooled_can(c) : route == T3D_PW_STREAM && stream_pooled_can(c))))
+    return T3D_ERR_UNSUPPORTED;
   GemmArgs a{};
   a.dgrad = 1;
   a.a0 = dz; a.a1 = y;
+  if (pooled) {
+    a.pool_g = bb->pooled; a.pool_scale = bb->pool_scale; a.pool_shift = bb->pool_shift; a.pool_act = bb->pool_act;
+    a.pool_inv_hw = 1.f / (float)HW;
+  }
   a.p0 = bb->alpha; a.p1 = bb->beta; a.p2 = bb->gamma; a.per_sample = bb->per_sample;
   a.w = wt;
   if (x_raw) {
@@ -148,11 +156,14 @@
 
 extern "C" int t3d_pwconv_wgrad(int dtype, const void* dz, const void* y, const t3d_bnbwd* bb, const void* x,
                                 const t3d_prologue* pro, float* dw, int M, int HW, int K, int N, void* stream) {
-  if (!dz || !y || !bb || !x || !dw) return T3D_ERR_ARG;
+  if (!y || !bb || !x || !dw) return T3D_ERR_ARG;
+  const bool pooled = bb->pooled != nullptr;
+  if (pooled ? dz != nullptr : dz == nullptr) return T3D_ERR_ARG;
   PwCall c = call(PW_WGRAD, dtype, M, HW, N, K);
   c.gated = pro && pro->se; c.per_sample = bb->per_sample != 0; c.alpha_gamma = bb->alpha && bb->gamma;
   const int route = t3d_pw_route(c);
   if (route < 0) return route;
+  if (pooled && !(route == T3D_PW_TR && tr_pooled_can(c))) return T3D_ERR_UNSUPPORTED;
   hipStream_t st = reinterpret_cast<hipStream_t>(stream);
   if (const int rc = settle(route, c, bb->alpha, st)) return rc;
   switch (route) {
diff --git a/3d-object-detection.pytorch_amd/csrc/pwconv_stream.hip b/3d-object-detection.pytorch_amd/csrc/pwconv_stream.hip
--- a/3d-object-detection.pytorch_amd/csrc/pwconv_stream.hip
+++ b/3d-object-detection.pytorch_amd/csrc/pwconv_stream.hip
@@ -46,14 +46,15 @@
 #define PW_STAMP(i)
 #endif
 
-template <int NT, int R, bool DG, bool GEN, bool YF = false, int KU = 2, bool ZM = false>
-__global__ __launch_bounds__(512, KU > 2 ? 1 : 2) void pw_stream_kernel(const GemmArgs a, const int nchunks, const int KS, const int nrep, const long long rstride) {
+template <int NT, int R, bool DG, bool GEN, bool YF, int KU, bool ZM, bool PG>
+__device__ __forceinline__ void pw_stream_body(const GemmArgs a, const int nchunks, const int KS, const int nrep, const long long rstride) {
+  static_assert(!PG || (DG && !GEN && !YF && !ZM), "the pooled form exists for the plain data gradient only");
   constexpr int BN = NT * 16;
   extern __shared__ __attribute__((aligned(16))) unsigned char smem[];
   ST8* Wf = reinterpret_cast<ST8*>(smem);
   const int kpad = KS * 32;
   float* coef = reinterpret_cast<float*>(smem + (size_t)NT * KS * 1024);
-  float* lstat = coef + 3 * kpad;
+  float* lstat = coef + (PG ? 5 : 3) * kpad;
   float* ecoef = lstat + BN * 2;
   double* dstat = reinterpret_cast<double*>(ecoef + 2 * BN);
 
@@ -132,6 +133,13 @@
   }
   };
   constexpr bool DGL = DG && !YF;
+  if constexpr (PG) {
+    for (int i = tid; i < kpad; i += nthr) {
+      const bool v = i < a.Kin && a.pool_scale;
+      coef[3 * kpad + i] = v ? a.pool_scale[i] : 1.f;
+      coef[4 * kpad + i] = v ? a.pool_shift[i] : 0.f;
+    }
+  }
   if (!YF && a.fold) {
     for (int i = a.Kin + tid; i < kpad; i += nthr) {
       coef[i] = DG ? 0.f : 1.f; coef[kpad + i] = 0.f; coef[2 * kpad + i] = 0.f;
@@ -195,6 +203,11 @@
       mok[r] = mrow[r] < mlim;
       mld[r] = min(mrow[r], a.M - 1);
     }
+    const float* grow[PG ? R : 1];
+    if constexpr (PG) {
+#pragma unroll
+      for (int r = 0; r < R; ++r) grow[r] = a.pool_g + (size_t)(mld[r] / a.HW) * a.Kin;
+    }
 
     constexpr bool HOIST = DG && !YF && !GEN && KU > 2;
     ST8 eyh[R][NT / 2];
@@ -211,6 +224,7 @@
       constexpr bool GUARD = decltype(guard_tag)::value;
       ST8 fa[KUr][R], fb[KUr][R];
       ST8 fz[ZM ? KUr : 1][R];
+      float4 fg[PG ? KUr : 1][R][2];
       float4 gs[GEN && !DGL ? KUr : 1][R][2];
       const bool gated = GEN && !DGL && a.p2 != nullptr;
 #pragma unroll
@@ -226,7 +240,12 @@
 #pragma unroll
           for (int r = 0; r < R; ++r) {
             {
-              fa[u][r] = *reinterpret_cast<const ST8*>(A0 + (size_t)mld[r] * a.row0 + k);
+              if constexpr (PG) {
+                fg[u][r][0] = *reinterpret_cast<const float4*>(grow[r] + k);
+                fg[u][r][1] = *reinterpret_cast<const float4*>(grow[r] + k + 4);
+              } else {
+                fa[u][r] = *reinterpret_cast<const ST8*>(A0 + (size_t)mld[r] * a.row0 + k);
+              }
               if (DGL) fb[u][r] = *reinterpret_cast<const ST8*>(A1 + (size_t)mld[r] * a.row0 + k);
               if constexpr (ZM) {
                 if (a.z_res)
@@ -312,6 +331,20 @@
               for (int r = 0; r < R; ++r) {
                 const bool ok = mok[r] && (k < a.Kin);
                 const size_t pb = (GEN && a.per_sample && ok) ? (size_t)(mrow[r] / a.HW) * a.Kin + k : 0;
+                if constexpr (PG) {
+                  const float4 sa = *reinterpret_cast<const float4*>(coef + 3 * kpad + k), sb = *reinterpret_cast<const float4*>(coef + 3 * kpad + k + 4);
+                  const float4 ha = *reinterpret_cast<const float4*>(coef + 4 * kpad + k), hb = *reinterpret_cast<const float4*>(coef + 4 * kpad + k + 4);
+                  const float ps[8] = {sa.x, sa.y, sa.z, sa.w, sb.x, sb.y, sb.z, sb.w}, ph[8] = {ha.x, ha.y, ha.z, ha.w, hb.x, hb.y, hb.z, hb.w};
+                  const float4 g0 = fg[PG ? u : 0][r][0], g1 = fg[PG ? u : 0][r][1];
+                  const float g[8] = {g0.x, g0.y, g0.z, g0.w, g1.x, g1.y, g1.z, g1.w};
+                  float yv[8], d[8];
+#pragma unroll
+                  for (int j = 0; j < 8; ++j) yv[j] = (float)fb[u][r][j];
+                  pooled_dz8(g, yv, ps, ph, a.pool_act, a.pool_inv_hw, d);
+#pragma unroll
+                  for (int j = 0; j < 8; ++j) b[r][j] = (ST)(c0[j] * d[j] + c1[j] * yv[j] + c2[j]);
+                  continue;
+                }
 #pragma unroll
                 for (int j = 0; j < 8; ++j) {
                   const float al = (GEN && a.per_sample) ? (ok ? a.p0[pb + j] : 0.f) : c0[j];
@@ -510,16 +543,37 @@
 }
 
 template <int NT, int R, bool DG, bool GEN, bool YF = false, int KU = 2, bool ZM = false>
+__global__ __launch_bounds__(512, KU > 2 ? 1 : 2) void pw_stream_kernel(const GemmArgs a, const int nchunks, const int KS, const int nrep, const long long rstride) {
+  pw_stream_body<NT, R, DG, GEN, YF, KU, ZM, false>(a, nchunks, KS, nrep, rstride);
+}
+
+#ifndef T3D_PW_F16
+template <int NT, int R>
+__global__ __launch_bounds__(512, 2) void pw_stream_pooled_kernel(const GemmArgs a, const int nchunks, const int KS, const int nrep, const long long rstride) {
+  pw_stream_body<NT, R, true, false, false, 2, false, true>(a, nchunks, KS, nrep, rstride);
+}
+#endif
+
+static size_t stream_lds(int NT, int KS, int rows) { return (size_t)NT * KS * 1024 + (size_t)rows * KS * 32 * 4 + NT * 16 * 4 * 4 + NT * 16 * 2 * 8; }
+
+template <int NT, int R, bool DG, bool GEN, bool YF = false, int KU = 2, bool ZM = false, bool PG = false>
 int launch_v(GemmArgs& a, int KS, hipStream_t st) {
   constexpr int BN = NT * 16;
   const int kpad = KS * 32;
-  const size_t lds = (size_t)NT * KS * 1024 + (size_t)3 * kpad * 4 + BN * 4 * 4 + BN * 2 * 8;
+  const size_t lds = stream_lds(NT, KS, PG ? 5 : 3);
+  const size_t lds_plan = stream_lds(NT, KS, 3);
+  (void)kpad;
   const int nchunks = cdiv(a.Nout, BN);
   const int ngroups = cdiv(a.M, 16 * R);
   const bool ps = GEN && a.ps_stats != nullptr;
   const int gps = cdiv(a.HW, 16 * R);
-  const int threads = (lds <= 48 * 1024 || (ps && gps <= 4)) ? 256 : 512;
+  const int threads = (lds_plan <= 48 * 1024 || (ps && gps <= 4)) ? 256 : 512;
   const void* fn = (const void*)pw_stream_kernel<NT, R, DG, GEN, YF, KU, ZM>;
+#ifndef T3D_PW_F16
+  if constexpr (PG) {
+    if (lds > 64 * 1024) (void)t3d_max_lds((const void*)pw_stream_pooled_kernel<NT, R>, (int)lds);
+  } else
+#endif
   if (lds > 64 * 1024) (void)t3d_max_lds(fn, (int)lds);
   static int occ_cache[2] = {0, 0};
   int& occ = occ_cache[threads == 512];
@@ -529,7 +583,7 @@
     occ = n;
   }
   int per_cu = occ;
-  const int by_lds = (int)(160 * 1024 / (lds + 512));
+  const int by_lds = (int)(160 * 1024 / (lds_plan + 512));
   if (per_cu > by_lds) per_cu = by_lds;
   if (per_cu < 1) per_cu = 1;
   int nxb = (256 * per_cu) / nchunks;
@@ -543,8 +597,16 @@
   }
   a.quant = (!DG && a.stats && !T3D_ENV_SET("T3D_NO_SNAP")) ? t3d_quant_for(a.M) : T3dQuant{0.0, 0.0};
   a.fold = (YF || a.per_sample) ? nullptr : t3d_take_fold(a.p0);
-  T3D_LAUNCH_TIMED((pw_stream_kernel<NT, R, DG, GEN, YF, KU, ZM>), dim3(nxb * nchunks), dim3(threads), lds, st, a, nchunks, KS,
-                     g_t3d_reduce.nrep, g_t3d_reduce.stats_stride);
+#ifndef T3D_PW_F16
+  if constexpr (PG) {
+    T3D_LAUNCH_TIMED((pw_stream_pooled_kernel<NT, R>), dim3(nxb * nchunks), dim3(threads), lds, st, a, nchunks, KS,
+                       g_t3d_reduce.nrep, g_t3d_reduce.stats_stride);
+  } else
+#endif
+  {
+    T3D_LAUNCH_TIMED((pw_stream_kernel<NT, R, DG, GEN, YF, KU, ZM>), dim3(nxb * nchunks), dim3(threads), lds, st, a, nchunks, KS,
+                       g_t3d_reduce.nrep, g_t3d_reduce.stats_stride);
+  }
   T3D_CHECK_LAUNCH();
   return T3D_OK;
 }
@@ -557,6 +619,7 @@
 #else
   if (a.a2) return launch_v<NT, R, true, false, true>(a, KS, st);
   const bool gen = a.per_sample || a.ps_stats || a.e_se || (!a.dgrad && a.p2);
+  if (a.dgrad && a.pool_g) return gen ? T3D_ERR_ARG : launch_v<NT, R, true, false, false, 2, false, true>(a, KS, st);
   if (a.dgrad) return gen ? launch_v<NT, R, true, true>(a, KS, st) : launch_v<NT, R, true, false>(a, KS, st);
   if (a.z_out) return launch_v<NT, R, false, false, false, 2, true>(a, KS, st);
   return gen ? launch_v<NT, R, false, true>(a, KS, st) : launch_v<NT, R, false, false>(a, KS, st);
@@ -578,6 +641,13 @@
   if (c.dtype != T3D_BF16 || c.op == PW_WGRAD || c.Kin > 1920) return false;
   if (c.ps_stats && (c.stats || c.M % c.HW)) return false;
   return !(c.op == PW_MAT && c.gated);
+}
+bool stream_pooled_can(const PwCall& c) {
+  if (!stream_can(c) || c.op != PW_DGRAD || c.gen()) return false;
+  const int KS = cdiv(c.Kin, 32);
+  int nt = 120 / KS;
+  if (nt > 10) nt = 10;
+  return stream_lds(nt & ~1, KS, 5) + 512 <= 160 * 1024;
 }
 #endif
 
diff --git a/3d-object-detection.pytorch_amd/csrc/pwconv_wgrad_tr.hip b/3d-object-detection.pytorch_amd/csrc/pwconv_wgrad_tr.hip
--- a/3d-object-detection.pytorch_amd/csrc/pwconv_wgrad_tr.hip
+++ b/3d-object-detection.pytorch_amd/csrc/pwconv_wgrad_tr.hip
@@ -49,7 +49,10 @@
   double* stats;
   int nrep;
   long long rstride;
-  int unused_[10];
+  const float *pool_g, *pool_scale, *pool_shift;
+  int pool_act;
+  float pool_inv_hw;
+  int unused_[2];
   int assign;
   int gs_ns;
   unsigned mulHW;
@@ -65,9 +68,10 @@
   return __builtin_bit_cast(bf16x8, v);
 }
 
-template <int NTPW, int NTQ, bool SWAP, int G, int D, int GEN, bool YF, int SK = 1, bool DGF = false>
-__global__ __launch_bounds__(256 * G) void pw_wgrad_tr_kernel(const WgtArgs a) {
+template <int NTPW, int NTQ, bool SWAP, int G, int D, int GEN, bool YF, int SK, bool DGF, bool PG>
+__device__ __forceinline__ void pw_wgrad_tr_body(const WgtArgs a) {
   static_assert(!DGF || (YF && !SWAP), "the fused data gradient exists for the y-free layout only");
+  static_assert(!PG || (!GEN && !YF && !DGF), "the pooled form exists for the plain kernel only");
   constexpr int PB = 64 * NTPW, QB = 16 * NTQ;
   constexpr int RSP = PB + 8, RSQ = QB + 8;
   constexpr int STEP = 32 * SK;
@@ -125,6 +129,15 @@
     ca[aB + i] = ((v && a.scale) ? a.shift[k] : 0.f) * (c6 ? T3D_SIXTH : 1.f);
   }
   float* const gsl = coef + ((NCOEF + 3) & ~3);
+  float* const pco = gsl;
+  if constexpr (PG) {
+    for (int i = threadIdx.x; i < dyB; i += 256 * G) {
+      const int n = dy0 + i;
+      const bool v = n < a.N && a.pool_scale;
+      pco[i] = v ? a.pool_scale[n] : 1.f;
+      pco[dyB + i] = v ? a.pool_shift[n] : 0.f;
+    }
+  }
   const int gs_b0 = GEN ? mbeg / a.HW : 0;
   if constexpr (GEN == 2) {
     {
@@ -233,12 +246,14 @@
   struct NoMask {};
   struct Regs { bf16x8 rz[VDY], ry[VDY], rx[VA]; Epi e; NoMask okm; };
   Regs rr[D];
+  typedef f32x4 PoolG[PG ? VDY : 1][2];
+  PoolG rgp[PG ? D : 1];
   Epi ecur;
   const int lgq = lane >> 4, lcq = lane & 15;
   const bf16_t* __restrict__ eres = reinterpret_cast<const bf16_t*>(a.e_res);
   const bf16_t* __restrict__ eyr = reinterpret_cast<const bf16_t*>(a.e_y);
 
-  auto gload = [&](Regs& R, int m0) {
+  auto gload = [&](Regs& R, PoolG& RG, int m0) {
 #pragma unroll
     for (int i = 0; i < VDY; ++i) {
       const int v = min(tid + 256 * i, ndv - 1);
@@ -250,7 +265,13 @@
         R.rz[i] = *reinterpret_cast<const bf16x8*>(src);
       } else {
         const int n = min(dy0 + (v % dyV) * 8, a.N - 8);
-        R.rz[i] = *reinterpret_cast<const bf16x8*>(dz + (size_t)m * a.N + n);
+        if constexpr (PG) {
+          const float* gp = a.pool_g + (size_t)(m / a.HW) * a.N + n;
+          RG[i][0] = *reinterpret_cast<const f32x4*>(gp);
+          RG[i][1] = *reinterpret_cast<const f32x4*>(gp + 4);
+        } else {
+          R.rz[i] = *reinterpret_cast<const bf16x8*>(dz + (size_t)m * a.N + n);
+        }
         R.ry[i] = *reinterpret_cast<const bf16x8*>(yy + (size_t)m * a.N + n);
       }
     }
@@ -277,7 +298,7 @@
   bf16x8 zero8;
 #pragma unroll
   for (int j = 0; j < 8; ++j) zero8[j] = (bf16_t)0.f;
-  auto lstore = [&](const Regs& R, int m0, int buf) {
+  auto lstore = [&](const Regs& R, const PoolG& RG, int m0, int buf) {
     const auto& rz = R.rz; const auto& ry = R.ry; const auto& rx = R.rx;
     bf16_t* const pb_ = tiles + buf * BUFE;
     bf16_t* const qb_ = pb_ + STEP * RSP;
@@ -316,8 +337,20 @@
           ld8(cdy + cl, al);
           ld8(cdy + 2 * dyB + cl, ga);
         }
-#pragma unroll
-        for (int j = 0; j < 8; ++j) o[j] = (bf16_t)fmaf(al[j], (float)rz[i][j], fmaf(be[j], (float)ry[i][j], ga[j]));
+        if constexpr (PG) {
+          float ps[8], ph[8], yv[8], d[8];
+          ld8(pco + cl, ps);
+          ld8(pco + dyB + cl, ph);
+          const float g[8] = {RG[i][0][0], RG[i][0][1], RG[i][0][2], RG[i][0][3], RG[i][1][0], RG[i][1][1], RG[i][1][2], RG[i][1][3]};
+#pragma unroll
+          for (int j = 0; j < 8; ++j) yv[j] = (float)ry[i][j];
+          t3d_pw::pooled_dz8(g, yv, ps, ph, a.pool_act, a.pool_inv_hw, d);
+#pragma unroll
+          for (int j = 0; j < 8; ++j) o[j] = (bf16_t)fmaf(al[j], d[j], fmaf(be[j], yv[j], ga[j]));
+        } else {
+#pragma unroll
+          for (int j = 0; j < 8; ++j) o[j] = (bf16_t)fmaf(al[j], (float)rz[i][j], fmaf(be[j], (float)ry[i][j], ga[j]));
+        }
         *reinterpret_cast<bf16x8*>(dyt + row * rsd + cl) = ok ? o : zero8;
       }
     }
@@ -441,8 +474,8 @@
   const int niter = (nsteps + G - 1) / G;
   auto step_m = [&](int it) { return mbeg + (it * G + grp) * STEP; };
 #pragma unroll
-  for (int u = 0; u < D; ++u) gload(rr[u], step_m(u));
-  lstore(rr[0], step_m(0), 0);
+  for (int u = 0; u < D; ++u) gload(rr[u], rgp[PG ? u : 0], step_m(u));
+  lstore(rr[0], rgp[0], step_m(0), 0);
   if constexpr (DGF) ecur = rr[0].e;
   __syncthreads();
   int buf = 0;
@@ -451,7 +484,7 @@
     for (int u = 0; u < D; ++u) {
       const int it = it0 + u;
       if (it < niter) {
-        gload(rr[u], step_m(it + D));
+        gload(rr[u], rgp[PG ? u : 0], step_m(it + D));
         const bf16_t* pcur = tiles + buf * BUFE;
         const bf16_t* qcur = pcur + STEP * RSP;
 #pragma unroll
@@ -470,7 +503,7 @@
           dgrad_step(pcur, step_m(it));
           ecur = rr[(u + 1) % D].e;
         }
-        lstore(rr[(u + 1) % D], step_m(it + 1), buf ^ 1);
+        lstore(rr[(u + 1) % D], rgp[PG ? (u + 1) % D : 0], step_m(it + 1), buf ^ 1);
         __syncthreads();
         buf ^= 1;
       }
@@ -546,6 +579,16 @@
           unsafeAtomicAdd(a.dw + (size_t)n * a.K + k, acc[i][j][r]);
         }
       }
+}
+
+template <int NTPW, int NTQ, bool SWAP, int G, int D, int GEN, bool YF, int SK = 1, bool DGF = false>
+__global__ __launch_bounds__(256 * G) void pw_wgrad_tr_kernel(const WgtArgs a) {
+  pw_wgrad_tr_body<NTPW, NTQ, SWAP, G, D, GEN, YF, SK, DGF, false>(a);
+}
+
+template <int NTPW, int NTQ, bool SWAP, int G, int D, int SK>
+__global__ __launch_bounds__(256 * G) void pw_wgrad_tr_pooled_kernel(const WgtArgs a) {
+  pw_wgrad_tr_body<NTPW, NTQ, SWAP, G, D, 0, false, SK, false, true>(a);
 }
 
 template <int SP>
@@ -606,7 +649,7 @@
   }
 }
 
-template <int NTPW, int NTQ, bool SWAP, int D, int GEN, bool YF = false, int SK = 1>
+template <int NTPW, int NTQ, bool SWAP, int D, int GEN, bool YF = false, int SK = 1, bool PG = false>
 int launch_d(WgtArgs& a, hipStream_t st) {
   constexpr int G = 2;
   constexpr int STEP = 32 * SK;
@@ -617,6 +660,7 @@
   const int tiles = a.ptiles * a.qtiles;
   const int dyB = a.swap ? QB : PB, aB = a.swap ? PB : QB;
   size_t lds = (size_t)G * 2 * STEP * ((PB + 8) + (QB + 8)) * 2 + (size_t)(3 * dyB + 2 * aB) * 4;
+  if (PG) lds += (size_t)2 * dyB * 4;
   const int tgt_blocks = 256;
   const long long cap_mb = 8;
   int S = (tgt_blocks + tiles - 1) / tiles;
@@ -644,10 +688,15 @@
   }
   a.ws = use_ws ? reinterpret_cast<float*>(g_t3d_ws.ptr) : nullptr;
   if (a.assign && !use_ws && hipMemsetAsync(a.dw, 0, (size_t)a.N * a.K * sizeof(float), st) != hipSuccess) return T3D_ERR_LAUNCH;
-  if (lds > 64 * 1024)
-    (void)t3d_max_lds((const void*)pw_wgrad_tr_kernel<NTPW, NTQ, SWAP, G, D, GEN, YF, SK, false>, (int)lds);
   a.nsplit = S;
-  T3D_LAUNCH_TIMED((pw_wgrad_tr_kernel<NTPW, NTQ, SWAP, G, D, GEN, YF, SK, false>), dim3(tiles * S), dim3(256 * G), lds, st, a);
+  if constexpr (PG) {
+    if (lds > 64 * 1024) (void)t3d_max_lds((const void*)pw_wgrad_tr_pooled_kernel<NTPW, NTQ, SWAP, G, D, SK>, (int)lds);
+    T3D_LAUNCH_TIMED((pw_wgrad_tr_pooled_kernel<NTPW, NTQ, SWAP, G, D, SK>), dim3(tiles * S), dim3(256 * G), lds, st, a);
+  } else {
+    if (lds > 64 * 1024)
+      (void)t3d_max_lds((const void*)pw_wgrad_tr_kernel<NTPW, NTQ, SWAP, G, D, GEN, YF, SK, false>, (int)lds);
+    T3D_LAUNCH_TIMED((pw_wgrad_tr_kernel<NTPW, NTQ, SWAP, G, D, GEN, YF, SK, false>), dim3(tiles * S), dim3(256 * G), lds, st, a);
+  }
   if (use_ws) {
 #define T3D_WGR(SPV)                                                                                                              \
   do {                                                                                                                            \
@@ -681,6 +730,11 @@
   }
   if (a.per_sample) return launch_d<NTPW, NTQ, SWAP, 1, 1>(a, st);
   if (a.se) return launch_d<NTPW, NTQ, SWAP, 2, 2>(a, st);
+  if (a.pool_g) {
+    if constexpr (narrow)
+      if (sk2) return launch_d<NTPW, NTQ, SWAP, 2, false, false, 2, true>(a, st);
+    return launch_d<NTPW, NTQ, SWAP, 2, false, false, 1, true>(a, st);
+  }
   if constexpr (narrow)
     if (sk2) return launch_d<NTPW, NTQ, SWAP, 2, false, false, 2>(a, st);
   return launch_d<NTPW, NTQ, SWAP, 2, false>(a, st);
@@ -730,6 +784,7 @@
 }
 
 bool t3d_pw::tr_can(const PwCall& c) { return c.dtype == T3D_BF16 && c.op == PW_WGRAD; }
+bool t3d_pw::tr_pooled_can(const PwCall& c) { return tr_can(c) && !c.per_sample && !c.gated && c.alpha_gamma; }
 
 int t3d_pw::tr_launch(const PwCall& c, const void* dz, const void* y, const t3d_bnbwd* bb, const void* x, const t3d_prologue* pro,
                       float* dw, hipStream_t st) {
@@ -739,6 +794,11 @@
   a.alpha = bb->alpha; a.beta = bb->beta; a.gamma = bb->gamma; a.per_sample = bb->per_sample;
   if (pro) { a.scale = pro->scale; a.shift = pro->shift; a.se = pro->se; a.act = pro->act; a.se_after = pro->se_after_act; }
   a.dw = dw; a.M = c.M; a.HW = c.HW; a.K = c.Nout; a.N = c.Kin;
+  if (bb->pooled) {
+    if (dz || !tr_pooled_can(c)) return T3D_ERR_ARG;
+    a.pool_g = bb->pooled; a.pool_scale = bb->pool_scale; a.pool_shift = bb->pool_shift; a.pool_act = bb->pool_act;
+    a.pool_inv_hw = 1.f / (float)c.HW;
+  }
   a.fold = a.per_sample ? nullptr : t3d_take_fold(a.alpha);
   return choose_and_launch(a, st);
 }
diff --git a/3d-object-detection.pytorch_amd/torchdet3d/_native.py b/3d-object-detection.pytorch_amd/torchdet3d/_native.py
--- a/3d-object-detection.pytorch_amd/torchdet3d/_native.py
+++ b/3d-object-detection.pytorch_amd/torchdet3d/_native.py
@@ -18,7 +18,8 @@
 
 
 class BnBwd(ctypes.Structure):
-    _fields_ = [('alpha', _P), ('beta', _P), ('gamma', _P), ('per_sample', _I)]
+    _fields_ = [('alpha', _P), ('beta', _P), ('gamma', _P), ('per_sample', _I), ('pool_act', _I), ('pooled', _P),
+                ('pool_scale', _P), ('pool_shift', _P)]
 
 
 class Prologue(ctypes.Structure):
@@ -198,9 +199,14 @@
     return p
 
 
-def bnbwd(alpha, beta, gamma, per_sample=False):
+def bnbwd(alpha, beta, gamma, per_sample=False, pooled=None, pool_pro=None):
     b = BnBwd(ptr(alpha), ptr(beta), ptr(gamma), int(per_sample))
     b._keep = (alpha, beta, gamma)
+    if pooled is not None:
+        b.pooled = ptr(pooled)
+        if pool_pro is not None:
+            b.pool_scale, b.pool_shift, b.pool_act = pool_pro.scale, pool_pro.shift, pool_pro.act
+        b._keep += (pooled, pool_pro)
     return b
 
 
diff --git a/3d-object-detection.pytorch_amd/torchdet3d/models/engine.py b/3d-object-detection.pytorch_amd/torchdet3d/models/engine.py
--- a/3d-object-detection.pytorch_amd/torchdet3d/models/engine.py
+++ b/3d-object-detection.pytorch_amd/torchdet3d/models/engine.py
@@ -61,6 +61,10 @@
 
 
 _concurrent_stream.log = []
+
+
+def _gated(x):
+    return bool((x.pro is not None and x.pro.se) or (x.gpro is not None and x.gpro.se))
 
 
 class _Src:
@@ -116,6 +120,7 @@
         self.persistent_outputs = False
         self.set_input_normalization([0.5931, 0.4690, 0.4229], [0.2471, 0.2214, 0.2157])
         self._fused_eval = True
+        self._tensor_pool_bwd = False
 
     def set_input_normalization(self, mean, std):
         self.in_mean = torch.tensor(mean, dtype=torch.float32, device=self.device)
@@ -991,10 +996,13 @@
         bnl = self.bns[a.keys.last_bn]
         x = sv['last_in']
         M, HW = B * sv['HWl'], sv['HWl']
-        dzl = self._buf('dz:last', (M, a.last_c))
+        pooled = self._pooled_last(x, M, HW)
+        dzl = None if pooled else self._buf('dz:last', (M, a.last_c))
         N.call('t3d_pool_bwd', dt, N.ptr(dpooled), N.ptr(sv['yl']), sv['prol'], self.pool, N.ptr(sv['pool_argmax']),
                N.ptr(dzl), self._bst(bnl), B, HW, a.last_c, st)
         bb = self._bn_bwd(bnl)
+        if pooled:
+            bb = N.bnbwd(bnl.alpha, bnl.bbeta, bnl.gammac, False, pooled=dpooled, pool_pro=sv['prol'])
         def last_wgrad():
             self._wgrad(dt, N.ptr(dzl), N.ptr(sv['yl']), bb, N.ptr(x.t), x.pro,
                         N.ptr(self.g[lw]), M, HW, x.C, a.last_c, nbytes=M * (x.C + a.last_c) * self.esz,
@@ -1008,6 +1016,17 @@
             self._maybe_hook(self.offsets[a.keys.blocks[rec['idx']].first][0])
 
         self._stem_wgrad(sv, dz, dw32)
+
+    def _pooled_last(self, x, M, HW):
+        a = self.arch
+        if self._tensor_pool_bwd or self.dt != N.BF16 or self.pool != N.POOL['avg'] or _gated(x):
+            return False
+        with_stats = x.bn is not None and not x.finished_act
+        wd, _ = self._wsel(self.wt[a.keys.last_w])
+        route = N.lib().t3d_pwconv_route
+        dg = route(N.PW_OP_DGRAD, wd, 0, 0, 0, 0, 0, int(with_stats), 1, 0, 0, M, HW, x.C, a.last_c)
+        wg = route(N.PW_OP_WGRAD, self.dt, 0, 0, 0, 0, 0, 0, 1, 0, 0, M, HW, x.C, a.last_c)
+        return dg in (N.PW_DEEP, N.PW_STREAM) and wg == N.PW_TR
 
     def _stem_wgrad(self, sv, dz, dw32):
         a, st, dt = self.arch, N.stream(), self.dt
diff --git a/include/t3d.h b/include/t3d.h
--- a/include/t3d.h
+++ b/include/t3d.h
@@ -39,6 +39,10 @@
   const float* beta;
   const float* gamma;
   int per_sample;
+  int pool_act;
+  const float* pooled;
+  const float* pool_scale;
+  const float* pool_shift;
 } t3d_bnbwd;
 
 int t3d_pwconv_fwd(int dtype, const void* x, const t3d_prologue* pro, const void* w, const float* bias,
```

Result: no change. 39220 crops/s, median of 5 (+0.3%).
